# NVIDIA-ISAAC-ROS/isaac_ros_nvblox

Hardware: AMD Instinct MI355X
Metric: frames/s, TSDF+Color+ESDF integrate per frame, synthetic Replica-like 640x480 @0.05m (higher is better)
Workload: dtype f32; 1 GPU; configs[1]: synthetic Replica-like room (SURVEY 8d); scene=room, cameras_per_gpu=1, unique_frames=200, color_deferral=True, parallelism=single GPU

## Files before the change

### isaac_ros_nvblox_amd/csrc/esdf.hip

```cpp
#include <algorithm>
#include <cmath>
#include <cstring>
#include <vector>
#include "nvbx_mapper.h"
#include "nvbx_esdf_mark.h"
#include "nvbx_esdf_edt.h"

using namespace nvbx;

__global__ __launch_bounds__(64) void k_esdf_mark(DMap m, EsdfArgs a) { esdf_mark_worker(m, a, (int)blockIdx.x, (int)gridDim.x); esdf_mark_pass_done(m, a, (int)gridDim.x); }

__global__ __launch_bounds__(256) void k_esdf_edt(DMap m, EsdfArgs a) {
  __shared__ EdtShared sh;
  esdf_edt_worker(m, a, (int)blockIdx.x, (int)gridDim.x, &sh);
}

constexpr int PROP_BATCH = 16;
constexpr int32_t PROP_NONE = INT32_MAX;
__device__ inline bool prop_block(const DMap& m, const EsdfArgs& a, int32_t s, uint32_t* flags_out) {
  const uint32_t flags = m.slot_flags[s];
  *flags_out = flags;
  return (flags & (F_ESDF | F_ESDF_PENDING)) && m.slot_index[3 * s + 2] == a.bz_out;
}
__global__ __launch_bounds__(64) void k_esdf_prop_init(DMap m, EsdfArgs a, int32_t plane_a) {
// ... 203 lines not shown
  NVBX_LAUNCH(m, k_esdf_slice, dim3(std::min(nbx * nby, 4096)), dim3(64), m->d, a.bz_out, a.vz_out, m->p.voxel_size,
                     unknown_value, image_dev, c[0], c[1], nbx, nby);
  NVBX_HIP(hipGetLastError());
  return NVBX_OK;
}

__global__ __launch_bounds__(64) void k_esdf_slice_rows(DMap m, int32_t bz_out, int32_t vz_out, float voxel_size, float unknown, float* img, int64_t cap, int32_t* header) {
  const int32_t bx0 = m.counters[C_ESDF_AABB], by0 = m.counters[C_ESDF_AABB + 1], bx1 = m.counters[C_ESDF_AABB + 2], by1 = m.counters[C_ESDF_AABB + 3];
  const int lane = (int)threadIdx.x;
  const bool empty = bx0 > bx1;
  const int32_t nbx = empty ? 0 : bx1 - bx0 + 1, nby = empty ? 0 : by1 - by0 + 1;
  const bool fits = (int64_t)nbx * nby * 64 <= cap;
  if (blockIdx.x == 0 && lane < 5) header[lane] = lane == 0 ? bx0 : lane == 1 ? by0 : lane == 2 ? bx1 : lane == 3 ? by1 : (empty ? 0 : (fits ? 1 : -1));
  if (empty || !fits) return;
  const int32_t strips_x = (nbx + 7) / 8, cols = nbx * 8;
  for (int32_t s = (int32_t)blockIdx.x; s < strips_x * nby; s += (int32_t)gridDim.x) {
    const int32_t cy = s / strips_x, cx0 = (s - cy * strips_x) * 8;
    uint32_t es = SLOT_NONE;
    if (lane < 8 && cx0 + lane < nbx) es = find_slot(m, bx0 + cx0 + lane, by0 + cy, bz_out, F_ESDF);
    const uint32_t mine = __shfl(es, lane >> 3);
    const bool in_img = cx0 + (lane >> 3) < nbx;
#pragma unroll
    for (int r = 0; r < 8; r++) {
      float v = unknown;
      if (slot_ok(mine)) {
        const uint2 e = m.esdf[(size_t)mine * 512 + vz_out * 64 + r * 8 + (lane & 7)];
        if (e.y & ESDF_OBSERVED) { v = sqrtf(__uint_as_float(e.x)) * voxel_size; if (e.y & ESDF_INSIDE) v = -v; }
      }
      if (in_img) img[(int64_t)(cy * 8 + r) * cols + cx0 * 8 + lane] = v;
    }
  }
}
static int ensure_slice_pinned(nvbx_mapper* m, int64_t elems) {
  if (elems <= m->slice_pinned_elems) return NVBX_OK;
  NVBX_HIP(hipStreamSynchronize(m->stream));
  if (m->slice_pinned) NVBX_HIP(hipHostFree(m->slice_pinned));
  m->slice_pinned = nullptr; m->slice_pinned_elems = 0; m->slice_pinned_dev = nullptr;
  NVBX_HIP(hipHostMalloc((void**)&m->slice_pinned, (size_t)(elems + 16) * 4, hipHostMallocMapped));
  { void* dp = nullptr; NVBX_HIP(hipHostGetDevicePointer(&dp, m->slice_pinned, 0)); m->slice_pinned_dev = (float*)dp; }
  m->slice_pinned_elems = elems;
  return NVBX_OK;
}

extern "C" int nvbx_esdf_slice_to_host(nvbx_mapper* m, float unknown_value, float* image_host, int64_t capacity_elems, int32_t* rows,
                                       int32_t* cols, float aabb[6]) {
  if (!m || !rows || !cols) return NVBX_E_INVALID;
  *rows = 0; *cols = 0;
  if (m->join_side()) return NVBX_E_DEVICE;
  int rc = ensure_slice_pinned(m, std::max<int64_t>(image_host ? capacity_elems : 0, 65536)); if (rc) return rc;
  const EsdfArgs a = m->make_esdf_args();
  int32_t* header = reinterpret_cast<int32_t*>(m->slice_pinned_dev);
  volatile int32_t* h = reinterpret_cast<volatile int32_t*>(m->slice_pinned);
  NVBX_LAUNCH(m, k_esdf_slice_rows, dim3(1024), dim3(64), m->d, a.bz_out, a.vz_out, m->p.voxel_size, unknown_value, m->slice_pinned_dev + 16, m->slice_pinned_elems, header);
  NVBX_HIP(hipGetLastError());
  if (m->wait_stream()) return NVBX_E_DEVICE;
  if (h[4] == 0) return NVBX_OK;
  const float bs = m->p.voxel_size * 8.0f;
  *cols = (h[2] - h[0] + 1) * 8; *rows = (h[3] - h[1] + 1) * 8;
  if (aabb) {
    aabb[0] = (float)h[0] * bs; aabb[1] = (float)h[1] * bs; aabb[2] = (float)a.bz_out * bs;
    aabb[3] = (float)(h[2] + 1) * bs; aabb[4] = (float)(h[3] + 1) * bs; aabb[5] = (float)(a.bz_out + 1) * bs;
  }
  const int64_t n = (int64_t)*rows * *cols;
  if (!image_host || n > capacity_elems) { set_error("slice image capacity too small"); return NVBX_E_CAPACITY; }
  if (h[4] < 0) {
    rc = ensure_slice_pinned(m, n + n / 2); if (rc) return rc;
    return nvbx_esdf_slice_to_host(m, unknown_value, image_host, capacity_elems, rows, cols, aabb);
  }
  memcpy(image_host, m->slice_pinned + 16, (size_t)n * 4);
  return NVBX_OK;
}

__global__ void k_occupancy(const float* img, int64_t n, float unknown, int8_t* grid) {
  for (int64_t i = (int64_t)blockIdx.x * blockDim.x + threadIdx.x; i < n; i += (int64_t)gridDim.x * blockDim.x) {
    const float v = img[i];
    int8_t o = 0;
    if (fabsf(v - unknown) < 1e-2f) o = -1; else if (v <= 0.0f) o = 100;
    grid[i] = o;
  }
}
extern "C" int nvbx_occupancy_grid_from_slice(nvbx_mapper* m, const float* image_dev, int32_t rows, int32_t cols, float unknown_value,
                                              int8_t* grid_dev) {
  if (!m || !image_dev || !grid_dev || rows <= 0 || cols <= 0) return NVBX_E_INVALID;
  if (m->join_side()) return NVBX_E_DEVICE;
  const int64_t n = (int64_t)rows * cols;
  NVBX_LAUNCH(m, k_occupancy, dim3((unsigned)std::min<int64_t>((n + 255) / 256, 2048)), dim3(256), image_dev, n, unknown_value, grid_dev);
  NVBX_HIP(hipGetLastError());
  return NVBX_OK;
}

__global__ __launch_bounds__(64) void k_slice_pointcloud(DMap m, const float* img, int32_t rows, int32_t cols, float ax, float ay,
                                                         float slice_height, float voxel_size, float unknown, float4* out) {
  const int lane = threadIdx.x;
  const int tiles_x = (cols + 7) >> 3, tiles_y = (rows + 7) >> 3;
  for (int32_t t = blockIdx.x; t < tiles_x * tiles_y; t += gridDim.x) {
    const int ty = t / tiles_x, tx = t - ty * tiles_x;
    const int r = ty * 8 + (lane >> 3), c = tx * 8 + (lane & 7);
    bool keep = false; float v = 0.0f;
    if (r < rows && c < cols) { v = img[(int64_t)r * cols + c]; keep = !(fabsf(v - unknown) < 1e-2f); }
    const u64 mask = __ballot(keep);
    int base = 0;
    if (lane == 0 && mask) base = atomicAdd(&m.counters[C_TMP], (int)__popcll(mask));
    base = __shfl(base, 0);
    if (keep) {
      const int off = (int)__popcll(mask & ((1ull << lane) - 1ull));
      out[base + off] = make_float4(ax + voxel_size * (float)c, ay + voxel_size * (float)r, slice_height, v);
    }
  }
}
__global__ void k_zero_tmp2(DMap m) { m.counters[C_TMP] = 0; }

extern "C" int nvbx_pointcloud_from_slice(nvbx_mapper* m, const float* image_dev, int32_t rows, int32_t cols, const float aabb[6],
                                          float slice_height, float unknown_value, float* points_xyzi_dev, int32_t* n_points) {
  if (!m || !image_dev || !aabb || !points_xyzi_dev || !n_points || rows <= 0 || cols <= 0) return NVBX_E_INVALID;
  if (m->join_side()) return NVBX_E_DEVICE;
  NVBX_LAUNCH(m, k_zero_tmp2, dim3(1), dim3(1), m->d);
  const int tiles = ((rows + 7) / 8) * ((cols + 7) / 8);
  NVBX_LAUNCH(m, k_slice_pointcloud, dim3(std::min(tiles, 4096)), dim3(64), m->d, image_dev, rows, cols, aabb[0], aabb[1],
                     slice_height, m->p.voxel_size, unknown_value, (float4*)points_xyzi_dev);
  if (m->fetch_counters()) return NVBX_E_DEVICE;
  *n_points = m->h_counters[C_TMP];
  return NVBX_OK;
}

__global__ void k_esdf_dense(DMap m, int32_t mx, int32_t my, int32_t mz, int32_t sx, int32_t sy, int32_t sz, float voxel_size, float def, float* out) {
  const int64_t n = (int64_t)sx * sy * sz;
  for (int64_t i = (int64_t)blockIdx.x * blockDim.x + threadIdx.x; i < n; i += (int64_t)gridDim.x * blockDim.x) {
    const int32_t z = (int32_t)(i % sz), y = (int32_t)((i / sz) % sy), x = (int32_t)(i / ((int64_t)sz * sy));
    const int32_t gx = mx + x, gy = my + y, gz = mz + z;
    const uint32_t es = find_slot(m, gx >> 3, gy >> 3, gz >> 3, F_ESDF);
    float v = def;
    if (slot_ok(es)) {
      const uint2 e = m.esdf[(size_t)es * 512 + (gx & 7) + 8 * (gy & 7) + 64 * (gz & 7)];
      if (e.y & ESDF_OBSERVED) { v = sqrtf(__uint_as_float(e.x)) * voxel_size; if (e.y & ESDF_INSIDE) v = v * -1.0f; }
    }
    out[i] = v;
  }
}
extern "C" int nvbx_esdf_dense_grid(nvbx_mapper* m, const int32_t min_vox[3], const int32_t size_vox[3], float default_value, float* grid_dev) {
  if (!m || !min_vox || !size_vox || !grid_dev || size_vox[0] <= 0 || size_vox[1] <= 0 || size_vox[2] <= 0) return NVBX_E_INVALID;
  if (m->join_side()) return NVBX_E_DEVICE;
  const int64_t n = (int64_t)size_vox[0] * size_vox[1] * size_vox[2];
  NVBX_LAUNCH(m, k_esdf_dense, dim3((unsigned)std::min<int64_t>((n + 255) / 256, 4096)), dim3(256), m->d, min_vox[0], min_vox[1],
                     min_vox[2], size_vox[0], size_vox[1], size_vox[2], m->p.voxel_size, default_value, grid_dev);
  NVBX_HIP(hipGetLastError());
  return NVBX_OK;
}

__global__ void k_export_dirty(DMap m, int32_t* out_idx, int32_t* out_count, int32_t cap) {
  ListView lv;
  int32_t n = list_open(m, S_LIST_ESDF_DIRTY, &lv); if (n > cap) n = cap;
  if (blockIdx.x == 0 && threadIdx.x == 0) *out_count = n;
  for (int32_t i = blockIdx.x * blockDim.x + threadIdx.x; i < n; i += gridDim.x * blockDim.x) {
    const int32_t s = list_at(m, S_LIST_ESDF_DIRTY, lv, i);
    out_idx[3 * i] = m.slot_index[3 * s]; out_idx[3 * i + 1] = m.slot_index[3 * s + 1]; out_idx[3 * i + 2] = m.slot_index[3 * s + 2];
  }
}
extern "C" int nvbx_esdf_dirty_list(nvbx_mapper* m, int32_t* indices_dev_out, int32_t* count_dev_out, int64_t capacity) {
  if (!m || !indices_dev_out || !count_dev_out || capacity <= 0) return NVBX_E_INVALID;
  if (m->join_side()) return NVBX_E_DEVICE;
  NVBX_LAUNCH(m, k_export_dirty, dim3(64), dim3(256), m->d, indices_dev_out, count_dev_out, (int32_t)std::min<int64_t>(capacity, m->capacity));
  NVBX_HIP(hipGetLastError());
  return NVBX_OK;
}
extern "C" int nvbx_set_view_export(nvbx_mapper* m, int32_t* packed_dev, int64_t capacity) {
  if (!m || capacity < 0) return NVBX_E_INVALID;
  m->view_export = packed_dev; m->view_export_cap = packed_dev ? std::min<int64_t>(capacity, m->capacity) : 0;
  return NVBX_OK;
}
__global__ void k_import_dirty(DMap m, const int32_t* idx, const int32_t* count, int64_t max_count) {
  int64_t n = *count; if (n > max_count) n = max_count;
  for (int64_t i = (int64_t)blockIdx.x * blockDim.x + threadIdx.x; i < n; i += (int64_t)gridDim.x * blockDim.x) {
    const uint32_t s = find_slot(m, idx[3 * i], idx[3 * i + 1], idx[3 * i + 2], F_TSDF);
    if (!slot_ok(s)) continue;
    const uint32_t old = atomicOr(&m.slot_flags[s], F_DIRTY_ESDF);
    if (!(old & F_DIRTY_ESDF)) list_append(m, S_LIST_ESDF_DIRTY, (int32_t)s);
  }
}
extern "C" int nvbx_mark_esdf_dirty(nvbx_mapper* m, const int32_t* indices_dev, const int32_t* count_dev, int64_t max_count) {
  if (!m || !indices_dev || !count_dev || max_count < 0) return NVBX_E_INVALID;
  if (m->join_side()) return NVBX_E_DEVICE;
  if (m->begin_dirtying()) return NVBX_E_DEVICE;
  NVBX_LAUNCH(m, k_import_dirty, dim3(64), dim3(256), m->d, indices_dev, count_dev, max_count);
  NVBX_HIP(hipGetLastError());
  return m->mark_main();
}

__global__ void k_import_dirty_gathered(DMap m, const int32_t* g, int32_t self_rank, int64_t max_count) {
  const int32_t r = (int32_t)blockIdx.y;
  if (r == self_rank) return;
  const int32_t* base = g + (size_t)r * (size_t)(max_count + 1) * 3;
  int64_t n = base[0]; if (n > max_count) n = max_count;
  const int32_t* idx = base + 3;
  for (int64_t i = (int64_t)blockIdx.x * blockDim.x + threadIdx.x; i < n; i += (int64_t)gridDim.x * blockDim.x) {
    const uint32_t s = find_slot(m, idx[3 * i], idx[3 * i + 1], idx[3 * i + 2], F_TSDF);
    if (!slot_ok(s)) continue;
    const uint32_t old = atomicOr(&m.slot_flags[s], F_DIRTY_ESDF);
    if (!(old & F_DIRTY_ESDF)) list_append(m, S_LIST_ESDF_DIRTY, (int32_t)s);
  }
}
__global__ __launch_bounds__(64) void k_import_mark_gathered(DMap m, EsdfArgs a, const int32_t* g, int32_t self_rank, int64_t max_count) {
  const int32_t r = (int32_t)blockIdx.y;
  if (r == self_rank) return;
  const int32_t* base = g + (size_t)r * (size_t)(max_count + 1) * 3;
  int64_t n = base[0]; if (n > max_count) n = max_count;
  const int32_t* idx = base + 3;
  const int srec = S_ESDF_REC + (int)(a.epoch & 1), sh = my_shard();
  for (int64_t i = blockIdx.x; i < n; i += gridDim.x) {
    const uint32_t s = find_slot(m, idx[3 * i], idx[3 * i + 1], idx[3 * i + 2], F_TSDF);
    if (!slot_ok(s)) continue;
    esdf_mark_entry(m, a, s, srec, sh);
  }
}
extern "C" int nvbx_mark_esdf_dirty_gathered(nvbx_mapper* m, const int32_t* gathered_dev, int32_t world, int32_t self_rank, int64_t max_count) {
  if (!m || !gathered_dev || world < 1 || max_count < 0) return NVBX_E_INVALID;
  if (m->join_side()) return NVBX_E_DEVICE;
  if (!(world > 1 || self_rank < 0)) return NVBX_OK;
  const EsdfArgs probe = m->make_esdf_args();
  if (m->p.esdf_mode == 0 && probe.bz_hi >= probe.bz_lo && probe.bz_hi - probe.bz_lo + 1 <= 63) {
    m->mark_pass++;
    const EsdfArgs a = m->make_esdf_args();
    m->unresolved_marks = true;
    NVBX_LAUNCH(m, k_import_mark_gathered, dim3(256, (unsigned)world), dim3(64), m->d, a, gathered_dev, self_rank, max_count);
  } else {
    if (m->begin_dirtying()) return NVBX_E_DEVICE;
    NVBX_LAUNCH(m, k_import_dirty_gathered, dim3(16, (unsigned)world), dim3(256), m->d, gathered_dev, self_rank, max_count);
  }
  NVBX_HIP(hipGetLastError());
  return m->mark_main();
}

__global__ __launch_bounds__(64) void k_undo_marks(DMap m, uint32_t pass_floor, int32_t srec, int32_t vz_out) {
  const int lane = threadIdx.x;
  if (blockIdx.x == 0 && lane < NSH) *shc_at(m, srec, lane, 4) = 0;
  const int32_t hw = m.counters[C_HIGH_WATER];
  for (int32_t s = blockIdx.x; s < hw; s += gridDim.x) {
    const uint32_t flags = m.slot_flags[s], cons = m.slot_consumed[s], stamp = m.slot_stamp[s];
    const bool cons_unres = cons != STAMP_NEVER && (int32_t)(cons - pass_floor) > 0;
    const bool stamp_unres = stamp != STAMP_NEVER && (int32_t)(stamp - pass_floor) > 0;
    if (cons_unres && lane == 0) {
      m.slot_consumed[s] = STAMP_NEVER;
      if (flags & (F_TSDF | F_COLOR | F_ESDF | F_MESH | F_ESDF_PENDING)) {
        const uint32_t old = atomicOr(&m.slot_flags[s], F_DIRTY_ESDF);
        if (!(old & F_DIRTY_ESDF)) list_append(m, S_LIST_ESDF_DIRTY, s);
      }
    }
    if (stamp_unres) {
      if (flags & F_ESDF) {
        const uint32_t meta = m.esdf[(size_t)s * 512 + vz_out * 64 + lane].y;
        const u64 sb = __ballot((meta & ESDF_SITE) != 0), ob = __ballot((meta & ESDF_OBSERVED) != 0), ib = __ballot((meta & ESDF_INSIDE) != 0);
        if (lane == 0) { m.site_bits[s] = sb; m.obs_bits[s] = ob; m.inside_bits[s] = ib; m.slot_stamp[s] = STAMP_NEVER; }
      } else if ((flags & F_ESDF_PENDING) && lane == 0) {
        atomicAnd(&m.slot_flags[s], ~F_ESDF_PENDING);
        m.site_bits[s] = 0ull; m.obs_bits[s] = 0ull; m.inside_bits[s] = 0ull; m.slot_stamp[s] = STAMP_NEVER;
        if (!(flags & (F_TSDF | F_COLOR | F_ESDF | F_MESH))) {
          atomicAnd(&m.slot_flags[s], ~(F_DIRTY_ESDF | F_DIRTY_MESH));
          const int32_t pos = atomicAdd(&m.counters[C_FREE_TOP], 1);
          m.free_stack[pos] = (uint32_t)s;

        }
      }
    }
  }
}
int nvbx_mapper::undo_marks() {
  if (!unresolved_marks) return NVBX_OK;
  if (reset_consumed_list()) return NVBX_E_DEVICE;
  const EsdfArgs a = make_esdf_args();
  NVBX_LAUNCH(this, k_undo_marks, dim3((unsigned)std::min<int64_t>(capacity, 2048)), dim3(64), d, pass_at_last_edt,
              (int32_t)(S_ESDF_REC + (int)(a.epoch & 1)), a.vz_out);
  NVBX_HIP(hipGetLastError());
  unresolved_marks = false; dirty_since_mark = true;
  return NVBX_OK;
}

extern "C" int nvbx_mark_esdf_dirty_gathered_deferred(nvbx_mapper* m, const int32_t* gathered_dev, int32_t world, int32_t self_rank, int64_t max_count) {
  if (!m || !gathered_dev || world < 1 || max_count < 0) return NVBX_E_INVALID;
  if (m->flush_import()) return NVBX_E_DEVICE;
  if (!(world > 1 || self_rank < 0)) return NVBX_OK;
  const EsdfArgs probe = m->make_esdf_args();
  if (!(m->p.esdf_mode == 0 && probe.bz_hi >= probe.bz_lo && probe.bz_hi - probe.bz_lo + 1 <= 63))
    return nvbx_mark_esdf_dirty_gathered(m, gathered_dev, world, self_rank, max_count);
  m->held.import_pending = true; m->held.import_ptr = gathered_dev; m->held.import_world = world; m->held.import_rank = self_rank; m->held.import_max = max_count;
  return NVBX_OK;
}
int nvbx_mapper::flush_import() {
  if (!held.import_pending) return NVBX_OK;
  held.import_pending = false;
  if (flush_edt()) return NVBX_E_DEVICE;
  mark_pass++;
  const EsdfArgs a = make_esdf_args();
  unresolved_marks = true;
  NVBX_LAUNCH(this, k_import_mark_gathered, dim3(256, (unsigned)held.import_world), dim3(64), d, a, held.import_ptr, held.import_rank, held.import_max);
  NVBX_HIP(hipGetLastError());
  return NVBX_OK;
}

int nvbx_mapper::flush_edt() {
  if (held.edt_pending) {
    held.edt_pending = false;
    NVBX_LAUNCH(this, k_esdf_edt, dim3(1024), dim3(256), d, held.edt_args);
    NVBX_HIP(hipGetLastError());
  }
  return NVBX_OK;
}
```

### isaac_ros_nvblox_amd/csrc/esdf3d.hip

```cpp
#include <algorithm>
#include <cmath>
#include "nvbx_mapper.h"

using namespace nvbx;

struct Win3 { int32_t bx0, by0, bz0, nbx, nby, nbz; };
constexpr uint32_t B_NONE = 0xFFFFFFFFu;

__global__ __launch_bounds__(512) void k_esdf3_mark(DMap m, EsdfArgs a) {
  const int tid = threadIdx.x;
  const int vx = tid >> 6, vy = (tid >> 3) & 7, vz = tid & 7;
  ListView lv;
  const int32_t n = list_open(m, S_LIST_ESDF_DIRTY, &lv);
  for (int32_t i = blockIdx.x; i < n; i += gridDim.x) {
    const uint32_t s = (uint32_t)list_at(m, S_LIST_ESDF_DIRTY, lv, i);
    const uint32_t flags = m.slot_flags[s];
    if (!(flags & (F_TSDF | F_ESDF))) continue;
    const float2 tv = m.tsdf[(size_t)s * 512 + tid];
    int observed = 0, inside = 0, site = 0;
    if (a.site_rule == 2) { if (tv.x != 0.0f) observed = 1; if (tv.x > 0.0f) { inside = 1; site = 1; } }
    else if ((flags & F_TSDF) && tv.y >= a.min_weight) {
      observed = 1;
      const int in = tv.x <= 0.0f;
      if (in) inside = 1;
      if ((a.site_rule == 1 || in) && fabsf(tv.x) <= a.site_dist_m) site = 1;
    }
    uint2* ev = &m.esdf[(size_t)s * 512 + vx + 8 * vy + 64 * vz];
    const uint2 old = *ev;
    *ev = make_uint2(old.x, (old.y & ~ESDF_FLAG_MASK) | (observed ? ESDF_OBSERVED : 0u) | (inside ? ESDF_INSIDE : 0u) | (site ? ESDF_SITE : 0u));
    if (tid == 0) {
      atomicOr(&m.slot_flags[s], F_ESDF);
      atomicAnd(&m.slot_flags[s], ~(F_DIRTY_ESDF | F_ESDF_REMARK));
      const int32_t bx = m.slot_index[3 * s], by = m.slot_index[3 * s + 1], bz = m.slot_index[3 * s + 2];
      if (bz == a.bz_out) {
        atomicMin(&m.counters[C_ESDF_AABB + 0], bx); atomicMin(&m.counters[C_ESDF_AABB + 1], by);
        atomicMax(&m.counters[C_ESDF_AABB + 2], bx); atomicMax(&m.counters[C_ESDF_AABB + 3], by);
      }
      atomicMin(&m.counters[C_ESDF3_WIN + 0], bx); atomicMin(&m.counters[C_ESDF3_WIN + 1], by); atomicMin(&m.counters[C_ESDF3_WIN + 2], bz);
      atomicMax(&m.counters[C_ESDF3_WIN + 3], bx); atomicMax(&m.counters[C_ESDF3_WIN + 4], by); atomicMax(&m.counters[C_ESDF3_WIN + 5], bz);
      atomicAdd(&m.counters[C_ESDF3_WIN + 6], 1);
    }
  }
}
__global__ void k_esdf3_reset(DMap m) {
  const int t = threadIdx.x;
  if (t < 3) m.counters[C_ESDF3_WIN + t] = INT32_MAX; else if (t < 6) m.counters[C_ESDF3_WIN + t] = INT32_MIN; else if (t == 6) m.counters[C_ESDF3_WIN + 6] = 0;
  if (t < NSH) *shc_at(m, S_LIST_ESDF_DIRTY, t, 0) = 0;
}

__global__ __launch_bounds__(64) void k_esdf3_bits(DMap m, Win3 w, uint8_t* bits) {
  const int lane = threadIdx.x, y = lane & 7, z = lane >> 3;
  const int64_t nblk = (int64_t)w.nbx * w.nby * w.nbz;
  const int64_t H = (int64_t)w.nby * 8;
  for (int64_t c = blockIdx.x; c < nblk; c += gridDim.x) {
    const int32_t cx = (int32_t)(c % w.nbx), cy = (int32_t)((c / w.nbx) % w.nby), cz = (int32_t)(c / ((int64_t)w.nbx * w.nby));
    const uint32_t s = find_slot(m, w.bx0 + cx, w.by0 + cy, w.bz0 + cz, F_ESDF);
    uint32_t byte = 0;
    if (slot_ok(s)) {
      const uint2* row = &m.esdf[(size_t)s * 512 + 8 * y + 64 * z];
#pragma unroll
      for (int x = 0; x < 8; x++) if (row[x].y & ESDF_SITE) byte |= 1u << x;
    }
    bits[(((int64_t)cz * 8 + z) * H + (int64_t)cy * 8 + y) * w.nbx + cx] = (uint8_t)byte;
  }
}
__device__ inline bool bit_at(const uint8_t* row_bits, int32_t nbx, int64_t x) {
  if (x < 0 || x >= (int64_t)nbx * 8) return false;
  return (row_bits[x >> 3] >> (x & 7)) & 1u;
}
__global__ __launch_bounds__(256) void k_esdf3_x(Win3 w, const uint8_t* bits, int8_t* A, int32_t ri) {
  const int64_t rows = (int64_t)w.nbz * 8 * w.nby * 8;
  const int64_t n = rows * w.nbx;
  for (int64_t i = (int64_t)blockIdx.x * blockDim.x + threadIdx.x; i < n; i += (int64_t)gridDim.x * blockDim.x) {
    const int64_t r = i / w.nbx; const int32_t cx = (int32_t)(i - r * w.nbx);
    const uint8_t* rb = bits + r * w.nbx;
    int8_t out[8];
#pragma unroll
    for (int x = 0; x < 8; x++) {
      const int64_t p = (int64_t)cx * 8 + x;
      int best = 127;
      for (int32_t d = 0; d <= ri; d++) {
        if (bit_at(rb, w.nbx, p - d)) { best = -d; break; }
        if (bit_at(rb, w.nbx, p + d)) { best = d; break; }
      }
      out[x] = (int8_t)best;
    }
    *reinterpret_cast<uint2*>(A + r * ((int64_t)w.nbx * 8) + (int64_t)cx * 8) = *reinterpret_cast<const uint2*>(out);
  }
}
__global__ __launch_bounds__(256) void k_esdf3_y(Win3 w, const int8_t* A, uint32_t* B, int32_t ri) {
  const int64_t W = (int64_t)w.nbx * 8, H = (int64_t)w.nby * 8, D = (int64_t)w.nbz * 8;
  const int64_t n = W * H * D;
  for (int64_t i = (int64_t)blockIdx.x * blockDim.x + threadIdx.x; i < n; i += (int64_t)gridDim.x * blockDim.x) {
    const int64_t x = i % W, y = (i / W) % H, z = i / (W * H);
    const int8_t* col = A + z * H * W + x;
    uint32_t best = B_NONE;
    for (int32_t k = 0; k <= ri; k++) {
      if (best != B_NONE && (uint32_t)(k * k) > (best >> 16)) break;
      for (int sgn = (k == 0 ? 1 : -1); sgn <= 1; sgn += 2) {
        const int64_t yy = y + (int64_t)sgn * k;
        if (yy < 0 || yy >= H) continue;
        const int dx = col[yy * W];
        if (dx == 127) continue;
        const uint32_t key = ((uint32_t)(k * k + dx * dx) << 16) | ((uint32_t)(sgn * k + 128) << 8) | (uint32_t)(dx + 128);
        if (key < best) best = key;
      }
    }
    B[i] = best;
  }
}
__global__ __launch_bounds__(512) void k_esdf3_z(DMap m, Win3 w, int32_t margin, const uint32_t* B, int32_t ri, float max_sq) {
  const int tid = threadIdx.x;
  const int x = tid & 7, y = (tid >> 3) & 7, z = tid >> 6;
  const int32_t ox = w.nbx - 2 * margin, oy = w.nby - 2 * margin, oz = w.nbz - 2 * margin;
  const int64_t W = (int64_t)w.nbx * 8, H = (int64_t)w.nby * 8, D = (int64_t)w.nbz * 8;
  const int64_t nblk = (int64_t)ox * oy * oz;
  for (int64_t c = blockIdx.x; c < nblk; c += gridDim.x) {
    const int32_t cx = (int32_t)(c % ox) + margin, cy = (int32_t)((c / ox) % oy) + margin, cz = (int32_t)(c / ((int64_t)ox * oy)) + margin;
    const uint32_t s = find_slot(m, w.bx0 + cx, w.by0 + cy, w.bz0 + cz, F_ESDF);
    if (!slot_ok(s)) continue;
    const int64_t gx = (int64_t)cx * 8 + x, gy = (int64_t)cy * 8 + y, gz = (int64_t)cz * 8 + z;
    const uint32_t* colz = B + gy * W + gx;
    uint64_t best = ~0ull;
    for (int32_t k = 0; k <= ri; k++) {
      if (best != ~0ull && (uint64_t)(k * k) > (best >> 32)) break;
      for (int sgn = (k == 0 ? 1 : -1); sgn <= 1; sgn += 2) {
        const int64_t zz = gz + (int64_t)sgn * k;
        if (zz < 0 || zz >= D) continue;
        const uint32_t b = colz[zz * H * W];
        if (b == B_NONE) continue;
        const uint64_t key = ((uint64_t)((uint32_t)(k * k) + (b >> 16)) << 32) | ((uint64_t)(uint32_t)(sgn * k + 128) << 24) | (uint64_t)(b & 0xFFFFu);
        if (key < best) best = key;
      }
    }
    uint2* ev = &m.esdf[(size_t)s * 512 + tid];
    const uint32_t fl = ev->y & ESDF_FLAG_MASK;
    float sq = max_sq; int dx = 0, dy = 0, dz = 0;
    if (best != ~0ull && (float)(uint32_t)(best >> 32) <= max_sq) {
      sq = (float)(uint32_t)(best >> 32);
      dz = (int)((best >> 24) & 0xFF) - 128; dy = (int)((best >> 8) & 0xFF) - 128; dx = (int)(best & 0xFF) - 128;
    }
    *ev = make_uint2(__float_as_uint(sq), (esdf_meta(dx, dy, dz, 0, 0, 0) & ~ESDF_FLAG_MASK) | fl);
  }
}

int nvbx_mapper::update_esdf_3d() {
  const EsdfArgs a = make_esdf_args();
  if (dirty_since_mark) NVBX_LAUNCH(this, k_esdf3_mark, dim3((unsigned)std::min<int64_t>(capacity, 1024)), dim3(512), d, a);
  dirty_since_mark = false; premark_consumed = false;
  if (fetch_counters()) return NVBX_E_DEVICE;
  const int32_t* c = h_counters + C_ESDF3_WIN;
  esdf3_blocks_marked = c[6];
  if (c[0] > c[3]) { NVBX_LAUNCH(this, k_esdf3_reset, dim3(1), dim3(64), d); esdf_epoch++; return NVBX_OK; }
  const int32_t rb = a.rb;
  Win3 w;
  w.bx0 = c[0] - 2 * rb; w.by0 = c[1] - 2 * rb; w.bz0 = c[2] - 2 * rb;
  w.nbx = c[3] - c[0] + 1 + 4 * rb; w.nby = c[4] - c[1] + 1 + 4 * rb; w.nbz = c[5] - c[2] + 1 + 4 * rb;
  const int64_t nblk = (int64_t)w.nbx * w.nby * w.nbz, nvox = nblk * 512;
  if (nvox > (1ll << 31)) { set_error("3-D ESDF update: the changed region (+ 2 R) exceeds 2^31 voxels; update more often or lower esdf_max_distance_m"); return NVBX_E_CAPACITY; }
  const int64_t need = nvox / 8 + nvox + nvox * 4 + 1024;
  if (esdf3_scratch.ensure(stream, (size_t)need)) return NVBX_E_DEVICE;
  uint32_t* B = esdf3_scratch.as<uint32_t>();
  int8_t* A = esdf3_scratch.as<int8_t>() + nvox * 4;
  uint8_t* bits = esdf3_scratch.as<uint8_t>() + nvox * 5;
  const unsigned gblk = (unsigned)std::min<int64_t>(nblk, 1 << 16);
  NVBX_LAUNCH(this, k_esdf3_bits, dim3(gblk), dim3(64), d, w, bits);
  NVBX_LAUNCH(this, k_esdf3_x, dim3((unsigned)std::min<int64_t>((nvox / 8 + 255) / 256, 1 << 16)), dim3(256), w, (const uint8_t*)bits, A, a.ri);
  NVBX_LAUNCH(this, k_esdf3_y, dim3((unsigned)std::min<int64_t>((nvox + 255) / 256, 1 << 18)), dim3(256), w, (const int8_t*)A, B, a.ri);
// ... 8 lines not shown
```

### isaac_ros_nvblox_amd/csrc/layers.hip

```cpp
#include <cstring>
#include "nvbx_mapper.h"
using namespace nvbx;

__global__ void k_collect_indices(DMap m, uint32_t layer, int32_t* out, int32_t cap) {
  const int32_t hw = m.counters[C_HIGH_WATER];
  for (int32_t s = blockIdx.x * blockDim.x + threadIdx.x; s < hw; s += gridDim.x * blockDim.x) {
    if (m.slot_flags[s] & layer) {
      const int32_t p = atomicAdd(&m.counters[C_TMP], 1);
      if (p < cap) { out[3 * p] = m.slot_index[3 * s]; out[3 * p + 1] = m.slot_index[3 * s + 1]; out[3 * p + 2] = m.slot_index[3 * s + 2]; }
    }
  }
}
__global__ void k_zero_tmp(DMap m) { m.counters[C_TMP] = 0; }

__global__ void k_viewlist_to_indices(DMap m, const int4* list, int32_t count_idx, uint32_t cam_mask, int32_t* out, int32_t cap) {
  int32_t n = m.counters[count_idx]; if (n > cap) n = cap;
  for (int32_t i = blockIdx.x * blockDim.x + threadIdx.x; i < n; i += gridDim.x * blockDim.x) {
    const int4 r = list[i];
    bool ok = slot_ok((uint32_t)r.x) && m.slot_flags[(uint32_t)r.x];
    if (ok && cam_mask && !(m.table[m.slot_entry[(uint32_t)r.x]].stamp & cam_mask)) ok = false;
    out[3 * i] = ok ? r.y : INT32_MIN; out[3 * i + 1] = ok ? r.z : INT32_MIN; out[3 * i + 2] = ok ? r.w : INT32_MIN;
  }
}

__global__ void k_shardlist_to_indices(DMap m, int list, int32_t* out, int32_t cap, int32_t* n_out) {
  ListView v; int32_t n = list_open(m, list, &v); if (n > cap) n = cap;
  if (blockIdx.x == 0 && threadIdx.x == 0) *n_out = n;
  for (int32_t i = blockIdx.x * blockDim.x + threadIdx.x; i < n; i += gridDim.x * blockDim.x) {
    const uint32_t s = (uint32_t)list_at(m, list, v, i);
    if (slot_ok(s) && m.slot_flags[s]) { out[3 * i] = m.slot_index[3 * s]; out[3 * i + 1] = m.slot_index[3 * s + 1]; out[3 * i + 2] = m.slot_index[3 * s + 2]; }
    else { out[3 * i] = INT32_MIN; out[3 * i + 1] = INT32_MIN; out[3 * i + 2] = INT32_MIN; }
  }
}

__global__ __launch_bounds__(512) void k_gather_blocks(DMap m, uint32_t layer, int32_t occupancy, const int32_t* idx, int32_t n, uint8_t* out, int32_t* found) {
  const int i = blockIdx.x; if (i >= n) return;
  const uint32_t s = find_slot(m, idx[3 * i], idx[3 * i + 1], idx[3 * i + 2], layer);
  const int t = threadIdx.x;
  if (t == 0) found[i] = slot_ok(s) ? 1 : 0;
  if (!slot_ok(s)) {
    const size_t vb = layer == F_ESDF ? sizeof(nvbx_esdf_voxel) : (layer == F_FREESPACE ? sizeof(nvbx_freespace_voxel) : ((layer == F_TSDF && occupancy) ? 4 : 8));
    for (size_t q = t; q < 512 * vb / 4; q += 512) reinterpret_cast<uint32_t*>(out + (size_t)i * 512 * vb)[q] = 0u;
    return;
  }
  if (layer == F_TSDF && occupancy) { reinterpret_cast<float*>(out)[(size_t)i * 512 + t] = m.tsdf[(size_t)s * 512 + t].x; }
  else if (layer == F_TSDF) { reinterpret_cast<float2*>(out)[(size_t)i * 512 + t] = m.tsdf[(size_t)s * 512 + t]; }
  else if (layer == F_COLOR) { reinterpret_cast<uint2*>(out)[(size_t)i * 512 + t] = m.color[(size_t)s * 512 + t]; }
  else if (layer == F_FREESPACE) {
    const int4 v = m.freespace[(size_t)s * 512 + t];
    nvbx_freespace_voxel o;
    o.last_occupied_timestamp_ms = (int64_t)(((u64)(uint32_t)v.y << 32) | (u64)(uint32_t)v.x);
    o.consecutive_occupancy_duration_ms = (int64_t)v.z;
    o.is_high_confidence_freespace = (uint8_t)(v.w & 1); o.initialized = (uint8_t)((v.w >> 1) & 1);
    for (int q = 0; q < 6; q++) o.pad[q] = 0;
    reinterpret_cast<nvbx_freespace_voxel*>(out)[(size_t)i * 512 + t] = o;
  }
  else if (layer == F_ESDF) {
    const int x = t >> 6, y = (t >> 3) & 7, z = t & 7;
    const uint2 v = m.esdf[(size_t)s * 512 + x + 8 * y + 64 * z];
    nvbx_esdf_voxel o;
    o.squared_distance_vox = __uint_as_float(v.x);
    o.parent_direction[0] = (int8_t)(v.y & 0xFF); o.parent_direction[1] = (int8_t)((v.y >> 8) & 0xFF); o.parent_direction[2] = (int8_t)((v.y >> 16) & 0xFF);
    o.observed = (v.y & ESDF_OBSERVED) ? 1 : 0; o.is_inside = (v.y & ESDF_INSIDE) ? 1 : 0; o.is_site = (v.y & ESDF_SITE) ? 1 : 0; o.pad = 0;
    reinterpret_cast<nvbx_esdf_voxel*>(out)[(size_t)i * 512 + t] = o;
  }
}

__global__ __launch_bounds__(512) void k_scatter_blocks(DMap m, uint32_t layer, int32_t occupancy, const int32_t* idx, const uint8_t* in_all, size_t block_bytes,
                                                        int32_t mesh_list, int32_t bz_out, int32_t vz_out, float trunc) {
  __shared__ uint32_t s_slot;
  __shared__ u64 s_sites, s_obs, s_ins;
  const int t = threadIdx.x;
  const int32_t x = idx[3 * blockIdx.x], y = idx[3 * blockIdx.x + 1], z = idx[3 * blockIdx.x + 2];
  const uint8_t* in = in_all + (size_t)blockIdx.x * block_bytes;
  if (t == 0) {
    bool is_new; const int32_t h = hash_insert(m, x, y, z, layer, &is_new);
    uint32_t s = SLOT_NONE;
    if (h >= 0) { do { s = ld_slot_acquire(&m.table[h]); } while (s == SLOT_INVALID); }
    if (slot_ok(s)) {
      uint32_t add = layer;
      if (layer == F_TSDF) add |= F_DIRTY_ESDF | F_DIRTY_MESH;
      const uint32_t old = atomicOr(&m.slot_flags[s], add);
      if (layer == F_TSDF) {
        if (!(old & F_DIRTY_ESDF)) list_append(m, S_LIST_ESDF_DIRTY, (int32_t)s);
        if (!(old & F_DIRTY_MESH)) list_append(m, mesh_list, (int32_t)s);
      }
      if (layer == F_ESDF && z == bz_out) {
        atomicMin(&m.counters[C_ESDF_AABB + 0], x); atomicMin(&m.counters[C_ESDF_AABB + 1], y);
        atomicMax(&m.counters[C_ESDF_AABB + 2], x); atomicMax(&m.counters[C_ESDF_AABB + 3], y);
      }
    }
    s_slot = s; s_sites = 0ull; s_obs = 0ull; s_ins = 0ull;
  }
  __syncthreads();
  const uint32_t s = s_slot;
  if (!slot_ok(s)) return;
  if (layer == F_TSDF && occupancy) m.tsdf[(size_t)s * 512 + t] = make_float2(reinterpret_cast<const float*>(in)[t], 0.0f);
  else if (layer == F_TSDF) {
    const float2 v = reinterpret_cast<const float2*>(in)[t];
    m.tsdf[(size_t)s * 512 + t] = v;
    publish_band(m.slot_flags, s, t, in_band(v.x, v.y, trunc));
  }
  else if (layer == F_COLOR) m.color[(size_t)s * 512 + t] = reinterpret_cast<const uint2*>(in)[t];
  else if (layer == F_ESDF) {
    const int vx = t >> 6, vy = (t >> 3) & 7, vz = t & 7;
    const nvbx_esdf_voxel v = reinterpret_cast<const nvbx_esdf_voxel*>(in)[t];
    m.esdf[(size_t)s * 512 + vx + 8 * vy + 64 * vz] =
        make_uint2(__float_as_uint(v.squared_distance_vox),
                   esdf_meta(v.parent_direction[0], v.parent_direction[1], v.parent_direction[2], v.observed, v.is_inside, v.is_site));
    if (z == bz_out && vz == vz_out) {
      if (v.is_site) atomicOr(&s_sites, 1ull << (vx + 8 * vy));
      if (v.observed) atomicOr(&s_obs, 1ull << (vx + 8 * vy));
      if (v.is_inside) atomicOr(&s_ins, 1ull << (vx + 8 * vy));
    }
    __syncthreads();
    if (t == 0) { m.site_bits[s] = (z == bz_out) ? s_sites : 0ull; m.obs_bits[s] = (z == bz_out) ? s_obs : 0ull; m.inside_bits[s] = (z == bz_out) ? s_ins : 0ull; }
  }
}
uint32_t nvbx::internal_layer(const nvbx_mapper* m, uint32_t layer) {
  const bool occ = m->p.projective_layer_type == 1;
  if (layer == NVBX_LAYER_OCCUPANCY) return occ ? F_TSDF : 0u;
  if (layer == F_TSDF) return occ ? 0u : F_TSDF;
  if (layer == F_FREESPACE) return m->d.freespace ? F_FREESPACE : 0u;
  return layer;
}

static void sort_indices(nvbx_index3d* v, int64_t n) {
  std::sort(v, v + n, [](const nvbx_index3d& a, const nvbx_index3d& b) {
    if (a.x != b.x) return a.x < b.x; if (a.y != b.y) return a.y < b.y; return a.z < b.z; });
}
static int64_t download_indices(nvbx_mapper* m, int64_t n, bool filter, nvbx_index3d* out, int64_t capacity) {
  if (!filter && !(out && std::min(n, capacity) > 0)) return n;
  std::vector<nvbx_index3d> tmp((size_t)n);
  if (n > 0) NVBX_HIP(hipMemcpy(tmp.data(), m->export_idx, (size_t)n * 12, hipMemcpyDeviceToHost));
  if (filter) { tmp.erase(std::remove_if(tmp.begin(), tmp.end(), [](const nvbx_index3d& i) { return i.x == INT32_MIN; }), tmp.end()); n = (int64_t)tmp.size(); }
  const int64_t k = std::min(n, capacity);
  if (out && k > 0) { sort_indices(tmp.data(), n); memcpy(out, tmp.data(), (size_t)k * 12); }
  return n;
}

extern "C" int64_t nvbx_block_indices(nvbx_mapper* m, uint32_t layer, nvbx_index3d* out, int64_t capacity) {
  if (!m || !layer_listable(layer)) return NVBX_E_INVALID;
  layer = internal_layer(m, layer);
  if (!layer) return 0;
  if (m->join_side()) return NVBX_E_DEVICE;
  NVBX_LAUNCH(m, k_zero_tmp, dim3(1), dim3(1), m->d);
  NVBX_LAUNCH(m, k_collect_indices, dim3(256), dim3(256), m->d, layer, m->export_idx, (int32_t)m->capacity);
  if (m->fetch_counters()) return NVBX_E_DEVICE;
  int64_t n = m->h_counters[C_TMP];
  if (n > m->capacity) n = m->capacity;
  return download_indices(m, n, false, out, capacity);
}
extern "C" int64_t nvbx_num_blocks(nvbx_mapper* m, uint32_t layer) { return nvbx_block_indices(m, layer, nullptr, 0); }

extern "C" int64_t nvbx_last_depth_view(nvbx_mapper* m, nvbx_index3d* out, int64_t capacity) {
  if (!m) return NVBX_E_INVALID;
  if (m->last_view_frame == 0) return 0;
  if (m->join_side()) return NVBX_E_DEVICE;
  const uint32_t cam_mask = m->last_view_batch > 1 ? (1u << (m->last_view_batch - 1)) : 0u;
  NVBX_LAUNCH(m, k_viewlist_to_indices, dim3(64), dim3(256), m->d, (const int4*)m->view_list, C_VIEW_COUNT + (int)(m->last_view_frame & 3), cam_mask, m->export_idx, (int32_t)m->capacity);
  if (m->fetch_counters()) return NVBX_E_DEVICE;
  int64_t n = m->h_counters[C_VIEW_COUNT + (m->last_view_frame & 3)]; if (n > m->capacity) n = m->capacity;
  return download_indices(m, n, true, out, capacity);
}
extern "C" int64_t nvbx_last_color_view(nvbx_mapper* m, nvbx_index3d* out, int64_t capacity) {
  if (!m) return NVBX_E_INVALID;
  if (m->join_side()) return NVBX_E_DEVICE;
  NVBX_LAUNCH(m, k_shardlist_to_indices, dim3(64), dim3(256), m->d, (int)S_LIST_COLOR, m->export_idx, (int32_t)m->capacity, m->export_count);
  int32_t n32 = 0;
  NVBX_HIP(hipMemcpyAsync(&n32, m->export_count, 4, hipMemcpyDeviceToHost, m->stream));
  NVBX_HIP(hipStreamSynchronize(m->stream));
  return download_indices(m, n32, false, out, capacity);
}

size_t nvbx::ref_voxel_bytes(uint32_t layer) { return layer == F_ESDF ? sizeof(nvbx_esdf_voxel) : (layer == NVBX_LAYER_OCCUPANCY ? sizeof(nvbx_occupancy_voxel) : (layer == F_FREESPACE ? sizeof(nvbx_freespace_voxel) : 8)); }

extern "C" int nvbx_get_blocks(nvbx_mapper* m, uint32_t layer, const nvbx_index3d* idx, int64_t n, void* voxels_out, int32_t* found_out) {
  if (!m || !idx || !voxels_out || n < 0 || !layer_readable(layer)) return NVBX_E_INVALID;
  if (m->join_side()) return NVBX_E_DEVICE;
  const size_t bb = 512 * ref_voxel_bytes(layer);
  const uint32_t ilayer = internal_layer(m, layer);
  if (!ilayer) { if (found_out) memset(found_out, 0, (size_t)n * 4); return NVBX_OK; }
  const int64_t chunk = std::max<int64_t>(1, (int64_t)((m->staging.bytes - 65536) / (bb + 16)));
  for (int64_t o = 0; o < n; o += chunk) {
    const int64_t c = std::min(chunk, n - o);
    int32_t* d_idx = m->staging.as<int32_t>(); int32_t* d_found = d_idx + 3 * c;
    uint8_t* d_out = m->staging.as<uint8_t>() + (((size_t)c * 16 + 255) & ~(size_t)255);
    NVBX_HIP(hipMemcpyAsync(d_idx, idx + o, (size_t)c * 12, hipMemcpyHostToDevice, m->stream));
    NVBX_LAUNCH(m, k_gather_blocks, dim3((unsigned)c), dim3(512), m->d, ilayer, (int32_t)(layer == NVBX_LAYER_OCCUPANCY), d_idx, (int32_t)c, d_out, d_found);
    NVBX_HIP(hipMemcpyAsync((uint8_t*)voxels_out + (size_t)o * bb, d_out, (size_t)c * bb, hipMemcpyDeviceToHost, m->stream));
    if (found_out) NVBX_HIP(hipMemcpyAsync(found_out + o, d_found, (size_t)c * 4, hipMemcpyDeviceToHost, m->stream));
    NVBX_HIP(hipStreamSynchronize(m->stream));
  }
  return NVBX_OK;
}
extern "C" int nvbx_get_block(nvbx_mapper* m, uint32_t layer, nvbx_index3d idx, void* voxels_out) {
  int32_t found = 0;
  const int rc = nvbx_get_blocks(m, layer, &idx, 1, voxels_out, &found);
  if (rc) return rc;
  return found ? NVBX_OK : NVBX_E_NOTFOUND;
}
extern "C" int nvbx_set_blocks(nvbx_mapper* m, uint32_t layer, const nvbx_index3d* idx, int64_t n, const void* voxels_in) {
  if (!m || (n > 0 && (!voxels_in || !idx)) || n < 0 || !layer_writable(layer)) return NVBX_E_INVALID;
  const uint32_t ilayer = internal_layer(m, layer);
  if (!ilayer) { set_error("nvbx_set_blocks: this mapper's projective layer type does not hold that layer"); return NVBX_E_INVALID; }
  for (int64_t i = 0; i < n; i++) if (!nvbx_index_in_range(idx[i].x, idx[i].y, idx[i].z)) { set_error("nvbx_set_blocks: block index outside +-2^20"); return NVBX_E_INVALID; }
  if (m->join_side()) return NVBX_E_DEVICE;
  if (m->capacity < m->max_capacity) {
    if (m->fetch_counters()) return NVBX_E_DEVICE;
    m->h_mirror[0] = m->h_counters[C_FREE_TOP];
    const int rcg = m->maybe_grow(n); if (rcg) return rcg;
  }
  if (m->begin_dirtying()) return NVBX_E_DEVICE;
  const size_t bb = 512 * ref_voxel_bytes(layer);
  const EsdfArgs ea = m->make_esdf_args();
  const int64_t chunk = std::max<int64_t>(1, (int64_t)((m->staging.bytes - 65536) / (bb + 16)));
  for (int64_t o = 0; o < n; o += chunk) {
    const int64_t c = std::min(chunk, n - o);
    int32_t* d_idx = m->staging.as<int32_t>();
    uint8_t* d_in = m->staging.as<uint8_t>() + (((size_t)c * 16 + 255) & ~(size_t)255);
    NVBX_HIP(hipMemcpyAsync(d_idx, idx + o, (size_t)c * 12, hipMemcpyHostToDevice, m->stream));
    NVBX_HIP(hipMemcpyAsync(d_in, (const uint8_t*)voxels_in + (size_t)o * bb, (size_t)c * bb, hipMemcpyHostToDevice, m->stream));
    NVBX_LAUNCH(m, k_scatter_blocks, dim3((unsigned)c), dim3(512), m->d, ilayer, (int32_t)(layer == NVBX_LAYER_OCCUPANCY), (const int32_t*)d_idx, (const uint8_t*)d_in, bb,
                (int32_t)m->mesh_list_live(), ea.bz_out, ea.vz_out, m->p.truncation_distance_vox * m->p.voxel_size);
    NVBX_HIP(hipStreamSynchronize(m->stream));
  }
  return NVBX_OK;
}
extern "C" int nvbx_set_block(nvbx_mapper* m, uint32_t layer, nvbx_index3d idx, const void* voxels_in) {
  return nvbx_set_blocks(m, layer, &idx, 1, voxels_in);
}
```

### isaac_ros_nvblox_amd/csrc/lidar.hip

```cpp
#define NVBX_WGT_HERE
#include "nvbx_view.h"

#ifdef NVBX_WG_TIMES
int wgt_bind_lidar(unsigned long long* buf) { return hipMemcpyToSymbol(HIP_SYMBOL(g_wgt), &buf, sizeof(buf)) == hipSuccess ? 0 : -1; }
#endif

struct ViewGrid {
  uint8_t* fine;
  uint8_t* coarse;
  int32_t ox, oy, oz;
  int32_t ncx, ncy, ncz;
  int32_t cx, cy, cz;
  uint32_t tag;
};
#ifndef NVBX_VG_NEAR
#define NVBX_VG_NEAR 0
#define NVBX_VG_CHUNK 16
#endif
constexpr int VG_NEAR = NVBX_VG_NEAR, VG_CHUNK = NVBX_VG_CHUNK;
constexpr uint32_t VG_NONE = 0xFFFFFFFFu;

#ifndef NVBX_VIEW_GRID_ATTR
#define NVBX_VIEW_GRID_ATTR
#endif
// ... 264 lines not shown
  int32_t n_mine = 0;
  const int32_t G = (n + 7) >> 3;
  auto ridx = [&](int32_t p, int g) -> int32_t { return NVBX_LIDAR_SPARSE_STRIDED ? g * G + p : p * 8 + g; };
  int32_t pass = (int32_t)blockIdx.x * 4 + wv;
  int4 rec_next = (pass < G && ridx(pass, grp) < n) ? view_list[ridx(pass, grp)] : make_int4((int32_t)SLOT_NONE, 0, 0, 0);
  for (; pass < G; pass += n_waves) {
    const int4 rec_g = rec_next;
    if (pass + n_waves < G && ridx(pass + n_waves, grp) < n) rec_next = view_list[ridx(pass + n_waves, grp)]; else rec_next = make_int4((int32_t)SLOT_NONE, 0, 0, 0);
    bool sparse_g = ridx(pass, grp) < n && slot_ok((uint32_t)rec_g.x);
    float org_g[3];
    sensor_block_origin(f, rec_g.y, rec_g.z, rec_g.w, org_g);
    int c0_g = 0, r0_g = 0, w_g = 0, h_g = 0;
    {
      float off[3], pc[3], u = 0.0f, v = 0.0f;
      rotate(f.R_CL, (float)(lane & 1) * bs, (float)((lane >> 1) & 1) * bs, (float)((lane >> 2) & 1) * bs, off);
      pc[0] = org_g[0] + off[0]; pc[1] = org_g[1] + off[1]; pc[2] = org_g[2] + off[2];
      const bool okc = nvbx_lidar_project(&sensor.l, pc, nvbx_lidar_range(pc), &u, &v) != 0;
      const u64 bad = __ballot(!okc);
      if ((bad >> (8 * grp)) & 0xFFull) sparse_g = false;
      float umin = u, umax = u, vmin = v, vmax = v;
#pragma unroll
      for (int o = 1; o < 8; o <<= 1) {
        umin = fminf(umin, __shfl_xor(umin, o)); umax = fmaxf(umax, __shfl_xor(umax, o));
        vmin = fminf(vmin, __shfl_xor(vmin, o)); vmax = fmaxf(vmax, __shfl_xor(vmax, o));
      }
      if (sparse_g) {
        if (umax - umin > (float)cols * 0.5f) sparse_g = false;
        c0_g = (int)floorf(umin - 0.75f); r0_g = (int)floorf(vmin - 0.75f);
        w_g = (int)floorf(umax + 0.75f) - c0_g + 1; h_g = (int)floorf(vmax + 0.75f) - r0_g + 1;
        if (w_g < 1 || h_g < 1 || w_g * h_g > 64) sparse_g = false;
      }
    }
    const u64 sparse_groups = __ballot(sparse_g);
    uint32_t dmask = 0;
#pragma unroll 1
    for (int j = 0; j < 8; j++) {
    const int32_t i = ridx(pass, j);
    if (i >= n) continue;
    bool sparse = ((sparse_groups >> (8 * j)) & 1ull) != 0;
    const uint32_t slot = (uint32_t)__builtin_amdgcn_readlane(rec_g.x, 8 * j);
    if (!sparse) { if (lane == 0) view_class[i] = 0; if (slot_ok(slot)) dmask |= 1u << j; continue; }
    const float org[3] = {__int_as_float(__builtin_amdgcn_readlane(__float_as_int(org_g[0]), 8 * j)), __int_as_float(__builtin_amdgcn_readlane(__float_as_int(org_g[1]), 8 * j)),
                          __int_as_float(__builtin_amdgcn_readlane(__float_as_int(org_g[2]), 8 * j))};
    const int c0 = __builtin_amdgcn_readlane(c0_g, 8 * j), r0 = __builtin_amdgcn_readlane(r0_g, 8 * j), w = __builtin_amdgcn_readlane(w_g, 8 * j), h = __builtin_amdgcn_readlane(h_g, 8 * j);
    const int ly = (int)(((float)lane + 0.5f) * (1.0f / (float)w)), lx = lane - ly * w;
    const int bc = c0 + lx, brr = r0 + ly;
    const bool in_img = ly < h && bc >= 0 && brr >= 0 && bc < cols && brr < rows;
    const float bd = in_img ? img(pix(brr, bc, cols)) : 0.0f;
    const float2 te = sensor.el_tab[in_img ? brr : 0], ta = sensor.az_tab[in_img ? bc : 0];
    bool anyq = false;
    const int nq = (w + 1) * (h + 1);
    const float iw1 = 1.0f / (float)(w + 1);
    for (int qi = lane; qi < nq; qi += 64) {
      const int qy = (int)(((float)qi + 0.5f) * iw1), qx = qi - qy * (w + 1);
      const int x0 = c0 - 1 + qx, y0 = r0 - 1 + qy;
      if (!(x0 < 0 || y0 < 0 || x0 + 1 > cols - 1 || y0 + 1 > rows - 1)) {
        const int32_t i00 = pix(y0, x0, cols);
        const float f00 = img(i00), f10 = img(i00 + 1), f01 = img(i00 + cols), f11 = img(i00 + cols + 1);
        if (f00 > 0.0f && f10 > 0.0f && f01 > 0.0f && f11 > 0.0f) {
          const float mx = fmaxf(fmaxf(f00, f10), fmaxf(f01, f11)), mn = fminf(fminf(f00, f10), fminf(f01, f11));
          if (mx - mn <= sensor.max_diff_m) anyq = true;
        }
      }
    }
    if (__ballot(anyq)) sparse = false;
    if (!sparse) { if (lane == 0) view_class[i] = 0; dmask |= 1u << j; continue; }
    float ob[3] = {0.0f, 0.0f, 0.0f}, db[3] = {1.0f, 0.0f, 0.0f};
    const float dir[3] = {te.y * ta.y, te.y * ta.x, te.x};
    bool crossing = false; int axis = 0;
    if (in_img && bd > 0.0f) {
      float t3[3];
      rotate(f.R_LC, org[0], org[1], org[2], t3);
      const float ivs = 1.0f / vs;
      ob[0] = -t3[0] * ivs; ob[1] = -t3[1] * ivs; ob[2] = -t3[2] * ivs;
      rotate(f.R_LC, dir[0], dir[1], dir[2], db);
      int a = 0; if (fabsf(db[1]) > fabsf(db[a])) a = 1; if (fabsf(db[2]) > fabsf(a == 0 ? db[0] : db[1])) a = 2;
      axis = a;
      const float oa = a == 0 ? ob[0] : (a == 1 ? ob[1] : ob[2]), da = a == 0 ? db[0] : (a == 1 ? db[1] : db[2]);
      const float obb = a == 0 ? ob[1] : (a == 1 ? ob[2] : ob[0]), dbb = a == 0 ? db[1] : (a == 1 ? db[2] : db[0]);
      const float occ = a == 0 ? ob[2] : (a == 1 ? ob[0] : ob[1]), dcc = a == 0 ? db[2] : (a == 1 ? db[0] : db[1]);
      const float ida = 1.0f / da;
      const float t0 = (0.5f - oa) * ida, t7 = (7.5f - oa) * ida;
      const float b0 = obb + t0 * dbb - 0.5f, b7 = obb + t7 * dbb - 0.5f, cc0 = occ + t0 * dcc - 0.5f, cc7 = occ + t7 * dcc - 0.5f;
      crossing = fmaxf(b0, b7) >= -1.0f && fminf(b0, b7) <= 8.0f && fmaxf(cc0, cc7) >= -1.0f && fminf(cc0, cc7) <= 8.0f;
    }
    const u64 cross = __ballot(crossing);
    const int nb = (int)__popcll(cross);
    if (crossing) {
      const int k = (int)__popcll(cross & ((1ull << lane) - 1ull));
      float* q = s_beam[wv][k];
      q[0] = ob[0]; q[1] = ob[1]; q[2] = ob[2]; q[3] = db[0]; q[4] = db[1]; q[5] = db[2];
      q[6] = __int_as_float(pix(brr, bc, cols)); q[7] = bd; q[8] = dir[0]; q[9] = dir[1]; q[10] = dir[2]; q[11] = __int_as_float(axis);
    }
    __threadfence_block();
    __builtin_amdgcn_wave_barrier();
    int32_t ns = 0;
    const float pre = sensor.max_ray_dist_m / vs + 0.02f, pre2 = pre * pre;
    for (int it0 = 0; it0 < nb * 32; it0 += 64) {
      const int item = it0 + lane;
      const int kb = item >> 5, sl = (item >> 2) & 7, cell = item & 3;
      bool keep = false; int vox = 0;
      if (kb < nb) {
        const float* q = s_beam[wv][kb];
        const float o0 = q[0], o1 = q[1], o2 = q[2], d0 = q[3], d1 = q[4], d2 = q[5];
        const int a = __float_as_int(q[11]);
        const float oa = a == 0 ? o0 : (a == 1 ? o1 : o2), da = a == 0 ? d0 : (a == 1 ? d1 : d2);
        const float obb = a == 0 ? o1 : (a == 1 ? o2 : o0), dbb = a == 0 ? d1 : (a == 1 ? d2 : d0);
        const float occ = a == 0 ? o2 : (a == 1 ? o0 : o1), dcc = a == 0 ? d2 : (a == 1 ? d0 : d1);
        const float t = ((float)sl + 0.5f - oa) / da;
        const int jb = (int)floorf(obb + t * dbb - 0.5f) + (cell & 1), jc = (int)floorf(occ + t * dcc - 0.5f) + (cell >> 1);
        if (jb >= 0 && jb <= 7 && jc >= 0 && jc <= 7) {
          const int vx = a == 0 ? sl : (a == 1 ? jc : jb), vy = a == 0 ? jb : (a == 1 ? sl : jc), vz = a == 0 ? jc : (a == 1 ? jb : sl);
          const float px = (float)vx + 0.5f - o0, py = (float)vy + 0.5f - o1, pz = (float)vz + 0.5f - o2;
          const float cx = py * d2 - pz * d1, cy = pz * d0 - px * d2, cz = px * d1 - py * d0;
          keep = (cx * cx + cy * cy) + cz * cz <= pre2;
          vox = vz + 8 * vy + 64 * vx;
        }
      }
      const u64 km = __ballot(keep);
      if (keep) { const int pos = ns + (int)__popcll(km & ((1ull << lane) - 1ull)); if (pos < 512) s_item[wv][pos] = (uint16_t)((kb << 9) | vox); }
      ns += (int32_t)__popcll(km);
    }
    if (ns > 512) sparse = false;
    if (lane == 0) view_class[i] = sparse ? 1 : 0;
    if (!sparse) { dmask |= 1u << j; __builtin_amdgcn_wave_barrier(); continue; }
    uint32_t old = 0;
    if (lane == 0) old = atomicOr(&m.slot_flags[slot], F_TSDF | F_DIRTY_ESDF | F_DIRTY_MESH | F_BAND_STALE);
    __threadfence_block();
    __builtin_amdgcn_wave_barrier();
    for (int it0 = 0; it0 < ns; it0 += 64) {
      if (it0 + lane >= ns) continue;
      const int code = s_item[wv][it0 + lane];
      const float* q = s_beam[wv][code >> 9];
      const int vox = code & 511, vx = vox >> 6, vy = (vox >> 3) & 7, vz = vox & 7;
      float off[3], pc[3];
      sensor_voxel_offset(f, vx, vy, vz, off);
      pc[0] = org[0] + off[0]; pc[1] = org[1] + off[1]; pc[2] = org[2] + off[2];
      const float r = nvbx_lidar_range(pc);
      if (f.max_dist > 0.0f && r > f.max_dist) continue;
      float u, v;
      if (!nvbx_lidar_project(&sensor.l, pc, r, &u, &v)) continue;
      const int c = (int)floorf(u), rr = (int)floorf(v);
      if (c < 0 || rr < 0 || c >= cols || rr >= rows) continue;
      if (pix(rr, c, cols) != __float_as_int(q[6])) continue;
      const float d = q[7];
      const float bdx = q[8], bdy = q[9], bdz = q[10];
      const float dot = __builtin_fmaf(pc[2], bdz, __builtin_fmaf(pc[1], bdy, pc[0] * bdx));
      const float ex = __builtin_fmaf(-dot, bdx, pc[0]), ey = __builtin_fmaf(-dot, bdy, pc[1]), ez = __builtin_fmaf(-dot, bdz, pc[2]);
      if (__builtin_fmaf(ez, ez, __builtin_fmaf(ey, ey, ex * ex)) > sensor.max_ray_dist_m * sensor.max_ray_dist_m) continue;
      float2* vp = &m.tsdf[(size_t)slot * 512 + vox];
      float2 fin = *vp;
      if (tsdf_fuse_plain(f, &fin, d, r)) *vp = fin;
    }
    if (lane == 0) {
      if (!(old & F_DIRTY_ESDF)) list_append(m, S_LIST_ESDF_DIRTY, (int32_t)slot);
      if (!(old & F_DIRTY_MESH)) list_append(m, mesh_list, (int32_t)slot);
    }
    n_mine++;
    __threadfence_block();
    __builtin_amdgcn_wave_barrier();
    }
    if (dense_list && dmask) {
      const int sh = my_shard();
      int32_t base0 = 0;
      if (lane == 0) base0 = atomicAdd(shc_at(m, S_LIDAR_SPARSE, sh, 1), (int32_t)__popc(dmask));
      base0 = __shfl(base0, 0);
      if (lane < 8 && ((dmask >> lane) & 1u)) {
        const int32_t pos = base0 + (int32_t)__popc(dmask & ((1u << lane) - 1u));
        if (pos < list_cap) dense_list[(size_t)sh * list_cap + pos] = ridx(pass, lane);
      }
    }
  }
  if (lane == 0 && n_mine) atomicAdd(shc_at(m, S_LIDAR_SPARSE, my_shard(), 0), n_mine);
}

int launch_lidar_sparse(nvbx_mapper* m, const FrameSet<DepthF32, 1>& fs, const LidarSensor& sensor, bool plain, uint8_t** view_class, int32_t** dense_list) {
  *view_class = nullptr; *dense_list = nullptr;
  static const int enabled = nvbx_knob_switch(getenv("NVBX_LIDAR_SPARSE"));
  if (!enabled || !plain || !(m->p.lidar_nearest_interpolation_max_allowable_dist_to_ray_vox <= 0.55f)) return NVBX_OK;
  const size_t class_bytes = ((size_t)m->capacity + 15) & ~(size_t)15;
  if (m->view_class.ensure(m->stream, class_bytes + (size_t)NSH * (size_t)m->capacity * 4)) return NVBX_E_DEVICE;
  uint8_t* vc = m->view_class.as<uint8_t>();
  static const int sparse_grid = nvbx_knob_lidar_sparse_grid(getenv("NVBX_LIDAR_SPARSE_GRID"));
  static const int use_list = nvbx_knob_switch(getenv("NVBX_LIDAR_DENSE_LIST"));
  int32_t* dense = (use_list && !m->view_export) ? reinterpret_cast<int32_t*>(vc + class_bytes) : nullptr;
  NVBX_LAUNCH(m, (k_lidar_sparse<DepthF32>), dim3(sparse_grid), dim3(256), m->d, fs, sensor, (const int4*)m->view_list, (int32_t)m->capacity, m->mesh_list_live(), vc, dense);
  *dense_list = dense;
  *view_class = vc;
  return NVBX_OK;
}

int launch_view_grid(nvbx_mapper* m, const FrameSet<DepthF32, 1>& fs, const LidarSensor& sensor, int tiles, int32_t fence_report, bool* used) {
  *used = false;
  static const int enabled = getenv("NVBX_LIDAR_VIEW_GRID") ? atoi(getenv("NVBX_LIDAR_VIEW_GRID")) : 1;
  const Frame& f = fs.f[0];
  if (!enabled || !(f.max_dist > 0.0f) || m->capacity > (1ll << 24)) return NVBX_OK;
  const double reach = (double)f.max_dist / (double)f.block_size;
  double wz = 0.0;
  const double hxy = std::hypot((double)f.R_LC[6], (double)f.R_LC[7]);
  for (int k = 0; k < sensor.l.rows; k++) wz = std::max(wz, hxy * std::fabs((double)m->lidar_host[2 * (size_t)k + 1]) + std::fabs((double)f.R_LC[8] * (double)m->lidar_host[2 * (size_t)k]));
  int64_t H = (int64_t)std::ceil(reach) + 2, Hz = std::min<int64_t>(H, (int64_t)std::ceil(reach * std::min(1.0, wz)) + 2);
  static const int64_t reach_cap = getenv("NVBX_VIEW_GRID_REACH") ? atoll(getenv("NVBX_VIEW_GRID_REACH")) : 0;
  if (reach_cap > 0) { H = std::min(H, reach_cap); Hz = std::min(Hz, reach_cap); }
  const int64_t ncx = (2 * H + 1 + 3) / 4, ncz = (2 * Hz + 1 + 3) / 4;
  const int64_t cells = ncx * ncx * ncz;
  static const int64_t cap_mb = getenv("NVBX_VIEW_GRID_MAX_MB") ? atoll(getenv("NVBX_VIEW_GRID_MAX_MB")) : 128;
  if (ncx > 256 || ncz > 256 || cells * 64 > (cap_mb << 20)) return NVBX_OK;
  const size_t coarse_bytes = ((size_t)cells + 3) & ~(size_t)3;
  bool grew = false;
  if (m->view_grid_fine.ensure(m->stream, (size_t)cells * 64 + coarse_bytes, &grew)) return NVBX_E_DEVICE;
  if (grew) { m->view_grid_cells = cells; m->view_grid_dirty = true; }
  if (m->view_grid_dirty) NVBX_HIP(hipMemsetAsync(m->view_grid_fine.p, 0, m->view_grid_fine.bytes, m->stream));
  m->view_grid_dirty = true;
  ViewGrid vg{};
  vg.fine = m->view_grid_fine.as<uint8_t>(); vg.coarse = vg.fine + (size_t)m->view_grid_cells * 64;
  vg.cx = (int32_t)std::floor(f.t_LC[0] / f.block_size); vg.cy = (int32_t)std::floor(f.t_LC[1] / f.block_size); vg.cz = (int32_t)std::floor(f.t_LC[2] / f.block_size);
  vg.ox = vg.cx - (int32_t)H; vg.oy = vg.cy - (int32_t)H; vg.oz = vg.cz - (int32_t)Hz;
  vg.ncx = (int32_t)ncx; vg.ncy = (int32_t)ncx; vg.ncz = (int32_t)ncz;
  vg.tag = 0x80000000u | f.frame_id;
  NVBX_LAUNCH(m, (k_mark_view_grid<DepthF32>), dim3(tiles), dim3(64), m->d, fs, sensor, (int4*)m->view_list, (int32_t)m->capacity, (int32_t)(m->premark_consumed ? 1 : 0), fence_report, vg);
  const int64_t coarse_lines = ((cells + 3) / 4 + 15) / 16;
  const int64_t scan_wg = (coarse_lines + 4 * VG_SCAN_WAVES - 1) / (4 * VG_SCAN_WAVES);
  NVBX_LAUNCH(m, k_scan_view_grid, dim3((unsigned)scan_wg), dim3(64 * VG_SCAN_WAVES), m->d, f.frame_id, (int4*)m->view_list, (int32_t)m->capacity, vg);
  const int64_t n_hint = std::max<int64_t>(0, __atomic_load_n(&m->h_mirror[2], __ATOMIC_RELAXED));
  const int64_t rec_wg = n_hint == 0 ? 512 : std::max<int64_t>(8, std::min<int64_t>(2048, (n_hint + n_hint / 4 + 255) / 256));
  NVBX_LAUNCH(m, k_resolve_view, dim3((unsigned)rec_wg), dim3(256), m->d, f.frame_id, (int4*)m->view_list, (int32_t)m->capacity, vg.tag);
  NVBX_HIP(hipGetLastError());
  m->view_grid_dirty = false;
  *used = true;
  return NVBX_OK;
}

static bool same_lidar(const nvbx_lidar& a, const nvbx_lidar& b) { return memcmp(&a, &b, sizeof(a)) == 0; }

static int ensure_lidar_tables(nvbx_mapper* m, const nvbx_lidar* ld, const nvbx_lidar_model& l) {
  if (m->lidar_tab.p && same_lidar(m->lidar_cached, *ld)) return NVBX_OK;
  const size_t n = (size_t)l.rows + (size_t)l.cols;
  if (m->lidar_tab.ensure(m->stream, n * sizeof(float2))) return NVBX_E_DEVICE;
  m->lidar_host.resize(n * 2);
  for (int k = 0; k < l.rows; k++) {
    const double el = (double)l.max_el - (double)k * (double)l.rpp_el;
    m->lidar_host[2 * (size_t)k] = (float)sin(el); m->lidar_host[2 * (size_t)k + 1] = (float)cos(el);
  }
  for (int j = 0; j < l.cols; j++) {
    const double az = -(double)NVBX_PI_F + (double)j * (double)l.rpp_az;
    m->lidar_host[2 * ((size_t)l.rows + j)] = (float)sin(az); m->lidar_host[2 * ((size_t)l.rows + j) + 1] = (float)cos(az);
  }
  NVBX_HIP(hipMemcpyAsync(m->lidar_tab.p, m->lidar_host.data(), n * sizeof(float2), hipMemcpyHostToDevice, m->stream));
  NVBX_HIP(hipStreamSynchronize(m->stream));
  m->lidar_cached = *ld;
  return NVBX_OK;
}

static bool lidar_ok(const nvbx_lidar* ld) {
  return ld && ld->num_azimuth_divisions >= 2 && ld->num_elevation_divisions >= 2 && ld->max_elevation_rad > ld->min_elevation_rad &&
         image_dims_ok(ld->num_elevation_divisions, ld->num_azimuth_divisions);
}

extern "C" int nvbx_integrate_lidar_depth(nvbx_mapper* m, const float* range_dev, int32_t rows, int32_t cols, const float T_L_C[16],
                                          const nvbx_lidar* lidar) {
  if (!m || !range_dev || !T_L_C || !lidar_ok(lidar) || rows != lidar->num_elevation_divisions || cols != lidar->num_azimuth_divisions) {
    set_error("nvbx_integrate_lidar_depth: invalid argument (range image must be elevation x azimuth divisions)"); return NVBX_E_INVALID;
  }
  if (!nvbx_pose_in_range(T_L_C, m->p.voxel_size * 8.0f, m->p.lidar_max_integration_distance_m + 2.0f * m->p.truncation_distance_vox * m->p.voxel_size)) {
    set_error("nvbx_integrate_lidar_depth: T_L_C is not finite or lies outside the addressable block range (+-2^20 blocks)"); return NVBX_E_INVALID; }
  NVBX_HIP(hipSetDevice(m->device));
  if (m->join_side()) return NVBX_E_DEVICE;
  const nvbx_lidar_model l = nvbx_lidar_make(cols, rows, lidar->min_valid_range_m, lidar->min_elevation_rad, lidar->max_elevation_rad);
  const int rc = ensure_lidar_tables(m, lidar, l); if (rc) return rc;
  { const int rcg = m->maybe_grow(); if (rcg) return rcg; }
  { const int rc2 = next_frame_id(m); if (rc2) return rc2; }
  nvbx_camera none{1.f, 1.f, 0.f, 0.f, cols, rows};
  FrameSet<DepthF32, 1> fs{}; fs.n = 1; fs.img[0] = DepthF32{range_dev};
  fs.f[0] = m->make_frame(T_L_C, &none, rows, cols, m->p.raycast_subsampling_factor);
  fs.f[0].max_dist = m->p.lidar_max_integration_distance_m;
  LidarSensor s{l, m->lidar_tab.as<const float2>(), m->lidar_tab.as<const float2>() + rows,
                m->p.lidar_linear_interpolation_max_allowable_difference_vox * m->p.voxel_size,
                m->p.lidar_nearest_interpolation_max_allowable_dist_to_ray_vox * m->p.voxel_size};
  return integrate_lidar_frame(m, fs, s);
}

__global__ void k_depth_from_points(const float* pts, int64_t n, nvbx_lidar_model l, float* img) {
  for (int64_t i = (int64_t)blockIdx.x * blockDim.x + threadIdx.x; i < n; i += (int64_t)gridDim.x * blockDim.x) {
    const float p[3] = {pts[3 * i], pts[3 * i + 1], pts[3 * i + 2]};
    if (isnan(p[0]) || isnan(p[1]) || isnan(p[2])) continue;
    const float r = nvbx_lidar_range(p);
    float u, v;
    if (!nvbx_lidar_project(&l, p, r, &u, &v)) continue;
    const int c = (int)floorf(u), rr = (int)floorf(v);
    if (c < 0 || rr < 0 || c >= l.cols || rr >= l.rows) continue;
    img[(int64_t)rr * l.cols + c] = r;
  }
}
extern "C" int nvbx_depth_image_from_pointcloud(nvbx_mapper* m, const float* points_xyz_dev, int64_t n_points, const nvbx_lidar* lidar,
                                                float* range_dev) {
  if (!m || !points_xyz_dev || n_points < 0 || !lidar_ok(lidar) || !range_dev) { set_error("nvbx_depth_image_from_pointcloud: invalid argument"); return NVBX_E_INVALID; }
  NVBX_HIP(hipSetDevice(m->device));
  if (m->join_side()) return NVBX_E_DEVICE;
  const nvbx_lidar_model l = nvbx_lidar_make(lidar->num_azimuth_divisions, lidar->num_elevation_divisions, lidar->min_valid_range_m,
                                             lidar->min_elevation_rad, lidar->max_elevation_rad);
  NVBX_HIP(hipMemsetAsync(range_dev, 0, (size_t)l.rows * l.cols * sizeof(float), m->stream));
  if (n_points > 0)
    NVBX_LAUNCH(m, k_depth_from_points, dim3((unsigned)std::min<int64_t>((n_points + 255) / 256, 4096)), dim3(256), points_xyz_dev, n_points, l, range_dev);
  NVBX_HIP(hipGetLastError());
  return NVBX_OK;
}
```

### isaac_ros_nvblox_amd/csrc/maintenance.hip

```cpp
#include <algorithm>
#include <cstring>
#include <vector>
#include "nvbx_mapper.h"

using namespace nvbx;

constexpr uint32_t LAYER_MASK = F_TSDF | F_COLOR | F_ESDF | F_MESH | F_ESDF_PENDING | F_FREESPACE;

__device__ inline void free_slot(DMap& m, uint32_t slot) {
  const int32_t pos = atomicAdd(&m.counters[C_FREE_TOP], 1);
  m.free_stack[pos] = slot;
  m.slot_consumed[slot] = STAMP_NEVER; m.slot_stamp[slot] = STAMP_NEVER; m.slot_cam[slot] = STAMP_NEVER;
}

__device__ inline void wave_list_append(const DMap& m, int32_t list, bool push, int32_t v, int lane) {
  const u64 mask = __ballot(push);
  if (!mask) return;
  const int sh = my_shard();
  int32_t base = 0;
  const int leader = __ffsll((long long)mask) - 1;
  if (lane == leader) base = atomicAdd(shc_at(m, list, sh, 0), (int32_t)__popcll(mask));
  base = __shfl(base, leader);
  if (push) {
    const int32_t p = base + (int32_t)__popcll(mask & ((1ull << lane) - 1ull));
    if (p < (int32_t)m.capacity) m.lists[((size_t)list * NSH + sh) * m.capacity + p] = v;
  }
}
template <bool OCC>
__global__ __launch_bounds__(512) __attribute__((amdgpu_waves_per_eu(8, 8))) void k_decay(DMap m, float factor, float thresh, uint32_t exclude_stamp, uint32_t exclude_mask, int32_t mesh_list,
                                               int32_t bz_lo, int32_t bz_hi, int32_t bz_out, float trunc, int32_t* cleared_idx, int32_t keep_blocks, int32_t to_free, float free_dist, Entry* next_table,
                                               Entry* clear_table, int32_t n_clear_wg) {
  const int tid = threadIdx.x, lane = tid & 63;
  const int32_t n_decay_wg = (int32_t)gridDim.x - n_clear_wg;
  if ((int32_t)blockIdx.x >= n_decay_wg) {
    uint4* t = reinterpret_cast<uint4*>(clear_table);
    const uint4 ff = make_uint4(0xFFFFFFFFu, 0xFFFFFFFFu, 0xFFFFFFFFu, 0xFFFFFFFFu);
    for (uint32_t i = ((uint32_t)blockIdx.x - (uint32_t)n_decay_wg) * 512u + (uint32_t)tid; i <= m.mask; i += (uint32_t)n_clear_wg * 512u) t[i] = ff;
    return;
  }
  const int32_t hw = m.counters[C_HIGH_WATER];
  const int32_t stride = n_decay_wg * 8;
  for (int32_t s0 = (int32_t)blockIdx.x * 8 + (tid >> 6); s0 < hw; s0 += 64 * stride) {
    const int32_t mine = s0 + lane * stride;
    const uint32_t fl = mine < hw ? m.slot_flags[mine] : 0u;
    bool act = (fl & F_TSDF) != 0;
    if (exclude_stamp && act) {
      const uint32_t st = m.slot_cam[mine];
      if (stamp_frame(st) == exclude_stamp && (st & exclude_mask)) act = false;
    }
    const u64 act_mask = __ballot(act);
    bool my_alive = false; uint32_t my_band = 0u;
#pragma unroll 1
    for (int j = 0; j < 64; j++) {
      if (!((act_mask >> j) & 1ull)) continue;
      const int32_t slot = s0 + j * stride;
      const uint32_t bflags = (uint32_t)__builtin_amdgcn_readlane((int)fl, j);
      float2* vp = &m.tsdf[(size_t)slot * 512 + lane];
      float2 tv[8];
#pragma unroll
      for (int r = 0; r < 8; r++) tv[r] = vp[r * 64];
      bool live = false;
#pragma unroll
      for (int r = 0; r < 8; r++) {
        if (OCC) {
          float v = tv[r].x;
          if (v > 0.0f) { v = v + thresh; if (v < 0.0f && !to_free) v = 0.0f; }
          else if (v < 0.0f && !to_free) { v = v + factor; if (v > 0.0f) v = 0.0f; }
          tv[r] = make_float2(v, 0.0f); live = live || v != 0.0f;
        } else {
          const float w0 = tv[r].y;
          float w = w0 * factor;
          if (!(w < thresh)) live = true;
          else if (to_free && w0 > 0.0f) { tv[r].x = free_dist; w = thresh; }
          tv[r].y = w;
        }
      }
      const bool alive = keep_blocks || __ballot(live) != 0ull;
      uint32_t band = 0u;
      if (alive) {
#pragma unroll
        for (int r = 0; r < 8; r++) {
          vp[r * 64] = tv[r];
          if (!OCC && __ballot(in_band(tv[r].x, tv[r].y, trunc)) != 0ull) band |= 1u << (F_BAND_SHIFT + r);
        }
      } else {
#pragma unroll
        for (int r = 0; r < 8; r++) vp[r * 64] = make_float2(0.0f, 0.0f);
        if (!OCC) {
          uint2* cp = &m.color[(size_t)slot * 512 + lane];
#pragma unroll
          for (int r = 0; r < 8; r++) cp[r * 64] = make_uint2(0u, 0u);
          if (bflags & F_FREESPACE) {
            int4* fp = &m.freespace[(size_t)slot * 512 + lane];
#pragma unroll
            for (int r = 0; r < 8; r++) fp[r * 64] = make_int4(0, 0, 0, 0);
          }
        }
      }
      if (lane == j) { my_alive = alive; my_band = band; }
    }
    const int32_t slot = mine;
    bool push_esdf = false, push_esdf2 = false, push_mesh = false, push_cleared = false; int32_t esdf2 = 0;
    if (act) {
      uint32_t old = F_DIRTY_MESH;
      if (my_alive) {
        if (!OCC) { atomicAnd(&m.slot_flags[slot], ~(F_BAND | F_BAND_STALE)); }
        const uint32_t o = atomicOr(&m.slot_flags[slot], OCC ? F_DIRTY_ESDF : (F_DIRTY_ESDF | F_DIRTY_MESH | my_band));
        if (!OCC) old = o;
        push_esdf = !(o & F_DIRTY_ESDF);
      } else {
        if (!OCC) old = atomicOr(&m.slot_flags[slot], F_DIRTY_MESH);
        push_cleared = true;
        atomicAnd(&m.slot_flags[slot], ~(F_TSDF | F_COLOR | F_FEATURE | F_MESH | F_FREESPACE | F_BAND | F_BAND_STALE));
        const int32_t bx = m.slot_index[3 * slot], by = m.slot_index[3 * slot + 1], bz = m.slot_index[3 * slot + 2];
        if (bz >= bz_lo && bz <= bz_hi) {
          const uint32_t es = bz_out == INT32_MIN ? (uint32_t)slot : any_slot(m, bx, by, bz_out);
          if (slot_ok(es) && (m.slot_flags[es] & F_ESDF)) {
            const uint32_t eold = atomicOr(&m.slot_flags[es], F_ESDF_REMARK | F_DIRTY_ESDF);
            if (!(eold & F_DIRTY_ESDF)) { push_esdf2 = true; esdf2 = (int32_t)es; }
          }
        }
        if (!(fl & (F_ESDF | F_ESDF_PENDING))) { atomicAnd(&m.slot_flags[slot], OCC ? ~(F_DIRTY_ESDF | F_DIRTY_MESH) : ~F_DIRTY_ESDF); free_slot(m, (uint32_t)slot); }
      }
      push_mesh = !(old & F_DIRTY_MESH);
    }
    wave_list_append(m, S_LIST_ESDF_DIRTY, push_esdf, slot, lane);
    wave_list_append(m, S_LIST_ESDF_DIRTY, push_esdf2, esdf2, lane);
    wave_list_append(m, mesh_list, push_mesh, slot, lane);
    {
      const u64 cm = __ballot(push_cleared);
      if (cm) {
        int32_t base = 0;
        const int leader = __ffsll((long long)cm) - 1;
        if (lane == leader) base = atomicAdd(&m.counters[C_CLEARED], (int32_t)__popcll(cm));
        base = __shfl(base, leader);
        if (push_cleared) {
          const int32_t p = base + (int32_t)__popcll(cm & ((1ull << lane) - 1ull));
          if (p < (int32_t)m.capacity) { cleared_idx[3 * p] = m.slot_index[3 * slot]; cleared_idx[3 * p + 1] = m.slot_index[3 * slot + 1]; cleared_idx[3 * p + 2] = m.slot_index[3 * slot + 2]; }
        }
      }
    }
    if (next_table && mine < hw) {
      const uint32_t layers_after = (act && !my_alive) ? (fl & (F_ESDF | F_ESDF_PENDING)) : (fl & LAYER_MASK);
      if (layers_after) {
        const int32_t x = m.slot_index[3 * slot], y = m.slot_index[3 * slot + 1], z = m.slot_index[3 * slot + 2];
        const uint32_t stamp = m.table[m.slot_entry[slot]].stamp;
        const u64 key = pack_key(x, y, z);
        uint32_t h = table_pos(m, x, y, z);
        for (;;) {
          const u64 k = atomicCAS(&next_table[h].key, KEY_EMPTY, key);
          if (k == KEY_EMPTY) break;
          h = (h + 1) & m.mask;
        }
        next_table[h].slot = (uint32_t)slot; next_table[h].stamp = stamp;
        m.slot_entry[slot] = h;
      }
    }
  }
}

__global__ __launch_bounds__(512) void k_clear_outside(DMap m, float cx, float cy, float cz, float r2, float bs, int32_t srec, int32_t esdf3d, int32_t* cleared_idx) {
  __shared__ int32_t s_out[512];
  __shared__ uint32_t s_oflags[512];
  __shared__ int32_t s_nout;
  const int32_t hw = m.counters[C_HIGH_WATER];
  const int tid = threadIdx.x;
  for (int32_t base = (int32_t)blockIdx.x * 512; base < hw; base += (int32_t)gridDim.x * 512) {
    __syncthreads();
    if (tid == 0) s_nout = 0;
    __syncthreads();
    {
      const int32_t slot = base + tid;
      const uint32_t flags = slot < hw ? m.slot_flags[slot] : 0u;
      if (flags & LAYER_MASK) {
        const float dx = ((float)m.slot_index[3 * slot] * bs + bs * 0.5f) - cx;
        const float dy = ((float)m.slot_index[3 * slot + 1] * bs + bs * 0.5f) - cy;
        const float dz = ((float)m.slot_index[3 * slot + 2] * bs + bs * 0.5f) - cz;
        const float d2 = (dx * dx + dy * dy) + dz * dz;
        if (d2 > r2) { const int32_t q = atomicAdd(&s_nout, 1); s_out[q] = slot; s_oflags[q] = flags; }
      }
    }
    __syncthreads();
    const int32_t nout = s_nout;
    for (int32_t k = 0; k < nout; k++) {
    const int32_t slot = s_out[k];
    const uint32_t flags = s_oflags[k];
    if (flags & F_TSDF) m.tsdf[(size_t)slot * 512 + tid] = make_float2(0.0f, 0.0f);
    if (flags & F_COLOR) m.color[(size_t)slot * 512 + tid] = make_uint2(0u, 0u);
    if (flags & F_ESDF) m.esdf[(size_t)slot * 512 + tid] = make_uint2(0u, 0u);
    if (flags & F_FREESPACE) m.freespace[(size_t)slot * 512 + tid] = make_int4(0, 0, 0, 0);
    if (tid == 0) {
      if (flags & F_TSDF) {
        const int32_t p = atomicAdd(&m.counters[C_CLEARED], 1);
        if (p < (int32_t)m.capacity) { cleared_idx[3 * p] = m.slot_index[3 * slot]; cleared_idx[3 * p + 1] = m.slot_index[3 * slot + 1]; cleared_idx[3 * p + 2] = m.slot_index[3 * slot + 2]; }
      }
      if ((flags & F_ESDF) && esdf3d) {
        const int32_t bx = m.slot_index[3 * slot], by = m.slot_index[3 * slot + 1], bz = m.slot_index[3 * slot + 2];
        atomicMin(&m.counters[C_ESDF3_WIN + 0], bx); atomicMin(&m.counters[C_ESDF3_WIN + 1], by); atomicMin(&m.counters[C_ESDF3_WIN + 2], bz);
        atomicMax(&m.counters[C_ESDF3_WIN + 3], bx); atomicMax(&m.counters[C_ESDF3_WIN + 4], by); atomicMax(&m.counters[C_ESDF3_WIN + 5], bz);
      } else if ((flags & F_ESDF) && m.site_bits[slot] != 0ull) {
        const int sh = my_shard(); const int32_t bx = m.slot_index[3 * slot], by = m.slot_index[3 * slot + 1];
        atomicMin(shc_at(m, srec, sh, 0), bx); atomicMin(shc_at(m, srec, sh, 1), by);
        atomicMax(shc_at(m, srec, sh, 2), bx); atomicMax(shc_at(m, srec, sh, 3), by);
      }
      atomicAnd(&m.slot_flags[slot], ~(LAYER_MASK | F_FEATURE | F_DIRTY_ESDF | F_DIRTY_MESH | F_ESDF_REMARK | F_BAND | F_BAND_STALE));
      m.site_bits[slot] = 0ull; m.obs_bits[slot] = 0ull; m.inside_bits[slot] = 0ull; free_slot(m, (uint32_t)slot);
    }
    }
  }
}

struct ShapeArgs { int32_t n; nvbx_bounding_shape s[16]; };
__global__ __launch_bounds__(512) void k_clear_shapes(DMap m, ShapeArgs sh, float vs, float bs, int32_t mesh_list, float trunc, int32_t occupancy) {
  __shared__ int s_touched;
  const int32_t hw = m.counters[C_HIGH_WATER];
  const int tid = threadIdx.x;
  const int vx = tid >> 6, vy = (tid >> 3) & 7, vz = tid & 7;
  for (int32_t slot = blockIdx.x; slot < hw; slot += gridDim.x) {
    if (!(m.slot_flags[slot] & F_TSDF)) continue;
    __syncthreads();
    if (tid == 0) s_touched = 0;
    __syncthreads();
    const float px = voxel_center(m.slot_index[3 * slot], vx, bs, vs), py = voxel_center(m.slot_index[3 * slot + 1], vy, bs, vs),
                pz = voxel_center(m.slot_index[3 * slot + 2], vz, bs, vs);
    bool inside = false;
    for (int k = 0; k < sh.n && !inside; k++) {
      const nvbx_bounding_shape& q = sh.s[k];
      if (q.kind == 0) { const float dx = px - q.a[0], dy = py - q.a[1], dz = pz - q.a[2]; inside = ((dx * dx + dy * dy) + dz * dz) <= q.b[0] * q.b[0]; }
      else inside = px >= q.a[0] && py >= q.a[1] && pz >= q.a[2] && px <= q.b[0] && py <= q.b[1] && pz <= q.b[2];
    }
    float2 fin = m.tsdf[(size_t)slot * 512 + tid];
    if (inside) { fin = make_float2(0.0f, 0.0f); m.tsdf[(size_t)slot * 512 + tid] = fin; s_touched = 1; }
    __syncthreads();
    if (s_touched && !occupancy) publish_band(m.slot_flags, (uint32_t)slot, tid, in_band(fin.x, fin.y, trunc));
    if (tid == 0 && s_touched) {
      const uint32_t old = atomicOr(&m.slot_flags[slot], F_DIRTY_ESDF | F_DIRTY_MESH);
      if (!(old & F_DIRTY_ESDF)) list_append(m, S_LIST_ESDF_DIRTY, slot);
      if (!(old & F_DIRTY_MESH)) list_append(m, mesh_list, slot);
    }
  }
}
extern "C" int nvbx_clear_tsdf_inside_shapes(nvbx_mapper* m, const nvbx_bounding_shape* shapes_host, int32_t n_shapes) {
  if (!m || n_shapes < 0 || (n_shapes > 0 && !shapes_host)) return NVBX_E_INVALID;
  NVBX_HIP(hipSetDevice(m->device));
  if (m->join_side()) return NVBX_E_DEVICE;
  if (m->begin_dirtying()) return NVBX_E_DEVICE;
  const int grid = (int)std::min<int64_t>(m->capacity, 1024);
  for (int32_t o = 0; o < n_shapes; o += 16) {
    ShapeArgs a{}; a.n = std::min(16, n_shapes - o);
    for (int i = 0; i < a.n; i++) a.s[i] = shapes_host[o + i];
    NVBX_LAUNCH(m, k_clear_shapes, dim3(grid), dim3(512), m->d, a, m->p.voxel_size, m->p.voxel_size * 8.0f, m->mesh_list_live(),
                m->p.truncation_distance_vox * m->p.voxel_size, (int32_t)(m->p.projective_layer_type == 1));
  }
  NVBX_HIP(hipGetLastError());
  return m->mark_main();
}

__global__ void k_save_stamps(DMap m, uint32_t* tmp) {
  const int32_t hw = m.counters[C_HIGH_WATER];
  for (int32_t s = blockIdx.x * blockDim.x + threadIdx.x; s < hw; s += gridDim.x * blockDim.x)
    tmp[s] = (m.slot_flags[s] & LAYER_MASK) ? m.table[m.slot_entry[s]].stamp : 0xFFFFFFFFu;
  if (blockIdx.x == 0 && threadIdx.x < 4) m.counters[C_ESDF_AABB + threadIdx.x] = threadIdx.x < 2 ? INT32_MAX : INT32_MIN;
}
__global__ void k_reinsert(DMap m, const uint32_t* tmp, int32_t bz_out) {
  const int32_t hw = m.counters[C_HIGH_WATER];
  for (int32_t s = blockIdx.x * blockDim.x + threadIdx.x; s < hw; s += gridDim.x * blockDim.x) {
    const uint32_t flags = m.slot_flags[s];
    if (!(flags & LAYER_MASK)) continue;
    const int32_t x = m.slot_index[3 * s], y = m.slot_index[3 * s + 1], z = m.slot_index[3 * s + 2];
    const u64 key = pack_key(x, y, z);
    uint32_t h = table_pos(m, x, y, z);
    for (;;) {
      const u64 k = atomicCAS(&m.table[h].key, KEY_EMPTY, key);
      if (k == KEY_EMPTY) break;
      h = (h + 1) & m.mask;
    }
    m.table[h].slot = (uint32_t)s; m.table[h].stamp = tmp[s];
    m.slot_entry[s] = h;
    if ((flags & F_ESDF) && z == bz_out) {
      int32_t* bb = &m.counters[C_ESDF_AABB];
      if (x < __hip_atomic_load(&bb[0], __ATOMIC_RELAXED, __HIP_MEMORY_SCOPE_AGENT)) atomicMin(&bb[0], x);
      if (y < __hip_atomic_load(&bb[1], __ATOMIC_RELAXED, __HIP_MEMORY_SCOPE_AGENT)) atomicMin(&bb[1], y);
      if (x > __hip_atomic_load(&bb[2], __ATOMIC_RELAXED, __HIP_MEMORY_SCOPE_AGENT)) atomicMax(&bb[2], x);
      if (y > __hip_atomic_load(&bb[3], __ATOMIC_RELAXED, __HIP_MEMORY_SCOPE_AGENT)) atomicMax(&bb[3], y);
    }
  }
}

#ifndef NVBX_DECAY_INLINE_REBUILD
#define NVBX_DECAY_INLINE_REBUILD 1
#endif
static int prepare_tables(nvbx_mapper* m, Entry** next_out, Entry** clear_out) {
  const size_t bytes = ((size_t)m->d.mask + 1) * sizeof(Entry);
  if (m->table_mask_extra != m->d.mask) {
    NVBX_HIP(hipStreamSynchronize(m->stream));
    if (m->table_spare) NVBX_HIP(hipFree(m->table_spare));
    if (m->table_dirty) NVBX_HIP(hipFree(m->table_dirty));
    m->table_spare = nullptr; m->table_dirty = nullptr; m->table_mask_extra = m->d.mask;
  }
  if (!m->table_spare) {
    NVBX_HIP(hipMalloc(&m->table_spare, bytes));
    NVBX_HIP(hipMemsetAsync(m->table_spare, 0xFF, bytes, m->stream));
  }
  *next_out = static_cast<Entry*>(m->table_spare); *clear_out = static_cast<Entry*>(m->table_dirty);
  return NVBX_OK;
}
static int rotate_tables(nvbx_mapper* m) {
  Entry* old_live = m->d.table;
  m->d.table = static_cast<Entry*>(m->table_spare);
  m->table_spare = m->table_dirty;
  m->table_dirty = old_live;
  NVBX_HIP(hipGetLastError());
  return NVBX_OK;
}
static int rebuild_table(nvbx_mapper* m) {
  uint32_t* tmp = (uint32_t*)m->export_idx;
  const unsigned rg = (unsigned)std::min<int64_t>((m->capacity + 255) / 256, 2048);
  NVBX_LAUNCH(m, k_save_stamps, dim3(rg), dim3(256), m->d, tmp);
  NVBX_HIP(hipMemsetAsync(m->d.table, 0xFF, ((size_t)m->d.mask + 1) * sizeof(Entry), m->stream));
  NVBX_LAUNCH(m, k_reinsert, dim3(rg), dim3(256), m->d, tmp, m->make_esdf_args().bz_out);
  NVBX_HIP(hipGetLastError());
  return NVBX_OK;
}

extern "C" int nvbx_decay_occupancy(nvbx_mapper* m) {
  if (!m) return NVBX_E_INVALID;
  if (m->p.projective_layer_type != 1) { set_error("nvbx_decay_occupancy: not an occupancy mapper"); return NVBX_E_INVALID; }
  NVBX_HIP(hipSetDevice(m->device));
  if (m->join_side()) return NVBX_E_DEVICE;
  if (m->undo_marks()) return NVBX_E_DEVICE;
  if (m->begin_dirtying()) return NVBX_E_DEVICE;
  EsdfArgs ea = m->make_esdf_args();
  if (m->p.esdf_mode == 1) { ea.bz_lo = INT32_MIN + 1; ea.bz_hi = INT32_MAX; ea.bz_out = INT32_MIN; }
  else if (ea.plane_on) { ea.bz_lo = INT32_MIN + 1; ea.bz_hi = INT32_MAX; }
  const int64_t hw_seen = std::max<int64_t>(1, __atomic_load_n(&m->h_mirror[1], __ATOMIC_RELAXED));
  const bool inline_rebuild = NVBX_DECAY_INLINE_REBUILD != 0;
  Entry* next_table = nullptr; Entry* clear_table = nullptr;
  if (inline_rebuild && prepare_tables(m, &next_table, &clear_table)) return NVBX_E_DEVICE;
  const int32_t n_clear_wg = clear_table ? 64 : 0;
  NVBX_LAUNCH(m, k_decay<true>, dim3((unsigned)std::min<int64_t>(std::min<int64_t>(m->capacity, 4096), std::max<int64_t>(512, (hw_seen + 7) / 8)) + (unsigned)n_clear_wg), dim3(512), m->d,
              log_odds(m->p.free_region_decay_probability), log_odds(m->p.occupied_region_decay_probability), 0u, 0u, (int32_t)m->mesh_list_live(),
              ea.bz_lo, ea.bz_hi, ea.bz_out, 0.0f, m->cleared_idx, (int32_t)(m->p.decay_deallocate_decayed_blocks ? 0 : 1), (int32_t)(m->p.occupancy_decay_to_free ? 1 : 0), 0.0f,
              next_table, clear_table, n_clear_wg);
  return inline_rebuild ? rotate_tables(m) : rebuild_table(m);
}

extern "C" int nvbx_decay_tsdf(nvbx_mapper* m, int32_t exclude_last_view) {
  if (!m) return NVBX_E_INVALID;
  if (m->p.projective_layer_type == 1) { set_error("nvbx_decay_tsdf: occupancy mapper (use nvbx_decay_occupancy)"); return NVBX_E_INVALID; }
  NVBX_HIP(hipSetDevice(m->device));
  if (m->join_side()) return NVBX_E_DEVICE;
  if (m->undo_marks()) return NVBX_E_DEVICE;
  if (m->begin_dirtying()) return NVBX_E_DEVICE;
  static const int decay_grid = nvbx_knob_decay_grid(getenv("NVBX_DECAY_GRID"));
  const int64_t hw_seen = std::max<int64_t>(1, __atomic_load_n(&m->h_mirror[1], __ATOMIC_RELAXED));
  const int grid = (int)std::min<int64_t>(std::min<int64_t>(m->capacity, decay_grid), std::max<int64_t>(512, (hw_seen + 7) / 8));
  EsdfArgs ea = m->make_esdf_args();
  if (m->p.esdf_mode == 1) { ea.bz_lo = INT32_MIN + 1; ea.bz_hi = INT32_MAX; ea.bz_out = INT32_MIN; }
  else if (ea.plane_on) { ea.bz_lo = INT32_MIN + 1; ea.bz_hi = INT32_MAX; }
  const bool inline_rebuild = NVBX_DECAY_INLINE_REBUILD != 0;
  Entry* next_table = nullptr; Entry* clear_table = nullptr;
  if (inline_rebuild && prepare_tables(m, &next_table, &clear_table)) return NVBX_E_DEVICE;
  const int32_t n_clear_wg = clear_table ? 64 : 0;
  NVBX_LAUNCH(m, k_decay<false>, dim3((unsigned)(grid + n_clear_wg)), dim3(512), m->d, m->p.tsdf_decay_factor, m->p.tsdf_decayed_weight_threshold,
                     exclude_last_view ? m->last_camera_view_frame : 0u, m->last_camera_view_mask, m->mesh_list_live(), ea.bz_lo, ea.bz_hi, ea.bz_out,
                     m->p.truncation_distance_vox * m->p.voxel_size, m->cleared_idx, (int32_t)(m->p.decay_deallocate_decayed_blocks ? 0 : 1),
                     (int32_t)(m->p.tsdf_set_free_distance_on_decayed ? 1 : 0), m->p.tsdf_decayed_free_distance_vox * m->p.voxel_size,
                     next_table, clear_table, n_clear_wg);
  return inline_rebuild ? rotate_tables(m) : rebuild_table(m);
}

extern "C" int nvbx_clear_outside_radius(nvbx_mapper* m, const float center[3], float radius) {
  if (!m || !center) return NVBX_E_INVALID;
  NVBX_HIP(hipSetDevice(m->device));
  if (m->join_side()) return NVBX_E_DEVICE;
  if (m->undo_marks()) return NVBX_E_DEVICE;
  const int grid = (int)std::min<int64_t>((m->capacity + 511) / 512, 2048);
  NVBX_LAUNCH(m, k_clear_outside, dim3(grid), dim3(512), m->d, center[0], center[1], center[2], radius * radius, m->p.voxel_size * 8.0f,
              (int32_t)(S_ESDF_REC + (int)(m->esdf_epoch & 1)), (int32_t)(m->p.esdf_mode == 1), m->cleared_idx);
  return rebuild_table(m);
}

__global__ void k_zero_cleared(DMap m) { m.counters[C_CLEARED] = 0; }
extern "C" int64_t nvbx_take_cleared_blocks(nvbx_mapper* m, nvbx_index3d* out, int64_t capacity) {
  if (!m || capacity < 0 || (capacity > 0 && !out)) return NVBX_E_INVALID;
  if (m->fetch_counters()) return NVBX_E_DEVICE;
  int64_t n = m->h_counters[C_CLEARED];
  if (n > m->capacity) n = m->capacity;
  if (n == 0) return 0;
  std::vector<nvbx_index3d> tmp((size_t)n);
  NVBX_HIP(hipMemcpy(tmp.data(), m->cleared_idx, (size_t)n * 12, hipMemcpyDeviceToHost));
  auto less = [](const nvbx_index3d& a, const nvbx_index3d& b) { if (a.x != b.x) return a.x < b.x; if (a.y != b.y) return a.y < b.y; return a.z < b.z; };
  std::sort(tmp.begin(), tmp.end(), less);
  tmp.erase(std::unique(tmp.begin(), tmp.end(), [](const nvbx_index3d& a, const nvbx_index3d& b) { return a.x == b.x && a.y == b.y && a.z == b.z; }), tmp.end());
  const int64_t u = (int64_t)tmp.size();
  if (u > capacity) return u;
  memcpy(out, tmp.data(), (size_t)u * 12);
  NVBX_LAUNCH(m, k_zero_cleared, dim3(1), dim3(1), m->d);
  NVBX_HIP(hipGetLastError());
  return u;
}

__global__ void k_grow_free_stack(DMap m, uint32_t old_cap, uint32_t new_cap) {
  const int32_t top = m.counters[C_FREE_TOP];
  const uint32_t added = new_cap - old_cap;
  for (uint32_t i = blockIdx.x * blockDim.x + threadIdx.x; i < added; i += gridDim.x * blockDim.x) m.free_stack[top + i] = new_cap - 1u - i;
}
__global__ void k_grow_commit(DMap m, int32_t added) { m.counters[C_FREE_TOP] += added; m.host_mirror[0] = m.counters[C_FREE_TOP]; }
__global__ void k_remap_mesh_records(MeshRecord* rec, int32_t n, int64_t old_vreg, int64_t new_vreg, int64_t old_treg, int64_t new_treg) {
  for (int32_t i = blockIdx.x * blockDim.x + threadIdx.x; i < n; i += gridDim.x * blockDim.x) {
    MeshRecord r = rec[i];
    if (r.x == INT32_MIN || r.vbase < 0) continue;
    const int64_t sv = r.vbase / old_vreg, st = r.tbase / old_treg;
    r.vbase = (int32_t)(sv * new_vreg + (r.vbase - sv * old_vreg)); r.tbase = (int32_t)(st * new_treg + (r.tbase - st * old_treg));
    rec[i] = r;
  }
}

int nvbx_mapper::grow_map(int64_t new_cap) {
  if (new_cap <= capacity) return NVBX_OK;
  if (new_cap > (1ll << 24)) new_cap = 1ll << 24;
  const int64_t old_cap = capacity;
  if (join_side()) return NVBX_E_DEVICE;
  if (fetch_counters()) return NVBX_E_DEVICE;
  { size_t free_b = 0, total_b = 0; NVBX_HIP(hipMemGetInfo(&free_b, &total_b));
    const size_t need = (size_t)new_cap * 4096 + ((size_t)new_cap - (size_t)old_cap) * (3 * 4096 + (d.freespace ? 8192 : 0) + 512) + (64u << 20) +
                        (feat_val ? (size_t)new_cap * (1024 * (size_t)feat_channels + 2048) : 0);
    if (free_b < need) { set_error("pool growth: not enough free HBM, the block pools stay at their size"); max_capacity = capacity; return NVBX_OK; } }
  std::vector<PoolArr> arrs;
  for (const PoolArr& a : pool_arrays(new_cap)) if (a.bytes_per_block && *a.p) arrs.push_back(a);
  const int64_t new_vcap = mesh_verts(new_cap), new_tcap = new_vcap * 2;
  const bool grow_mesh = new_vcap > mesh_vert_cap;
  const uint64_t tsz = hash_slots(new_cap);
  std::vector<void*> fresh;
  auto take = [&](size_t bytes) -> void* {
    void* q = nullptr;
    if (hipMalloc(&q, bytes) != hipSuccess) { (void)hipGetLastError(); return nullptr; }
    fresh.push_back(q); return q;
  };
  bool ok = true;
  uint32_t* saved = (uint32_t*)take((size_t)old_cap * sizeof(uint32_t)); ok = ok && saved;
  std::vector<void*> np(arrs.size(), nullptr);
  for (size_t i = 0; ok && i < arrs.size(); i++) { np[i] = take(arrs[i].bytes_per_block * (size_t)new_cap); ok = ok && np[i]; }
  int32_t* nl = ok ? (int32_t*)take((size_t)N_LISTS * NSH * (size_t)new_cap * 4) : nullptr; ok = ok && nl;
  float* nv = nullptr; float* nn = nullptr; uint8_t* nc = nullptr; int32_t* nt = nullptr;
  if (ok && grow_mesh) {
    nv = (float*)take(new_vcap * 12); nn = (float*)take(new_vcap * 12); nc = (uint8_t*)take(new_vcap * 4); nt = (int32_t*)take(new_tcap * 12);
    ok = nv && nn && nc && nt;
  }
  Entry* ntab = ok ? (Entry*)take(tsz * sizeof(Entry)) : nullptr; ok = ok && ntab;
  if (!ok) {
    for (void* q : fresh) (void)hipFree(q);
    set_error("pool growth: device allocation failed, the block pools stay at their size"); max_capacity = capacity;
    return NVBX_OK;
  }
  const unsigned rg = (unsigned)std::min<int64_t>((old_cap + 255) / 256, 2048);
  NVBX_LAUNCH(this, k_save_stamps, dim3(rg), dim3(256), d, saved);
  for (size_t i = 0; i < arrs.size(); i++) {
    const PoolArr& a = arrs[i];
    NVBX_HIP(hipMemcpyAsync(np[i], *a.p, a.bytes_per_block * (size_t)old_cap, hipMemcpyDeviceToDevice, stream));
    if (a.fill >= 0) NVBX_HIP(hipMemsetAsync((char*)np[i] + a.bytes_per_block * (size_t)old_cap, a.fill, a.bytes_per_block * (size_t)(new_cap - old_cap), stream));
  }
  for (int q = 0; q < N_LISTS * NSH; q++)
    NVBX_HIP(hipMemcpyAsync(nl + (size_t)q * new_cap, d.lists + (size_t)q * old_cap, (size_t)old_cap * 4, hipMemcpyDeviceToDevice, stream));
  if (grow_mesh) {
    const int64_t ovr = mesh_vert_cap / NSH, otr = mesh_tri_cap / NSH, nvr = new_vcap / NSH, ntr = new_tcap / NSH;
    if (mesh_epoch) {
      const int par = (int)((mesh_epoch + 1) & 1);
      for (int sh = 0; sh < NSH; sh++) {
        const int64_t uv = std::min<int64_t>((uint32_t)h_shc[((S_MESH_REC + par) * NSH + sh) * SH_STRIDE + 2], ovr);
        const int64_t ut = std::min<int64_t>((uint32_t)h_shc[((S_MESH_REC + par) * NSH + sh) * SH_STRIDE + 3], otr);
        if (uv) {
          NVBX_HIP(hipMemcpyAsync(nv + sh * nvr * 3, mesh_vert + sh * ovr * 3, (size_t)uv * 12, hipMemcpyDeviceToDevice, stream));
          NVBX_HIP(hipMemcpyAsync(nn + sh * nvr * 3, mesh_nrm + sh * ovr * 3, (size_t)uv * 12, hipMemcpyDeviceToDevice, stream));
          NVBX_HIP(hipMemcpyAsync(nc + sh * nvr * 4, mesh_col + sh * ovr * 4, (size_t)uv * 4, hipMemcpyDeviceToDevice, stream));
        }
        if (ut) NVBX_HIP(hipMemcpyAsync(nt + sh * ntr * 3, mesh_tri + sh * otr * 3, (size_t)ut * 12, hipMemcpyDeviceToDevice, stream));
      }
      const int32_t nraw = h_counters[C_MESH_OUT + 4 * par + 0];
      MeshRecord* new_rec = nullptr;
      for (size_t i = 0; i < arrs.size(); i++) if (arrs[i].p == reinterpret_cast<void**>(&mesh_rec)) new_rec = (MeshRecord*)np[i];
      if (nraw > 0) NVBX_LAUNCH(this, k_remap_mesh_records, dim3(64), dim3(256), new_rec, std::min<int32_t>(nraw, (int32_t)old_cap), ovr, nvr, otr, ntr);
    }
  }
  NVBX_HIP(hipMemsetAsync(ntab, 0xFF, tsz * sizeof(Entry), stream));
  NVBX_HIP(hipStreamSynchronize(stream));
  for (size_t i = 0; i < arrs.size(); i++) { (void)hipFree(*arrs[i].p); *arrs[i].p = np[i]; }
  (void)hipFree(d.lists); d.lists = nl;
  if (grow_mesh) {
    (void)hipFree(mesh_vert); (void)hipFree(mesh_nrm); (void)hipFree(mesh_col); (void)hipFree(mesh_tri);
    mesh_vert = nv; mesh_nrm = nn; mesh_col = nc; mesh_tri = nt; mesh_vert_cap = new_vcap; mesh_tri_cap = new_tcap;
  }
  (void)hipFree(d.table); d.table = ntab;
  d.mask = (uint32_t)(tsz - 1);
  { uint32_t lg = 0; while ((1ull << lg) < tsz) lg++; d.shift = 32u - lg; }
  d.capacity = (uint32_t)new_cap; capacity = new_cap;
  NVBX_LAUNCH(this, k_grow_free_stack, dim3(256), dim3(256), d, (uint32_t)old_cap, (uint32_t)new_cap);
  NVBX_LAUNCH(this, k_grow_commit, dim3(1), dim3(1), d, (int32_t)(new_cap - old_cap));
  NVBX_LAUNCH(this, k_reinsert, dim3(rg), dim3(256), d, saved, make_esdf_args().bz_out);
  NVBX_HIP(hipStreamSynchronize(stream));
  (void)hipFree(saved);
  if (view_export_cap > 0) view_export_cap = std::min<int64_t>(view_export_cap, capacity);
  growths++;
  return NVBX_OK;
}

int nvbx_mapper::maybe_grow(int64_t extra_blocks_wanted) {
  if (capacity >= max_capacity) return NVBX_OK;
  const int64_t free_seen = __atomic_load_n(&h_mirror[0], __ATOMIC_RELAXED);
  int64_t target = capacity;
  while (target < max_capacity && (free_seen + (target - capacity) - extra_blocks_wanted) * 2 < target) target *= 2;
  if (target > max_capacity) target = max_capacity;
  if (target == capacity) return NVBX_OK;
  return grow_map(target);
}
extern "C" int nvbx_mapper_set_max_capacity(nvbx_mapper* m, int64_t max_block_capacity) {
  if (!m) return NVBX_E_INVALID;
  m->max_capacity = std::max<int64_t>(m->capacity, std::min<int64_t>(max_block_capacity, 1ll << 24));
  return NVBX_OK;
}
extern "C" int64_t nvbx_mapper_capacity(nvbx_mapper* m) { return m ? m->capacity : NVBX_E_INVALID; }
```

### isaac_ros_nvblox_amd/csrc/mapper.hip

```cpp
#include <cstdlib>
#include <cstring>
#include "nvbx_mapper.h"
using namespace nvbx;

namespace nvbx {
static thread_local std::string g_err;
void set_error(const char* what, hipError_t e) {
  g_err = std::string(what) + ": " + hipGetErrorString(e);
}
void set_error(const char* what) { g_err = what; }
}

extern "C" const char* nvbx_last_error(void) { return nvbx::g_err.c_str(); }
__global__ void k_init_map(DMap m) {
  const uint32_t i = blockIdx.x * blockDim.x + threadIdx.x;
  if (i < m.capacity) { m.free_stack[i] = m.capacity - 1 - i; m.slot_flags[i] = 0; m.slot_stamp[i] = STAMP_NEVER; m.slot_consumed[i] = STAMP_NEVER; m.slot_cam[i] = STAMP_NEVER; }
  if (i < (uint32_t)(S_NUM * NSH * SH_STRIDE)) {
    const int id = (int)i / (NSH * SH_STRIDE), field = (int)i % SH_STRIDE;
    int32_t v = 0;
    if (id == S_ESDF_REC || id == S_ESDF_REC + 1) { if (field < 2) v = INT32_MAX; else if (field < 4) v = INT32_MIN; }
    m.shc[i] = v;
  }
  if (i < C_NUM) {
    int32_t v = 0;
    if (i == C_FREE_TOP) v = (int32_t)m.capacity;
    const int a = (int)i - C_ESDF_AABB;
    if (a >= 0 && a < 4) v = a < 2 ? INT32_MAX : INT32_MIN;
    const int w3 = (int)i - C_ESDF3_WIN;
    if (w3 >= 0 && w3 < 6) v = w3 < 3 ? INT32_MAX : INT32_MIN;
#ifdef NVBX_CHECK_INVARIANTS
    if (i >= C_INV_I1 && i <= C_INV_I3) v = m.counters[i];
#endif
    m.counters[i] = v;
  }
}

__global__ __launch_bounds__(512) void k_recompute_band(DMap m, float trunc) {
  const int32_t hw = m.counters[C_HIGH_WATER];
  for (int32_t slot = blockIdx.x; slot < hw; slot += gridDim.x) {
    if (!(m.slot_flags[slot] & F_TSDF)) continue;
    const float2 v = m.tsdf[(size_t)slot * 512 + threadIdx.x];
    publish_band(m.slot_flags, (uint32_t)slot, (int)threadIdx.x, in_band(v.x, v.y, trunc));
  }
}

std::vector<PoolArr> nvbx_mapper::pool_arrays(int64_t cap) {
  const size_t n = (size_t)cap, mv = (size_t)mesh_verts(cap);
  auto per_block = [n](auto** p, size_t bpb, int fill) { return PoolArr{reinterpret_cast<void**>(p), bpb, fill, bpb * n}; };
  auto other = [](auto** p, size_t bytes) { return PoolArr{reinterpret_cast<void**>(p), 0, -1, bytes}; };
  return {
      per_block(&d.free_stack, 4, -1), per_block(&d.slot_flags, 4, 0), per_block(&d.slot_index, 12, 0), per_block(&d.slot_entry, 4, 0), per_block(&d.slot_stamp, 4, 0xFF),
      per_block(&d.slot_consumed, 4, 0xFF), per_block(&d.slot_cam, 4, 0xFF), per_block(&d.tsdf, 4096, 0), per_block(&d.color, 4096, 0), per_block(&d.esdf, 4096, 0),
      per_block(&view_list, 16, -1),
      per_block(&export_idx, 12, -1), per_block(&cleared_idx, 12, -1), per_block(&d.site_bits, 8, 0), per_block(&d.obs_bits, 8, 0), per_block(&d.inside_bits, 8, 0),
      per_block(&mesh_rec, sizeof(MeshRecord), -1),
      PoolArr{reinterpret_cast<void**>(&d.freespace), 512 * 16, 0, 0},
      PoolArr{&feat_val, 1024 * (size_t)feat_channels, -1, 0}, PoolArr{reinterpret_cast<void**>(&feat_w), feat_channels ? (size_t)2048 : 0, -1, 0},
      other(&d.table, hash_slots(cap) * sizeof(Entry)), other(&d.lists, (size_t)N_LISTS * NSH * n * 4),
      other(&mesh_vert, mv * 12), other(&mesh_nrm, mv * 12), other(&mesh_col, mv * 4), other(&mesh_tri, mv * 2 * 12),
      other(&d.counters, C_NUM * 4), other(&d.shc, S_NUM * NSH * SH_STRIDE * 4), other(&export_count, 64),
      other(&table_spare, 0), other(&table_dirty, 0)};
}

static int alloc_all(nvbx_mapper* m) {
  const int64_t cap = m->capacity;
  const uint64_t tsz = nvbx_mapper::hash_slots(cap);
  DMap& d = m->d;
  d.capacity = (uint32_t)cap; d.mask = (uint32_t)(tsz - 1);
  { uint32_t lg = 0; while ((1ull << lg) < tsz) lg++; d.shift = 32u - lg; }
  for (const PoolArr& a : m->pool_arrays(cap)) if (a.bytes) NVBX_HIP(hipMalloc(a.p, a.bytes));
  m->mesh_vert_cap = nvbx_mapper::mesh_verts(cap); m->mesh_tri_cap = m->mesh_vert_cap * 2;
  NVBX_HIP(hipMemsetAsync(d.counters, 0, C_NUM * 4, m->stream));
  if (m->staging.ensure(m->stream, 8 << 20)) return NVBX_E_DEVICE;
  NVBX_HIP(hipHostMalloc(&m->h_counters, C_NUM * 4));
  NVBX_HIP(hipHostMalloc(&m->h_shc, S_NUM * NSH * SH_STRIDE * 4));
  NVBX_HIP(hipHostMalloc(&m->h_mirror, 64, hipHostMallocMapped));
  { void* dp = nullptr; NVBX_HIP(hipHostGetDevicePointer(&dp, m->h_mirror, 0)); d.host_mirror = (int32_t*)dp; }
  m->h_mirror[0] = (int32_t)cap; m->h_mirror[1] = 0; m->h_mirror[2] = 0; m->h_mirror[3] = 0; m->h_mirror[4] = 0; m->h_mirror[8] = 0;
  return NVBX_OK;
}

static int reset_map(nvbx_mapper* m) {
  DMap& d = m->d;
  const int64_t cap = m->capacity;
  NVBX_HIP(hipMemsetAsync(d.table, 0xFF, ((size_t)d.mask + 1) * sizeof(Entry), m->stream));
  NVBX_HIP(hipMemsetAsync(d.tsdf, 0, cap * 4096, m->stream));
  NVBX_HIP(hipMemsetAsync(d.color, 0, cap * 4096, m->stream));
  NVBX_HIP(hipMemsetAsync(d.esdf, 0, cap * 4096, m->stream));
  NVBX_HIP(hipMemsetAsync(d.site_bits, 0, cap * 8, m->stream));
  NVBX_HIP(hipMemsetAsync(d.obs_bits, 0, cap * 8, m->stream));
  NVBX_HIP(hipMemsetAsync(d.inside_bits, 0, cap * 8, m->stream));
  NVBX_HIP(hipMemsetAsync(m->export_count, 0, 64, m->stream));
  if (d.freespace) NVBX_HIP(hipMemsetAsync(d.freespace, 0, cap * 512 * 16, m->stream));
  const int64_t n = std::max<int64_t>(cap, std::max<int64_t>(C_NUM, S_NUM * NSH * SH_STRIDE));
  NVBX_LAUNCH(m, k_init_map, dim3((unsigned)((n + 255) / 256)), dim3(256), d);
  NVBX_HIP(hipGetLastError());
  m->reset_marking(); m->held.drop(*m); m->lidar_integrated = false;
  if (m->h_mirror) { m->h_mirror[0] = (int32_t)m->capacity; m->h_mirror[1] = 0; m->h_mirror[2] = 0; m->h_mirror[3] = 0; }
  m->frame_id = 0; m->esdf_epoch = 0; m->mesh_epoch = 0; m->last_view_frame = 0; m->last_camera_view_frame = 0; m->synth_rows = m->synth_cols = 0;
  return NVBX_OK;
}

int nvbx_mapper::wait_stream() {
  NVBX_HIP(hipStreamSynchronize(stream));
  return NVBX_OK;
}
int nvbx_mapper::fetch_counters() {
  if (join_side()) return NVBX_E_DEVICE;
  NVBX_HIP(hipMemcpyAsync(h_counters, d.counters, C_NUM * 4, hipMemcpyDeviceToHost, stream));
  NVBX_HIP(hipMemcpyAsync(h_shc, d.shc, S_NUM * NSH * SH_STRIDE * 4, hipMemcpyDeviceToHost, stream));
  return wait_stream();
}

float nvbx::log_odds(float p) { return logf(p / (1.0f - p)); }

Frame nvbx_mapper::make_frame(const float T[16], const nvbx_camera* cam, int32_t rows, int32_t cols, int32_t subsample) const {
  Frame f{};
  for (int i = 0; i < 3; i++) { for (int j = 0; j < 3; j++) f.R_LC[3 * i + j] = T[4 * i + j]; f.t_LC[i] = T[4 * i + 3]; }
  for (int i = 0; i < 3; i++) for (int j = 0; j < 3; j++) f.R_CL[3 * i + j] = f.R_LC[3 * j + i];
  for (int i = 0; i < 3; i++) {
    float s = f.R_CL[3 * i + 0] * f.t_LC[0];
    s = s + f.R_CL[3 * i + 1] * f.t_LC[1];
    s = s + f.R_CL[3 * i + 2] * f.t_LC[2];
    f.t_CL[i] = -s;
  }
  f.fu = cam->fu; f.fv = cam->fv; f.cu = cam->cu; f.cv = cam->cv; f.w = cam->width; f.h = cam->height;
  f.rows = rows; f.cols = cols;
  f.voxel_size = p.voxel_size; f.block_size = p.voxel_size * 8.0f;
  f.trunc = p.truncation_distance_vox * p.voxel_size;
  f.max_dist = p.max_integration_distance_m; f.max_weight = p.max_weight;
  f.weighting_mode = p.weighting_mode; f.interp_nearest = p.depth_interp_nearest;
  f.invalid_decay = p.invalid_depth_decay_factor;
  f.weighting_variant = p.tsdf_weighting_variant; f.skip_at_neg_trunc = p.tsdf_skip_at_negative_truncation; f.clamp_before_blend = p.tsdf_weight_clamp_before_blend;
  f.occlusion_thresh = p.color_occlusion_threshold_vox < 0.0f ? f.trunc : p.color_occlusion_threshold_vox * p.voxel_size;
  f.occupancy = p.projective_layer_type == 1 ? 1 : 0;
  f.lo_free = log_odds(p.free_region_occupancy_probability); f.lo_occupied = log_odds(p.occupied_region_occupancy_probability);
  f.lo_unobserved = log_odds(p.unobserved_region_occupancy_probability); f.occ_half_width = p.occupied_region_half_width_m;
  f.ws_type = p.workspace_bounds_type;
  for (int i = 0; i < 3; i++) { f.ws_min[i] = p.workspace_bounds_min_corner_m[i]; f.ws_max[i] = p.workspace_bounds_max_corner_m[i]; }
  f.subsample = subsample < 1 ? 1 : subsample;
  f.n_ray_rows = 0; f.n_ray_cols = 0;
  f.frame_id = frame_id;
  return f;
}

EsdfArgs nvbx_mapper::make_esdf_args() const {
  EsdfArgs c{};
  const float vs = p.voxel_size;
  c.kz_min = (int32_t)floorf(p.esdf_slice_min_height / vs);
  c.kz_max = (int32_t)floorf(p.esdf_slice_max_height / vs);
  c.kz_out = (int32_t)floorf(p.esdf_slice_height / vs);
  c.bz_lo = c.kz_min >> 3; c.bz_hi = c.kz_max >> 3; c.bz_out = c.kz_out >> 3; c.vz_out = c.kz_out & 7;
  const float r = p.esdf_max_distance_m / vs;
  c.max_sq = r * r;
  c.ri = (int32_t)floorf(r); if (c.ri > 63) c.ri = 63; if (c.ri < 1) c.ri = 1;
  c.rb = (c.ri + 7) / 8;
  c.site_dist_m = p.esdf_max_site_distance_vox * vs;
  c.min_weight = p.esdf_min_weight; c.voxel_size = vs; c.site_rule = p.projective_layer_type == 1 ? 2 : p.esdf_site_rule;
  c.epoch = esdf_epoch; c.mark_pass = mark_pass;
  c.rec = C_ESDF_UPD + 8 * (int)(esdf_epoch & 1); c.rec_next = C_ESDF_UPD + 8 * (int)((esdf_epoch + 1) & 1);
  c.self_reset = c.keep_list = pipelined_order ? 1 : 0;
  c.plane_on = (p.esdf_use_ground_plane && p.esdf_ground_plane[2] > 1e-3f && p.slice_height_thickness_m > 0.0f) ? 1 : 0;
  for (int i = 0; i < 4; i++) c.pl[i] = p.esdf_ground_plane[i];
  c.above = p.slice_height_above_plane_m; c.thick = p.slice_height_thickness_m;
  return c;
}

static const char* params_problem(const nvbx_mapper_params* p) {
  auto pos = [](float v) { return std::isfinite(v) && v > 0.0f; };
  if (!pos(p->voxel_size)) return "voxel_size must be > 0";
  if (!pos(p->max_integration_distance_m)) return "max_integration_distance_m must be > 0 (it bounds the view rays)";
  if (!pos(p->lidar_max_integration_distance_m)) return "lidar_max_integration_distance_m must be > 0 (it bounds the view rays)";
  if (p->max_integration_distance_m / (p->voxel_size * 8.0f) > 65536.0f || p->lidar_max_integration_distance_m / (p->voxel_size * 8.0f) > 65536.0f)
    return "integration distance exceeds 65536 blocks";
  if (!pos(p->truncation_distance_vox)) return "truncation_distance_vox must be > 0";
  if (!pos(p->max_weight)) return "max_weight must be > 0";
  if (p->projective_layer_type < 0 || p->projective_layer_type > 2) return "projective_layer_type must be 0 (TSDF), 1 (occupancy) or 2 (TSDF + freespace)";
  if (p->esdf_mode < 0 || p->esdf_mode > 1) return "esdf_mode must be 0 (2-D) or 1 (3-D)";
  if (p->tsdf_weighting_variant < 0 || p->tsdf_weighting_variant > 1 || p->esdf_propagation < 0 || p->esdf_propagation > 1 ||
      p->mesh_ambiguity_rule < 0 || p->mesh_ambiguity_rule > 2 || p->mesh_normal_rule < 0 || p->mesh_normal_rule > 1) return "open-choice switch out of range";
  if (p->esdf_propagation == 1 && p->esdf_mode == 1) return "esdf_propagation 1 (iterative) is defined for the 2-D slice only";
  if (p->sphere_tracing_max_steps < 0 || p->sphere_tracing_max_steps > (1 << 20)) return "sphere_tracing_max_steps out of range";
  if (p->projective_layer_type == 1) {
    auto prob = [](float v) { return v > 0.0f && v < 1.0f; };
    if (!prob(p->free_region_occupancy_probability) || !prob(p->occupied_region_occupancy_probability) || !prob(p->unobserved_region_occupancy_probability) ||
        !prob(p->free_region_decay_probability) || !prob(p->occupied_region_decay_probability)) return "occupancy probabilities must lie strictly between 0 and 1";
  }
  return nullptr;
}

extern "C" int nvbx_mapper_create(int device, void* hip_stream, const nvbx_mapper_params* params, int64_t block_capacity, nvbx_mapper** out) {
  if (!params || !out || (block_capacity != 0 && (block_capacity < 64 || block_capacity > (1ll << 24)))) {
    set_error("nvbx_mapper_create: invalid argument (null pointer, or block_capacity outside 64 .. 2^24 and not 0 = automatic)"); return NVBX_E_INVALID;
  }
  if (const char* why = params_problem(params)) { set_error(why); return NVBX_E_INVALID; }
  NVBX_HIP(hipSetDevice(device));
  if (block_capacity == 0) {
    size_t free_b = 0, total_b = 0; NVBX_HIP(hipMemGetInfo(&free_b, &total_b));
    int64_t want = (int64_t)((double)free_b * 0.04 / 12700.0), cap = 1ll << 16;
    while (cap * 2 <= want && cap < (1ll << 20)) cap *= 2;
    block_capacity = cap;
  }
  nvbx_mapper* m = new nvbx_mapper();
  m->device = device; m->p = *params; m->capacity = block_capacity;
  m->max_capacity = std::max<int64_t>(block_capacity, 1ll << 22);
  { const char* e = getenv("NVBX_MAX_BLOCKS"); if (e && atoll(e) > 0) m->max_capacity = std::max<int64_t>(block_capacity, std::min<int64_t>(atoll(e), 1ll << 24)); }
  if (hip_stream) { m->stream = (hipStream_t)hip_stream; m->own_stream = false; }
  else { hipError_t e = hipStreamCreateWithFlags(&m->stream, hipStreamNonBlocking); if (e != hipSuccess) { set_error("hipStreamCreate", e); delete m; return NVBX_E_DEVICE; } m->own_stream = true; }
  nvbx::frames_register_stream(device, m->stream); m->stream_registered = true;
  { const char* e = getenv("NVBX_SIDE_STREAM"); m->use_side = (e && e[0] == '1'); }
  m->defer_edt = nvbx_knob_switch(getenv("NVBX_DEFER_EDT")) != 0;
// ... 165 lines not shown
```

### isaac_ros_nvblox_amd/csrc/measure.hip

```cpp
#include "nvbx_view.h"

struct MeasRec { int32_t x, y, z, rank; float2 v[512]; };
static_assert(sizeof(MeasRec) == sizeof(nvbx_measurement_block), "measurement record layout");

template <typename Img>
__global__ __launch_bounds__(512) void k_measure_tsdf(DMap m, Frame f, Img depth, CameraSensor sensor, const int4* view_list, int32_t list_cap,
                                                      MeasRec* out, int32_t* out_count, int32_t out_cap) {
  int32_t n = m.counters[C_VIEW_COUNT + (f.frame_id & 3)];
  if (n > list_cap) n = list_cap;
  if (n > out_cap) n = out_cap;
  const int tid = threadIdx.x;
  if (blockIdx.x == 0 && tid == 0) *out_count = n;
  if (blockIdx.x == 0 && tid == 64) __hip_atomic_store(&m.host_mirror[0], m.counters[C_FREE_TOP], __ATOMIC_RELAXED, __HIP_MEMORY_SCOPE_SYSTEM);
  const int vx = tid >> 6, vy = (tid >> 3) & 7, vz = tid & 7;
  for (int32_t i = blockIdx.x; i < n; i += gridDim.x) {
    const int4 rec = view_list[i];
    float pc[3], org[3], off[3];
    sensor_block_origin(f, rec.y, rec.z, rec.w, org); sensor_voxel_offset(f, vx, vy, vz, off);
    pc[0] = org[0] + off[0]; pc[1] = org[1] + off[1]; pc[2] = org[2] + off[2];
    float ds = 0.0f, vd = 0.0f;
    const int got = sensor.sample(f, depth, pc, &ds, &vd);
    float2 o = make_float2(0.0f, -1.0f);
    if (got > 0) o = make_float2(ds, vd); else if (got < 0) o = make_float2(-1.0f, vd);
    MeasRec* r = out + i;
    if (tid == 0) { r->x = rec.y; r->y = rec.z; r->z = rec.w; r->rank = 0; }
    if (tid == 64 && slot_ok((uint32_t)rec.x)) m.slot_cam[rec.x] = (f.frame_id << 8) | 1u;
    r->v[tid] = o;
  }
}
__global__ void k_apply_index(DMap m, const MeasRec* all, const int32_t* counts, int32_t world, int64_t stride, int32_t owner_mod, int32_t owner_rank,
                              uint32_t frame_id, int32_t* postab, int4* view_list, int32_t list_cap) {
  int32_t* cnt = &m.counters[C_VIEW_COUNT + (frame_id & 3)];
  if (blockIdx.x == 0 && blockIdx.y == 0 && threadIdx.x == 0) m.counters[C_VIEW_COUNT + ((frame_id + 1) & 3)] = 0;
  const int32_t r = (int32_t)blockIdx.y;
  int64_t n = counts[r]; if (n > stride) n = stride;
  for (int64_t i = (int64_t)blockIdx.x * blockDim.x + threadIdx.x; i < n; i += (int64_t)gridDim.x * blockDim.x) {
    const MeasRec* rec = all + (size_t)r * stride + i;
    const int32_t x = rec->x, y = rec->y, z = rec->z;
    if (owner_mod > 1 && (int32_t)(index_hash(x, y, z) % (uint32_t)owner_mod) != owner_rank) continue;
    int4 out;
    int32_t h = -1;
    const bool first = mark_block(m, pack_key(x, y, z), frame_id, 1u << r, &out, &h);
    uint32_t slot;
    if (first) slot = (uint32_t)out.x;
    else { slot = SLOT_INVALID; if (h >= 0) { do { slot = ld_slot_acquire(&m.table[h]); } while (slot == SLOT_INVALID); } }
    if (!slot_ok(slot)) continue;
    postab[(size_t)slot * MAX_BATCH + r] = (int32_t)i + 1;
    if (first) { const int32_t p = atomicAdd(cnt, 1); if (p < list_cap) view_list[p] = out; }
  }
}
__global__ __launch_bounds__(512) void k_apply_fuse(DMap m, Frame f, const MeasRec* all, int64_t stride, int32_t world, int32_t* postab,
                                                    const int4* view_list, int32_t list_cap, int32_t mesh_list) {
  int32_t n = m.counters[C_VIEW_COUNT + (f.frame_id & 3)];
  if (n > list_cap) n = list_cap;
  const int tid = threadIdx.x;
  if (blockIdx.x == 0 && tid == 64) __hip_atomic_store(&m.host_mirror[0], m.counters[C_FREE_TOP], __ATOMIC_RELAXED, __HIP_MEMORY_SCOPE_SYSTEM);
  for (int32_t i = blockIdx.x; i < n; i += gridDim.x) {
    const uint32_t slot = (uint32_t)view_list[i].x;
    if (!slot_ok(slot)) continue;
    float2* vp = &m.tsdf[(size_t)slot * 512 + tid];
    float2 fin = *vp;
    uint32_t old = 0;
    if (tid == 0) old = atomicOr(&m.slot_flags[slot], F_TSDF | F_DIRTY_ESDF | F_DIRTY_MESH);
    bool touched = false;
    uint32_t cams = 0u;
    for (int r = 0; r < world; r++) {
      const int32_t p = postab[(size_t)slot * MAX_BATCH + r];
      if (!p) continue;
      cams |= 1u << r;
      const float2 mv = all[(size_t)r * stride + (p - 1)].v[tid];
      if (mv.y < 0.0f) continue;
      if (f.occupancy) { if (!(mv.x < 0.0f)) { fin = make_float2(occupancy_update(f, fin.x, mv.x, mv.y), 0.0f); touched = true; } }
      else if (mv.x < 0.0f) { if (f.invalid_decay >= 0.0f) { fin = make_float2(fin.x, fin.y * f.invalid_decay); touched = true; } }
      else if (tsdf_fuse(f, &fin, mv.x, mv.y)) touched = true;
    }
    if (touched) *vp = fin;
    if (tid == 64) m.slot_cam[slot] = (f.frame_id << 8) | cams;
    __syncthreads();
    if (tid < MAX_BATCH) postab[(size_t)slot * MAX_BATCH + tid] = 0;
    if (!f.occupancy) {
      const int any_band = __syncthreads_or(in_band(fin.x, fin.y, f.trunc) ? 1 : 0);
      if (tid == 0) { if (any_band) atomicOr(&m.slot_flags[slot], F_BAND); else atomicAnd(&m.slot_flags[slot], ~F_BAND); if (old & F_BAND_STALE) atomicAnd(&m.slot_flags[slot], ~F_BAND_STALE); }
    }
    if (tid == 0) {
      if (!(old & F_DIRTY_ESDF)) list_append(m, S_LIST_ESDF_DIRTY, (int32_t)slot);
      if (!(old & F_DIRTY_MESH)) list_append(m, mesh_list, (int32_t)slot);
    }
  }
}

extern "C" int nvbx_measure_depth(nvbx_mapper* m, const float* depth_dev, int32_t rows, int32_t cols, const float T_L_C[16], const nvbx_camera* camera,
                                  nvbx_measurement_block* out_dev, int32_t* count_dev, int64_t capacity_blocks) {
  if (!m || !depth_dev || !T_L_C || !camera || !out_dev || !count_dev || capacity_blocks <= 0 || !image_dims_ok(rows, cols)) { set_error("nvbx_measure_depth: invalid argument"); return NVBX_E_INVALID; }
  if (!nvbx_camera_matches(camera, rows, cols)) { set_error("nvbx_measure_depth: camera width/height must equal the image's cols/rows, focal lengths > 0"); return NVBX_E_INVALID; }
  if (!nvbx_pose_in_range(T_L_C, m->p.voxel_size * 8.0f, m->p.max_integration_distance_m + 2.0f * m->p.truncation_distance_vox * m->p.voxel_size)) {
    set_error("nvbx_measure_depth: T_L_C is not finite or lies outside the addressable block range"); return NVBX_E_INVALID; }
  if (m->p.projective_layer_type == 2 || (m->p.do_depth_preprocessing && m->p.depth_preprocessing_num_dilations > 0)) {
    set_error("nvbx_measure_depth: mappers with depth preprocessing (dilation) or a freespace layer integrate per frame -- use nvbx_integrate_depth"); return NVBX_E_INVALID; }
  NVBX_HIP(hipSetDevice(m->device));
  if (m->join_side()) return NVBX_E_DEVICE;
  { const int rc = m->maybe_grow(); if (rc) return rc; }
  { const int rc = next_frame_id(m); if (rc) return rc; }
  FrameSet<DepthF32, 1> fs{}; fs.n = 1; fs.img[0] = DepthF32{depth_dev};
  fs.f[0] = m->make_frame(T_L_C, camera, rows, cols, m->p.raycast_subsampling_factor);
  size_ray_grid(fs);
  const Frame& f = fs.f[0];
  launch_mark_view_camera(m, fs);
  NVBX_LAUNCH(m, (k_measure_tsdf<DepthF32>), dim3((unsigned)std::min<int64_t>(m->capacity, 1024)), dim3(512), m->d, f, DepthF32{depth_dev}, CameraSensor{},
              (const int4*)m->view_list, (int32_t)m->capacity, reinterpret_cast<MeasRec*>(out_dev), count_dev, (int32_t)std::min<int64_t>(capacity_blocks, INT32_MAX));
  NVBX_HIP(hipGetLastError());
  m->last_view_frame = m->frame_id; m->last_camera_view_frame = m->frame_id; m->last_camera_view_mask = 1u; m->last_view_batch = 1;
  return m->mark_main();
}

extern "C" int nvbx_apply_measurements(nvbx_mapper* m, const nvbx_measurement_block* gathered_dev, const int32_t* counts_dev, int32_t world, int64_t stride_blocks,
                                       int32_t owner_mod, int32_t owner_rank) {
  if (!m || !gathered_dev || !counts_dev || world < 1 || world > MAX_BATCH || stride_blocks <= 0 || owner_mod < 0 || (owner_mod > 1 && (owner_rank < 0 || owner_rank >= owner_mod))) {
    set_error("nvbx_apply_measurements: invalid argument (1 <= world <= 8)"); return NVBX_E_INVALID; }
  if (m->p.projective_layer_type == 2) { set_error("nvbx_apply_measurements: mappers with a freespace layer integrate per frame (time stamps)"); return NVBX_E_INVALID; }
  NVBX_HIP(hipSetDevice(m->device));
  if (m->join_side()) return NVBX_E_DEVICE;
  { const int rc = m->maybe_grow(); if (rc) return rc; }
  bool grew = false;
  if (m->apply_postab.ensure(m->stream, (size_t)m->capacity * MAX_BATCH * 4, &grew)) return NVBX_E_DEVICE;
  if (grew) NVBX_HIP(hipMemsetAsync(m->apply_postab.p, 0, m->apply_postab.bytes, m->stream));
  if (m->begin_dirtying()) return NVBX_E_DEVICE;
  { const int rc = next_frame_id(m); if (rc) return rc; }
  nvbx_camera none{1.f, 1.f, 0.f, 0.f, 1, 1};
  float I[16] = {1, 0, 0, 0, 0, 1, 0, 0, 0, 0, 1, 0, 0, 0, 0, 1};
  const Frame f = m->make_frame(I, &none, 1, 1, 1);
  const MeasRec* all = reinterpret_cast<const MeasRec*>(gathered_dev);
  NVBX_LAUNCH(m, k_apply_index, dim3(64, (unsigned)world), dim3(256), m->d, all, counts_dev, world, stride_blocks, owner_mod, owner_rank, m->frame_id, m->apply_postab.as<int32_t>(),
              (int4*)m->view_list, (int32_t)m->capacity);
  NVBX_LAUNCH(m, k_apply_fuse, dim3((unsigned)std::min<int64_t>(m->capacity, 1024)), dim3(512), m->d, f, all, stride_blocks, world, m->apply_postab.as<int32_t>(),
              (const int4*)m->view_list, (int32_t)m->capacity, m->mesh_list_live());
  NVBX_HIP(hipGetLastError());
  m->last_view_frame = m->frame_id; m->last_camera_view_frame = m->frame_id; m->last_camera_view_mask = 1u << (world - 1); m->last_view_batch = world;
  return m->mark_main();
}
```

### isaac_ros_nvblox_amd/csrc/nvbx_esdf_mark.h

```cpp
#pragma once
#include "nvbx_mapper.h"

namespace nvbx {

__device__ inline void esdf_mark_entry(const DMap& m, const EsdfArgs& a, uint32_t tslot, int srec, int sh, bool from_dirty_list = false) {
  const int lane = threadIdx.x & 63;
  const int vx = lane & 7, vy = lane >> 3;
  const uint32_t tflags = m.slot_flags[tslot];
  const int32_t bx = m.slot_index[3 * tslot], by = m.slot_index[3 * tslot + 1], bz = m.slot_index[3 * tslot + 2];
  int32_t kz_lo = a.kz_min, kz_hi = a.kz_max, bz_lo = a.bz_lo, bz_hi = a.bz_hi;
  if (a.plane_on) {
    const float bs = a.voxel_size * 8.0f;
    const float hl = esdf_plane_height(a.pl, voxel_center(bx, vx, bs, a.voxel_size), voxel_center(by, vy, bs, a.voxel_size));
    kz_lo = (int32_t)floorf((hl + a.above) / a.voxel_size); kz_hi = (int32_t)floorf(((hl + a.above) + a.thick) / a.voxel_size);
    const float x0 = (float)bx * bs, x1 = (float)(bx + 1) * bs, y0 = (float)by * bs, y1 = (float)(by + 1) * bs;
    const float h00 = esdf_plane_height(a.pl, x0, y0), h10 = esdf_plane_height(a.pl, x1, y0), h01 = esdf_plane_height(a.pl, x0, y1), h11 = esdf_plane_height(a.pl, x1, y1);
    const float hmin = fminf(fminf(h00, h10), fminf(h01, h11)), hmax = fmaxf(fmaxf(h00, h10), fmaxf(h01, h11));
    bz_lo = floor_div8((int32_t)floorf((hmin + a.above) / a.voxel_size)); bz_hi = floor_div8((int32_t)floorf(((hmax + a.above) + a.thick) / a.voxel_size));
    if (bz_hi - bz_lo > 61) bz_hi = bz_lo + 61;
  }
  const int nz = bz_hi - bz_lo + 1;
  if (from_dirty_list && !(tflags & F_DIRTY_ESDF)) return;
  NVBX_INV_TSDF_READER(m);
  NVBX_INV_COUNT(m, C_INV_I4, lane == 0 && from_dirty_list && !(tflags & (F_TSDF | F_ESDF)));
  NVBX_TV(0, 3, wall_clock64());
  if (lane == 0) { atomicAnd(&m.slot_flags[tslot], ~F_DIRTY_ESDF); m.slot_consumed[tslot] = a.mark_pass; }
  if (!(tflags & F_ESDF_REMARK) && (bz < bz_lo || bz > bz_hi)) return;
  const int32_t qz = lane == 0 ? a.bz_out : bz_lo + lane - 1;
  const bool probing = lane <= nz;
  const u64 qkey = pack_key(bx, by, qz);
  const uint32_t qh = probing ? table_pos(m, bx, by, qz) : 0u;
  const uint4 qe = ld_entry(m, qh);
  uint32_t qslot = probing ? resolve_any(m, qkey, qh, qe) : SLOT_NONE;
  uint32_t eslot = __shfl(qslot, 0);
  NVBX_TV(0, 4, wall_clock64());
  const bool early = (tflags & F_TSDF) && slot_ok(eslot);
  int first = 0;
  if (early && lane == 0) first = atomicExch(&m.slot_stamp[eslot], a.mark_pass) != a.mark_pass;
  const uint32_t ts0 = __shfl(qslot, 1), ts1 = __shfl(qslot, nz > 1 ? 2 : 1);
  const float4* c0 = reinterpret_cast<const float4*>(&m.tsdf[(size_t)(slot_ok(ts0) ? ts0 : 0) * 512 + 64 * vx + 8 * vy]);
  const float4* c1 = reinterpret_cast<const float4*>(&m.tsdf[(size_t)(slot_ok(ts1) ? ts1 : 0) * 512 + 64 * vx + 8 * vy]);
  const float4 p00 = c0[0], p01 = c0[1], p02 = c0[2], p03 = c0[3], p10 = c1[0], p11 = c1[1], p12 = c1[2], p13 = c1[3];
  const bool e_exists = slot_ok(eslot) && (m.slot_flags[slot_ok(eslot) ? eslot : 0] & (F_ESDF | F_ESDF_PENDING));
  if (!(tflags & F_TSDF) && !(e_exists && (tflags & F_ESDF_REMARK))) return;
  if (lane == 0) {
    if (!slot_ok(eslot)) {
      bool is_new;
      const int32_t h = hash_insert(m, bx, by, a.bz_out, F_ESDF_PENDING, &is_new);
      if (h >= 0) { do { eslot = ld_slot_acquire(&m.table[h]); } while (eslot == SLOT_INVALID); }
    }
    if (slot_ok(eslot)) {
      if (!e_exists) atomicOr(&m.slot_flags[eslot], F_ESDF_PENDING);
      if (!early) first = atomicExch(&m.slot_stamp[eslot], a.mark_pass) != a.mark_pass;
    }
  }
  int observed = 0, inside = 0, site = 0;
  auto column = [&](int32_t bzz, const float4& v0, const float4& v1, const float4& v2, const float4& v3) {
    const float dz[8] = {v0.x, v0.z, v1.x, v1.z, v2.x, v2.z, v3.x, v3.z}, wz[8] = {v0.y, v0.w, v1.y, v1.w, v2.y, v2.w, v3.y, v3.w};
#pragma unroll
    for (int z = 0; z < 8; z++) {
      const int32_t kz = bzz * 8 + z;
      if (kz < kz_lo || kz > kz_hi) continue;
      if (a.site_rule == 2) {
        if (dz[z] != 0.0f) observed = 1;
        if (dz[z] > 0.0f) { inside = 1; site = 1; }
      } else if (wz[z] >= a.min_weight) {
        observed = 1;
        const int in = dz[z] <= 0.0f;
        if (in) inside = 1;
        if ((a.site_rule == 1 || in) && fabsf(dz[z]) <= a.site_dist_m) site = 1;
      }
    }
  };
  if (slot_ok(ts0)) column(bz_lo, p00, p01, p02, p03);
  if (nz > 1 && slot_ok(ts1)) column(bz_lo + 1, p10, p11, p12, p13);
  for (int32_t q = 2; q < nz; ++q) {
    const uint32_t ts = __shfl(qslot, q + 1);
    if (!slot_ok(ts)) continue;
    const float4* col = reinterpret_cast<const float4*>(&m.tsdf[(size_t)ts * 512 + 64 * vx + 8 * vy]);
    column(bz_lo + q, col[0], col[1], col[2], col[3]);
  }
  eslot = __shfl(eslot, 0); first = __shfl(first, 0);
  NVBX_TV(0, 5, wall_clock64());
  if (!first || !slot_ok(eslot)) return;
  if (lane == 0) {
    atomicMin(shc_at(m, srec, sh, 0), bx); atomicMin(shc_at(m, srec, sh, 1), by);
    atomicMax(shc_at(m, srec, sh, 2), bx); atomicMax(shc_at(m, srec, sh, 3), by);
    atomicAdd(shc_at(m, srec, sh, 4), 1);
  }
  const u64 sbits = __ballot(site != 0), obits = __ballot(observed != 0), ibits = __ballot(inside != 0);
  if (lane == 0) { m.site_bits[eslot] = sbits; m.obs_bits[eslot] = obits; m.inside_bits[eslot] = ibits; }
}

__device__ inline void esdf_mark_worker(const DMap& m, const EsdfArgs& a, int wg, int nwg) {
  const int per = nwg >> 3;
  const int sh_l = wg & (NSH - 1), j0 = wg >> 3;
  if (per < 1 || j0 >= per) return;
  const int32_t* base = &m.lists[((size_t)S_LIST_ESDF_DIRTY * NSH + sh_l) * m.capacity];
  const int32_t first = base[j0];
  int32_t cnt = *shc_at(m, S_LIST_ESDF_DIRTY, sh_l, 0);
  if (cnt > (int32_t)m.capacity) cnt = (int32_t)m.capacity;
  const int srec = S_ESDF_REC + (int)(a.epoch & 1), sh = my_shard();
  int n_done = 0;
  for (int32_t j = j0; j < cnt; j += per) { esdf_mark_entry(m, a, (uint32_t)(j == j0 ? first : base[j]), srec, sh, true); n_done++;  if (n_done == 1) NVBX_TV(0, 1, wall_clock64()); }
  NVBX_TV(0, 6, n_done); NVBX_TV(0, 2, wall_clock64());
}

__device__ inline void esdf_mark_pass_done(const DMap& m, const EsdfArgs& a, int n_workers, int worker = -1) {
  if (!a.self_reset) return;
  if ((threadIdx.x & 63) == 0) {
    const int w = worker >= 0 ? worker : (int)blockIdx.x, sh = w & (NSH - 1);
    const int32_t in_shard = (n_workers - sh + NSH - 1) / NSH;
    const int32_t arrived = atomicAdd(shc_at(m, S_MARK_DONE, sh, 0), 1);
    if (arrived == in_shard - 1) {
      __hip_atomic_store(shc_at(m, S_MARK_DONE, sh, 0), 0, __ATOMIC_RELAXED, __HIP_MEMORY_SCOPE_AGENT);
      const int32_t shards_with_workers = n_workers < NSH ? n_workers : NSH;
      const int32_t done = atomicAdd(&m.counters[C_MARK_DONE], 1);
      if (done == shards_with_workers - 1) {
#pragma unroll
        for (int s = 0; s < NSH; s++) __hip_atomic_store(shc_at(m, S_LIST_ESDF_DIRTY, s, 0), 0, __ATOMIC_RELAXED, __HIP_MEMORY_SCOPE_AGENT);
        __hip_atomic_store(&m.counters[C_MARK_DONE], 0, __ATOMIC_RELAXED, __HIP_MEMORY_SCOPE_AGENT);
      }
    }
  }
}

struct ImportArgs { const int32_t* g; int32_t world, self_rank; int64_t max_count; int32_t n_wg; };
__device__ inline void esdf_import_mark_worker(const DMap& m, const EsdfArgs& a, const ImportArgs& imp, int w) {
  const int srec = S_ESDF_REC + (int)(a.epoch & 1), sh = my_shard();
  const int n_peers = imp.self_rank >= 0 && imp.self_rank < imp.world ? imp.world - 1 : imp.world;
  const int per_rank = max(1, imp.n_wg / max(1, n_peers));
  const int peer = w / per_rank, wi = w - peer * per_rank;
  if (peer >= n_peers) return;
  const int32_t r = (n_peers < imp.world && peer >= imp.self_rank) ? peer + 1 : peer;
  const int32_t* base = imp.g + (size_t)r * (size_t)(imp.max_count + 1) * 3;
  int64_t n = base[0]; if (n > imp.max_count) n = imp.max_count;
  const int32_t* idx = base + 3;
  for (int64_t i = wi; i < n; i += per_rank) {
    const uint32_t s = find_slot(m, idx[3 * i], idx[3 * i + 1], idx[3 * i + 2], F_TSDF);
    if (!slot_ok(s)) continue;
    esdf_mark_entry(m, a, s, srec, sh);
  }
}

__device__ inline void esdf_import_dirty_worker(const DMap& m, const ImportArgs& imp, int64_t t, int64_t nt) {
  for (int32_t r = 0; r < imp.world; r++) {
    if (r == imp.self_rank) continue;
    const int32_t* base = imp.g + (size_t)r * (size_t)(imp.max_count + 1) * 3;
    int64_t n = base[0]; if (n > imp.max_count) n = imp.max_count;
    const int32_t* idx = base + 3;
    for (int64_t i = t; i < n; i += nt) {
      const uint32_t s = find_slot(m, idx[3 * i], idx[3 * i + 1], idx[3 * i + 2], F_TSDF);
      if (!slot_ok(s)) continue;
      const uint32_t old = atomicOr(&m.slot_flags[s], F_DIRTY_ESDF);
      if (!(old & F_DIRTY_ESDF)) list_append(m, S_LIST_ESDF_DIRTY, (int32_t)s);
    }
  }
}

}
```

### isaac_ros_nvblox_amd/csrc/nvbx_internal.h

```cpp
#pragma once
#include <hip/hip_runtime.h>
#include <stdint.h>
#include "nvbx_arith.h"

namespace nvbx {

typedef unsigned long long u64;

constexpr u64 KEY_EMPTY = ~0ull;
constexpr uint32_t SLOT_INVALID = 0xFFFFFFFFu;
constexpr uint32_t STAMP_NEVER = 0xFFFFFFFFu;
constexpr uint32_t SLOT_NONE = 0xFFFFFFFEu;
__host__ __device__ inline bool slot_ok(uint32_t s) { return s < SLOT_NONE; }

constexpr uint32_t F_TSDF = 1u, F_COLOR = 2u, F_ESDF = 4u, F_MESH = 8u;
constexpr uint32_t F_FREESPACE = 32u;
constexpr uint32_t F_FEATURE = 64u;
constexpr uint32_t F_DIRTY_ESDF = 1u << 8, F_DIRTY_MESH = 1u << 9;
constexpr uint32_t F_ESDF_PENDING = 1u << 10;
constexpr uint32_t F_ESDF_REMARK = 1u << 11;
constexpr uint32_t F_BAND_SHIFT = 12, F_BAND = 0xFFu << F_BAND_SHIFT;
constexpr uint32_t F_BAND_STALE = 1u << 20;
__host__ __device__ inline bool in_band(float d, float w, float trunc) { return w > 1e-4f && fabsf(d) < trunc; }
#ifdef __HIPCC__
__device__ inline void publish_band(uint32_t* slot_flags, uint32_t slot, int tid, bool pred) {
  const unsigned long long b = __ballot(pred);
  if ((tid & 63) == 0) {
    const uint32_t bit = 1u << (F_BAND_SHIFT + (tid >> 6));
    if (b) atomicOr(&slot_flags[slot], bit); else atomicAnd(&slot_flags[slot], ~bit);
    if (tid == 0) atomicAnd(&slot_flags[slot], ~F_BAND_STALE);
  }
}
#endif

struct Entry { u64 key; uint32_t slot; uint32_t stamp; };
constexpr uint32_t STAMP_FRAME_MAX = 0xFFFFF0u;
constexpr int MAX_BATCH = 8;
constexpr int MAX_IMAGE_DIM = 32768;
inline bool image_dims_ok(int64_t rows, int64_t cols) { return rows > 0 && cols > 0 && rows <= MAX_IMAGE_DIM && cols <= MAX_IMAGE_DIM; }
__host__ __device__ inline uint32_t stamp_frame(uint32_t s) { return s >> 8; }

enum {
  C_FREE_TOP = 0,
  C_HIGH_WATER = 1,
  C_OVERFLOW = 2,
  C_VIEW_COUNT = 4,
  C_ESDF3_WIN = 8,
  C_ESDF_UPD = 16,
  C_ESDF_AABB = 32,
  C_MESH_OUT = 36,
  C_LIVE = 44,
  C_TMP = 45,
  C_CLEARED = 46,
  C_MARK_DONE = 47,
  C_CAND_COUNT = 48,
  C_INV_WRITERS = 50,
  C_INV_I1 = 51,
  C_INV_I4 = 52,
  C_INV_I3 = 53,
  C_NUM = 56
};

constexpr int NSH = 8;
constexpr int SH_STRIDE = 16;
enum {
  S_LIST_ESDF_DIRTY = 0,
  S_LIST_MESH_DIRTY = 1,
  S_LIST_COLOR = 3,
  S_ESDF_REC = 4,
  S_MESH_REC = 6,
  S_LIDAR_SPARSE = 9,
  S_MARK_DONE = 8,
  S_NUM = 10
};
constexpr int N_LISTS = 4;

struct DMap {
  Entry* table; uint32_t mask; uint32_t shift;
  uint32_t capacity;
  uint32_t* free_stack;
  int32_t* counters;
  uint32_t* slot_flags;
  int32_t* slot_index;
  uint32_t* slot_entry;
  uint32_t* slot_stamp;
  uint32_t* slot_cam;
  uint32_t* slot_consumed;
  float2* tsdf;
  uint2* color;
  uint2* esdf;
  int4* freespace;
  u64* site_bits;
  u64* obs_bits;
  u64* inside_bits;
  int32_t* shc;
  int32_t* lists;
  int32_t* host_mirror;
};

struct FrameCore {
  float R_CL[9], t_CL[3];
  float R_LC[9], t_LC[3];
  float fu, fv, cu, cv; int32_t w, h;
  int32_t rows, cols;
  float voxel_size, block_size, trunc, max_dist, max_weight;
  float occlusion_thresh;
  int32_t subsample;
};
struct Frame : FrameCore {
  int32_t weighting_mode, interp_nearest;
  int32_t weighting_variant, skip_at_neg_trunc, clamp_before_blend;
  float invalid_decay;
  int32_t occupancy; float lo_free, lo_occupied, lo_unobserved, occ_half_width;
  int32_t ws_type; float ws_min[3], ws_max[3];
  int32_t n_ray_rows, n_ray_cols;
  uint32_t frame_id;
  uint32_t cam_bit;
};

__host__ __device__ inline u64 pack_key(int32_t x, int32_t y, int32_t z) {
  const u64 B = 1ull << 20;
  return (((u64)(int64_t)x + B) & 0x1FFFFFull) | ((((u64)(int64_t)y + B) & 0x1FFFFFull) << 21) |
         ((((u64)(int64_t)z + B) & 0x1FFFFFull) << 42);
}
__host__ __device__ inline void unpack_key(u64 key, int32_t* x, int32_t* y, int32_t* z) {
  *x = (int32_t)(key & 0x1FFFFFull) - (1 << 20);
  *y = (int32_t)((key >> 21) & 0x1FFFFFull) - (1 << 20);
  *z = (int32_t)((key >> 42) & 0x1FFFFFull) - (1 << 20);
}
__host__ __device__ inline uint32_t index_hash(int32_t x, int32_t y, int32_t z) {
  return (uint32_t)x + (uint32_t)y * 17191u + (uint32_t)z * (17191u * 17191u);
}

__host__ __device__ inline uint32_t table_pos(const DMap& m, int32_t x, int32_t y, int32_t z) {
  return (index_hash(x, y, z) * 2654435761u) >> m.shift;
}

#ifdef __HIPCC__
#if defined(NVBX_WG_TIMES) && defined(NVBX_WGT_HERE)
__device__ unsigned long long* g_wgt = nullptr;
#define NVBX_TV(k, i, v) do { if ((threadIdx.x & 63) == 0 && (threadIdx.x >> 6) == 0 && g_wgt && blockIdx.x < 8192) g_wgt[((size_t)(k) * 8192 + blockIdx.x) * 8 + (i)] = (unsigned long long)(v); } while (0)
#else
#define NVBX_TV(k, i, v) do { (void)sizeof(v); } while (0)
#endif
#ifdef NVBX_CHECK_INVARIANTS
#define NVBX_INV_WRITER_BEGIN(m) do { __syncthreads(); if (threadIdx.x == 0) atomicAdd(&(m).counters[C_INV_WRITERS], 1); } while (0)
#define NVBX_INV_WRITER_END(m) do { __syncthreads(); if (threadIdx.x == 0) atomicSub(&(m).counters[C_INV_WRITERS], 1); } while (0)
#define NVBX_INV_TSDF_READER(m) do { if ((threadIdx.x & 63) == 0 && __hip_atomic_load(&(m).counters[C_INV_WRITERS], __ATOMIC_RELAXED, __HIP_MEMORY_SCOPE_AGENT) != 0) atomicAdd(&(m).counters[C_INV_I1], 1); } while (0)
#define NVBX_INV_COUNT(m, idx, cond) do { if (cond) atomicAdd(&(m).counters[idx], 1); } while (0)
#else
#define NVBX_INV_WRITER_BEGIN(m) do { } while (0)
#define NVBX_INV_WRITER_END(m) do { } while (0)
#define NVBX_INV_TSDF_READER(m) do { } while (0)
#define NVBX_INV_COUNT(m, idx, cond) do { } while (0)
#endif
__device__ inline int32_t* shc_at(const DMap& m, int id, int shard, int field) { return &m.shc[(id * NSH + shard) * SH_STRIDE + field]; }
__device__ inline int my_shard() { return (int)(blockIdx.x & (NSH - 1)); }

__device__ inline void list_append(const DMap& m, int list, int32_t v) {
  const int sh = my_shard();
  const int32_t p = atomicAdd(shc_at(m, list, sh, 0), 1);
  if (p < (int32_t)m.capacity) m.lists[((size_t)list * NSH + sh) * m.capacity + p] = v;
}
struct ListView { int32_t pre[NSH + 1]; };
__device__ inline int32_t list_open(const DMap& m, int list, ListView* v) {
  int32_t c[NSH];
#pragma unroll
  for (int s = 0; s < NSH; s++) c[s] = *shc_at(m, list, s, 0);
  v->pre[0] = 0;
#pragma unroll
  for (int s = 0; s < NSH; s++) v->pre[s + 1] = v->pre[s] + min(c[s], (int32_t)m.capacity);
  return v->pre[NSH];
}
__device__ inline int32_t list_at(const DMap& m, int list, const ListView& v, int32_t i) {
  int s = 0; int32_t base = 0;
#pragma unroll
  for (int q = 1; q < NSH; q++) if (i >= v.pre[q]) { s = q; base = v.pre[q]; }
  return m.lists[((size_t)list * NSH + s) * m.capacity + (i - base)];
}
__device__ inline void list_reset(const DMap& m, int list) {
#pragma unroll
  for (int s = 0; s < NSH; s++) *shc_at(m, list, s, 0) = 0;
}

#include "nvbx_numbering.h"
static_assert(NVBX_N_XCD == NSH, "one shard per XCD");

__device__ inline int32_t floor_div8(int32_t v) { return v >> 3; }
__device__ inline int32_t mod8(int32_t v) { return v & 7; }

__device__ inline uint32_t ld_slot_acquire(const Entry* e) {
  return __hip_atomic_load(&e->slot, __ATOMIC_RELAXED, __HIP_MEMORY_SCOPE_AGENT);
}

__device__ inline int32_t hash_find(const DMap& m, int32_t x, int32_t y, int32_t z) {
  const u64 key = pack_key(x, y, z);
  uint32_t h = table_pos(m, x, y, z);
  for (uint32_t probe = 0; probe <= m.mask; ++probe) {
    const u64 k = m.table[h].key;
    if (k == key) return (int32_t)h;
    if (k == KEY_EMPTY) return -1;
    h = (h + 1) & m.mask;
  }
  return -1;
}
__device__ inline uint32_t find_slot(const DMap& m, int32_t x, int32_t y, int32_t z, uint32_t layer) {
  const int32_t h = hash_find(m, x, y, z);
  if (h < 0) return SLOT_NONE;
  const uint32_t s = m.table[h].slot;
  if (!slot_ok(s)) return SLOT_NONE;
  return (m.slot_flags[s] & layer) ? s : SLOT_NONE;
}

__device__ inline uint4 ld_entry(const DMap& m, uint32_t h) { return *reinterpret_cast<const uint4*>(&m.table[h]); }
__device__ inline uint4 ld_pair(const uint2* p) {
  typedef unsigned int u4a8 __attribute__((ext_vector_type(4), aligned(8)));
  const u4a8 v = *reinterpret_cast<const u4a8*>(p);
  return make_uint4(v.x, v.y, v.z, v.w);
}
__device__ inline uint32_t resolve_any(const DMap& m, u64 key, uint32_t h, uint4 e) {
  for (uint32_t probe = 0; probe <= m.mask; ++probe) {
    const u64 k = ((u64)e.y << 32) | (u64)e.x;
    if (k == key) return slot_ok(e.z) ? e.z : SLOT_NONE;
    if (k == KEY_EMPTY) return SLOT_NONE;
    h = (h + 1) & m.mask;
    e = ld_entry(m, h);
  }
  return SLOT_NONE;
}
__device__ inline uint32_t any_slot(const DMap& m, int32_t x, int32_t y, int32_t z) {
  const uint32_t h = table_pos(m, x, y, z);
  return resolve_any(m, pack_key(x, y, z), h, ld_entry(m, h));
}

__device__ inline int32_t hash_insert(const DMap& m, int32_t x, int32_t y, int32_t z, uint32_t layer_flags, bool* is_new) {
  const u64 key = pack_key(x, y, z);
  uint32_t h = table_pos(m, x, y, z);
  *is_new = false;
  for (uint32_t probe = 0; probe <= m.mask; ++probe) {
    u64 k = m.table[h].key;
    if (k == KEY_EMPTY) {
      k = atomicCAS(&m.table[h].key, KEY_EMPTY, key);
      if (k == KEY_EMPTY) {
        *is_new = true;
        const int32_t top = atomicSub(&m.counters[C_FREE_TOP], 1);
        uint32_t slot = SLOT_NONE;
        if (top > 0) {
          slot = m.free_stack[top - 1];
          m.slot_index[3 * slot] = x; m.slot_index[3 * slot + 1] = y; m.slot_index[3 * slot + 2] = z;
          m.slot_entry[slot] = h;
          atomicOr(&m.slot_flags[slot], layer_flags);
          atomicMax(&m.counters[C_HIGH_WATER], (int32_t)slot + 1);
        } else {
          atomicAdd(&m.counters[C_FREE_TOP], 1);
          atomicExch(&m.counters[C_OVERFLOW], 1);
        }
        __hip_atomic_store(&m.table[h].slot, slot, __ATOMIC_RELAXED, __HIP_MEMORY_SCOPE_AGENT);
        return (int32_t)h;
      }
    }
    if (k == key) return (int32_t)h;
    h = (h + 1) & m.mask;
  }
  atomicExch(&m.counters[C_OVERFLOW], 1);
  return -1;
}

__device__ inline void apply_rt(const float* R, const float* t, float x, float y, float z, float* o) {
#pragma unroll
  for (int i = 0; i < 3; i++) {
    float s = R[3 * i + 0] * x;
    s = s + R[3 * i + 1] * y;
    s = s + R[3 * i + 2] * z;
    o[i] = s + t[i];
  }
}
__device__ inline void rotate(const float* R, float x, float y, float z, float* o) {
#pragma unroll
  for (int i = 0; i < 3; i++) {
    float s = R[3 * i + 0] * x;
    s = s + R[3 * i + 1] * y;
    s = s + R[3 * i + 2] * z;
    o[i] = s;
  }
}
__device__ inline void sensor_block_origin(const Frame& f, int32_t bx, int32_t by, int32_t bz, float* o) {
  apply_rt(f.R_CL, f.t_CL, (float)bx * f.block_size, (float)by * f.block_size, (float)bz * f.block_size, o);
}
__device__ inline void sensor_voxel_offset(const Frame& f, int vx, int vy, int vz, float* o) {
  const float h = f.voxel_size * 0.5f;
  rotate(f.R_CL, (float)vx * f.voxel_size + h, (float)vy * f.voxel_size + h, (float)vz * f.voxel_size + h, o);
}
__device__ inline float voxel_center(int32_t bi, int32_t vi, float bs, float vs) {
  return ((float)bi * bs + (float)vi * vs) + vs * 0.5f;
}
__device__ inline bool cam_project(const FrameCore& f, const float* p, float* u, float* v) {
  if (p[2] <= 0.0f) return false;
  *u = f.fu * NVBX_DIV(p[0], p[2]) + f.cu;
  *v = f.fv * NVBX_DIV(p[1], p[2]) + f.cv;
  return *u >= 0.0f && *v >= 0.0f && *u <= (float)f.w && *v <= (float)f.h;
}

__device__ inline int32_t pix(int r, int c, int cols) { return __mul24(r, cols) + c; }
struct DepthF32 { const float* p; __device__ float operator()(int32_t i) const { return p[i]; } };
struct DepthU16mm {
  const uint16_t* p; __device__ float operator()(int32_t i) const { return (float)p[i] * (1.0f / 1000.0f); } };

template <typename Img>
__device__ inline int interp_depth(const Img& img, int rows, int cols, float u, float v, int nearest, float* out) {
  if (nearest) {
    const int c = (int)floorf(u), r = (int)floorf(v);
    if (c < 0 || r < 0 || c >= cols || r >= rows) return 0;
    const float d = img(pix(r, c, cols));
    if (!(d > 0.0f)) return -1;
    *out = d; return 1;
  }
  const float uc = u - 0.5f, vc = v - 0.5f;
  const float fx = floorf(uc), fy = floorf(vc);
  const int x0 = (int)fx, y0 = (int)fy;
  if (x0 < 0 || y0 < 0 || x0 + 1 > cols - 1 || y0 + 1 > rows - 1) return 0;
  const float ax = uc - fx, ay = vc - fy;
  const int32_t i00 = pix(y0, x0, cols);
  const float f00 = img(i00), f10 = img(i00 + 1), f01 = img(i00 + cols), f11 = img(i00 + cols + 1);
  __builtin_amdgcn_sched_barrier(0);
  if (!(f00 > 0.0f) || !(f10 > 0.0f) || !(f01 > 0.0f) || !(f11 > 0.0f)) return -1;
  const float top = (1.0f - ax) * f00 + ax * f10;
  const float bot = (1.0f - ax) * f01 + ax * f11;
  *out = (1.0f - ay) * top + ay * bot;
  return 1;
}

// ... 79 lines not shown
```

### isaac_ros_nvblox_amd/csrc/tsdf.hip

```cpp
#define NVBX_WGT_HERE
#include "nvbx_view.h"

#ifdef NVBX_WG_TIMES
constexpr int WGT_MAX_WG = 8192, WGT_SLOTS = 8;
static unsigned long long* g_wgt_host = nullptr;
extern "C" int nvbx_debug_wg_times(unsigned long long* out_host, int64_t n_words) {
  const size_t total = (size_t)2 * WGT_MAX_WG * WGT_SLOTS;
  if (!g_wgt_host) {
    if (hipMalloc(&g_wgt_host, total * 8) != hipSuccess) return -1;
    (void)hipMemset(g_wgt_host, 0, total * 8);
    (void)hipMemcpyToSymbol(HIP_SYMBOL(g_wgt), &g_wgt_host, sizeof(g_wgt_host));
    (void)wgt_bind_lidar(g_wgt_host);
  }
  if (out_host) {
    (void)hipDeviceSynchronize();
    (void)hipMemcpy(out_host, g_wgt_host, std::min<size_t>(total, (size_t)n_words) * 8, hipMemcpyDeviceToHost);
    (void)hipMemset(g_wgt_host, 0, total * 8);
  }
  return (int)WGT_MAX_WG;
}
#endif

template <typename Img> struct MarkViewArgs { DMap m; FrameSet<Img, 1> fs; int4* view_list; int32_t list_cap, reset_esdf_dirty, n_edt_wg; EsdfArgs ea; TraceRiderT<1> tr; int32_t n_tiles, n_wg; };
template <typename Img>
__global__ __launch_bounds__(CameraSensor::kThreads) void k_mark_view_pair(MarkViewArgs<Img> a, MarkViewArgs<Img> b) {
  extern __shared__ __align__(16) unsigned char smem[];
  const int32_t g = (int32_t)blockIdx.x, at = a.n_tiles, bt = b.n_tiles, ar = a.n_wg - a.n_tiles;
  bool is_a; int32_t wg;
  if (g < at) { is_a = true; wg = g; }
  else if (g < at + bt) { is_a = false; wg = g - at; }
  else if (g < at + bt + ar) { is_a = true; wg = at + (g - at - bt); }
  else { is_a = false; wg = bt + (g - at - bt - ar); }
  if (is_a) mark_view_body<Img, CameraSensor, 1>(a.m, a.fs, CameraSensor{}, a.view_list, a.list_cap, a.reset_esdf_dirty, a.n_edt_wg, a.ea, a.tr, wg, smem);
  else mark_view_body<Img, CameraSensor, 1>(b.m, b.fs, CameraSensor{}, b.view_list, b.list_cap, b.reset_esdf_dirty, b.n_edt_wg, b.ea, b.tr, wg, smem);
}
static_assert(2 * sizeof(MarkViewArgs<DepthF32>) <= 4096, "k_mark_view_pair: kernel arguments");

template <typename T> __device__ inline T in_vgpr(T x) { asm volatile("" : "+v"(x)); return x; }

template <typename Img, typename Sensor, int NB, bool Plain>
__device__ inline void integrate_tsdf_worker(const DMap& m, const FrameSet<Img, NB>& fs, const Sensor& sensor, const int4* view_list, int32_t list_cap,
                                             int32_t mesh_list, int32_t* view_export, int32_t view_export_cap, int32_t spec_lanes, const uint8_t* view_class,
                                             const int32_t wgi, const int32_t n_wg, const int32_t* dense_list = nullptr) {
  const Frame& f0 = fs.f[0];
  const int tid = threadIdx.x, lane = tid & 63;
  const int32_t wgr = dense_list ? wgi : xcd_chunked(wgi, n_wg);
  int32_t mine = wgr + lane * n_wg;
  int4 rec = (!dense_list && lane < spec_lanes && mine < list_cap) ? view_list[mine] : make_int4((int32_t)SLOT_NONE, 0, 0, 0);
  int32_t n = m.counters[C_VIEW_COUNT + (f0.frame_id & 3)];
  if (n > list_cap) n = list_cap;
  if (wgi == 0 && tid == 192) __hip_atomic_store(&m.host_mirror[2], n, __ATOMIC_RELAXED, __HIP_MEMORY_SCOPE_SYSTEM);
  int32_t dpre[NSH + 1];
  auto dense_at = [&](int32_t k) -> int32_t {
    int sh = 0; int32_t base = 0;
#pragma unroll
    for (int q = 1; q < NSH; q++) if (k >= dpre[q]) { sh = q; base = dpre[q]; }
    return dense_list[(size_t)sh * list_cap + (k - base)];
  };
  if (dense_list) {
    int32_t c[NSH];
#pragma unroll
    for (int q = 0; q < NSH; q++) c[q] = *shc_at(m, S_LIDAR_SPARSE, q, 1);
    dpre[0] = 0;
#pragma unroll
    for (int q = 0; q < NSH; q++) dpre[q + 1] = dpre[q] + min(c[q], list_cap);
    n = dpre[NSH];
    if (mine < n) rec = view_list[dense_at(mine)];
  } else {
    if (lane >= spec_lanes && mine < n) rec = view_list[mine];
    if (view_class && mine < n && view_class[mine]) rec.x = (int32_t)SLOT_NONE;
  }
  if (view_export && wgi == 0 && tid == 0) { view_export[0] = min(n, view_export_cap); view_export[1] = 0; view_export[2] = 0; }
  if (wgi == 0 && tid == 64) __hip_atomic_store(&m.host_mirror[0], m.counters[C_FREE_TOP], __ATOMIC_RELAXED, __HIP_MEMORY_SCOPE_SYSTEM);
  if (wgi == 0 && tid == 128) __hip_atomic_store(&m.host_mirror[1], m.counters[C_HIGH_WATER], __ATOMIC_RELAXED, __HIP_MEMORY_SCOPE_SYSTEM);
  const int vx = tid >> 6, vy = (tid >> 3) & 7, vz = tid & 7;
  float off0[3] = {0.0f, 0.0f, 0.0f};
  if (NB == 1) sensor_voxel_offset(f0, vx, vy, vz, off0);
  Frame fl = f0; Img img0 = fs.img[0];
  if (Sensor::kLongRays && NB == 1) { fl.cols = in_vgpr(f0.cols); fl.rows = in_vgpr(f0.rows); img0.p = in_vgpr(fs.img[0].p); }
  for (int32_t i0 = wgr; i0 < n; i0 += 64 * n_wg) {
    if (i0 != wgr) {
      mine = i0 + lane * n_wg;
      if (dense_list) rec = mine < n ? view_list[dense_at(mine)] : make_int4((int32_t)SLOT_NONE, 0, 0, 0);
      else {
        rec = mine < n ? view_list[mine] : make_int4((int32_t)SLOT_NONE, 0, 0, 0);
        if (view_class && mine < n && view_class[mine]) rec.x = (int32_t)SLOT_NONE;
      }
    }
    if (view_export && tid < 64 && mine < n && mine < view_export_cap) { int32_t* e = view_export + 3 * (1 + (int64_t)mine); e[0] = rec.y; e[1] = rec.z; e[2] = rec.w; }
    float org[3] = {0.0f, 0.0f, 0.0f};
    if (NB == 1) sensor_block_origin(f0, rec.y, rec.z, rec.w, org);
#pragma unroll 1
    for (int32_t j = 0; j < 64 && i0 + j * n_wg < n; j++) {
      const uint32_t slot = (uint32_t)__builtin_amdgcn_readlane(rec.x, j);
      if (!slot_ok(slot)) continue;
      float2* vp = &m.tsdf[(size_t)slot * 512 + tid];
      const float2 cur_c = *vp;
      uint32_t cams = 1u;
      if (NB > 1) cams = __builtin_amdgcn_readfirstlane(m.table[m.slot_entry[slot]].stamp & 0xFFu);
      uint32_t old = 0;
      if (tid == 0) old = atomicOr(&m.slot_flags[slot], F_TSDF | F_DIRTY_ESDF | F_DIRTY_MESH | ((Sensor::kLongRays && (Plain || !f0.occupancy)) ? F_BAND_STALE : 0u));
      if (!Sensor::kLongRays && tid == 64) m.slot_cam[slot] = (f0.frame_id << 8) | cams;
      const int32_t bx = __builtin_amdgcn_readlane(rec.y, j), by = __builtin_amdgcn_readlane(rec.z, j), bz = __builtin_amdgcn_readlane(rec.w, j);
      float2 fin = cur_c;
      bool touched = false;
#pragma unroll 1
      for (int c = 0; c < (NB > 1 ? fs.n : 1); c++) {
        if (NB > 1 && !((cams >> c) & 1u)) continue;
        const Frame& f = (Sensor::kLongRays && NB == 1) ? fl : fs.f[c];
        const Img& img = (Sensor::kLongRays && NB == 1) ? img0 : fs.img[c];
        float pc[3];
        if (NB == 1) {
          pc[0] = __int_as_float(__builtin_amdgcn_readlane(__float_as_int(org[0]), j)) + off0[0];
          pc[1] = __int_as_float(__builtin_amdgcn_readlane(__float_as_int(org[1]), j)) + off0[1];
          pc[2] = __int_as_float(__builtin_amdgcn_readlane(__float_as_int(org[2]), j)) + off0[2];
        } else {
          float o[3], d[3];
          sensor_block_origin(f, bx, by, bz, o); sensor_voxel_offset(f, vx, vy, vz, d);
          pc[0] = o[0] + d[0]; pc[1] = o[1] + d[1]; pc[2] = o[2] + d[2];
        }
        float ds = 0.0f, vd = 0.0f;
        const int got = sensor.sample(f, img, pc, &ds, &vd);
        if (Plain) {
          if (got > 0 && tsdf_fuse_plain(f, &fin, ds, vd)) touched = true;
        } else if (f.occupancy) {
          if (got > 0) { fin = make_float2(occupancy_update(f, fin.x, ds, vd), 0.0f); touched = true; }
        } else {
          if (got < 0 && f.invalid_decay >= 0.0f) { fin = make_float2(fin.x, fin.y * f.invalid_decay); touched = true; }
          if (got > 0 && tsdf_fuse(f, &fin, ds, vd)) touched = true;
        }
      }
      if (touched) *vp = fin;
      if (Plain || !f0.occupancy) {
        if (!Sensor::kLongRays) {
          const int any_band = __syncthreads_or(in_band(fin.x, fin.y, f0.trunc) ? 1 : 0);
          if (tid == 0) { if (any_band) atomicOr(&m.slot_flags[slot], F_BAND); else atomicAnd(&m.slot_flags[slot], ~F_BAND); if (old & F_BAND_STALE) atomicAnd(&m.slot_flags[slot], ~F_BAND_STALE); }
        }
      }
      if (tid == 0) {
        if (!(old & F_DIRTY_ESDF)) list_append(m, S_LIST_ESDF_DIRTY, (int32_t)slot);
        if (!(old & F_DIRTY_MESH)) list_append(m, mesh_list, (int32_t)slot);
      }
    }
  }
}
template <typename Img, typename Sensor, int NB, bool Plain>
__global__ __launch_bounds__(512) __attribute__((amdgpu_waves_per_eu(8, 8))) void k_integrate_tsdf(DMap m, FrameSet<Img, NB> fs, Sensor sensor, const int4* view_list, int32_t list_cap,
                                                        int32_t mesh_list, int32_t* view_export, int32_t view_export_cap, int32_t spec_lanes, const uint8_t* view_class,
                                                        const int32_t* dense_list) {
  NVBX_INV_WRITER_BEGIN(m);
  integrate_tsdf_worker<Img, Sensor, NB, Plain>(m, fs, sensor, view_list, list_cap, mesh_list, view_export, view_export_cap, spec_lanes, view_class, (int32_t)blockIdx.x, (int32_t)gridDim.x, dense_list);
  NVBX_INV_WRITER_END(m);
}

template <typename Img, typename Pix, int NB, bool Plain>
__device__ __forceinline__ void integrate_tsdf_color_body(const DMap& m, const FrameSet<Img, NB>& fs, const CameraSensor& sensor, const int4* view_list, int32_t list_cap,
                                                          int32_t mesh_list, int32_t* view_export, int32_t view_export_cap, int32_t spec_lanes, int32_t n_tsdf_wg,
                                                          const FrameSetC<Pix, NB>& fsc, const float* synth, int32_t srows, int32_t scols, const int4* cand, int32_t cand_cnt_idx,
                                                          int32_t n_edt_wg, const EsdfArgs& ea, const ImportArgs& imp, const int32_t b, const int32_t n_wg_total, unsigned char* smem) {
  NVBX_T(1, 0);
  if (b < n_edt_wg) { esdf_edt_worker<512>(m, ea, (int)b, n_edt_wg, reinterpret_cast<EdtShared*>(smem)); NVBX_T(1, 1); NVBX_T(1, 7); return; }
  if (b < n_edt_wg + n_tsdf_wg) {
    NVBX_INV_WRITER_BEGIN(m);
    integrate_tsdf_worker<Img, CameraSensor, NB, Plain>(m, fs, sensor, view_list, list_cap, mesh_list, view_export, view_export_cap, spec_lanes, nullptr, b - n_edt_wg, n_tsdf_wg);
    NVBX_INV_WRITER_END(m);
    NVBX_T(1, 2); NVBX_T(1, 7);
    return;
  }
  const int32_t n_color_wg = n_wg_total - n_edt_wg - n_tsdf_wg - imp.n_wg;
  if (b >= n_edt_wg + n_tsdf_wg + n_color_wg) { esdf_import_dirty_worker(m, imp, (int64_t)(b - n_edt_wg - n_tsdf_wg - n_color_wg) * 512 + threadIdx.x, (int64_t)imp.n_wg * 512); return; }
  color_integrate_list_worker<Pix, NB>(m, fsc, synth, srows, scols, mesh_list, cand, cand_cnt_idx, b - n_edt_wg - n_tsdf_wg, n_color_wg);
  NVBX_T(1, 3); NVBX_T(1, 7);
}
template <typename Img, typename Pix, int NB, bool Plain>
__global__ __launch_bounds__(512) NVBX_FUSED_ATTR void k_integrate_tsdf_color(DMap m, FrameSet<Img, NB> fs, CameraSensor sensor, const int4* view_list, int32_t list_cap,
                                                              int32_t mesh_list, int32_t* view_export, int32_t view_export_cap, int32_t spec_lanes, int32_t n_tsdf_wg,
                                                              FrameSetC<Pix, NB> fsc, const float* synth, int32_t srows, int32_t scols, const int4* cand, int32_t cand_cnt_idx,
                                                              int32_t n_edt_wg, EsdfArgs ea, ImportArgs imp) {
  __shared__ __align__(16) unsigned char smem[sizeof(EdtShared)];
  integrate_tsdf_color_body<Img, Pix, NB, Plain>(m, fs, sensor, view_list, list_cap, mesh_list, view_export, view_export_cap, spec_lanes, n_tsdf_wg, fsc, synth, srows, scols, cand, cand_cnt_idx,
                                                 n_edt_wg, ea, imp, (int32_t)blockIdx.x, (int32_t)gridDim.x, smem);
}
template <typename Img, typename Pix> struct FusedArgs {
  DMap m; FrameSet<Img, 1> fs; const int4* view_list; int32_t list_cap, mesh_list; int32_t* view_export; int32_t view_export_cap, spec_lanes, n_tsdf_wg;
  FrameSetC<Pix, 1> fsc; const float* synth; int32_t srows, scols; const int4* cand; int32_t cand_cnt_idx, n_edt_wg; EsdfArgs ea; ImportArgs imp; int32_t n_wg; };
template <typename Img, typename Pix>
__global__ __launch_bounds__(512) void k_integrate_tsdf_color_pair(FusedArgs<Img, Pix> a, FusedArgs<Img, Pix> b) {
  __shared__ __align__(16) unsigned char smem[sizeof(EdtShared)];
  const int32_t g = (int32_t)blockIdx.x;
  const bool is_a = g < a.n_wg; const int32_t wg = is_a ? g : g - a.n_wg;
  if (is_a)
    integrate_tsdf_color_body<Img, Pix, 1, false>(a.m, a.fs, CameraSensor{}, a.view_list, a.list_cap, a.mesh_list, a.view_export, a.view_export_cap, a.spec_lanes, a.n_tsdf_wg, a.fsc, a.synth, a.srows,
                                                  a.scols, a.cand, a.cand_cnt_idx, a.n_edt_wg, a.ea, a.imp, wg, a.n_wg, smem);
  else
    integrate_tsdf_color_body<Img, Pix, 1, false>(b.m, b.fs, CameraSensor{}, b.view_list, b.list_cap, b.mesh_list, b.view_export, b.view_export_cap, b.spec_lanes, b.n_tsdf_wg, b.fsc, b.synth, b.srows,
                                                  b.scols, b.cand, b.cand_cnt_idx, b.n_edt_wg, b.ea, b.imp, wg, b.n_wg, smem);
}
static_assert(2 * sizeof(FusedArgs<DepthF32, PixRgb8>) <= 4096, "k_integrate_tsdf_color_pair: kernel arguments");
static_assert(sizeof(DMap) + sizeof(FrameSet<DepthF32, MAX_BATCH>) + sizeof(FrameSetC<PixRgb8, MAX_BATCH>) + sizeof(EsdfArgs) + sizeof(ImportArgs) + 160 <= 4096, "k_integrate_tsdf_color<.., MAX_BATCH>: kernel arguments");

static bool fused_colour_applies(const nvbx_mapper* m) {
  static const int fuse_on = nvbx_knob_switch(getenv("NVBX_FUSE_COLC"));
  return fuse_on && m->p.projective_layer_type != 1 && m->p.esdf_mode == 0 && m->p.esdf_propagation == 0 && !m->lidar_integrated && m->capacity <= (1ll << 24);
}
template <int NB> struct DepthSteps {
  int tiles = 0, edt_wg = 0; EsdfArgs ea{}; TraceRiderT<NB> tr{};
  bool plain = true, has_color = false, pipelined = false, fused = false;
  HeldColorFrames<NB> col{};
  int grid = 8; int32_t spec_lanes = 1;
  int32_t n_edt = 0; EsdfArgs ea_edt{}; const int4* cand = nullptr; int32_t cand_idx = 0; int cgrid = 0; ImportArgs imp{};
  nvbx_mapper::ModeScope pipelined_order;
};
template <typename Img, typename Sensor, int NB>
static int depth_step_before_mark_view(nvbx_mapper* m, FrameSet<Img, NB>& fs, DepthSteps<NB>& st) {
  size_ray_grid(fs);
  const Frame& f = fs.f[0];
  st.tiles = mark_view_tile_wgs<Sensor>(f) * fs.n;
  st.edt_wg = 0; st.ea = m->held.edt_args;
  if (m->held.edt_pending) {
    if (Sensor::kRiders) { st.edt_wg = 256; m->held.edt_pending = false; }
    else if (m->flush_edt()) return NVBX_E_DEVICE;
  }
  st.tr = TraceRiderT<NB>{};
  st.plain = true;
  for (int c = 0; c < fs.n; c++) st.plain = st.plain && frame_is_plain(fs.f[c]);
  st.has_color = m->held.color_pending.on;
  st.pipelined = Sensor::kRiders && (st.has_color ? m->held.color_pending.carried_by(NB) : m->held.esdf_update_pending);
  st.fused = false;
  if (st.pipelined) {
    st.fused = st.has_color ? fused_colour_applies(m)
                            : true;
    if (st.fused && st.edt_wg) { m->held.edt_pending = true; st.edt_wg = 0; if (m->flush_edt()) return NVBX_E_DEVICE; }
    st.pipelined_order.enter(m->pipelined_order);
    if (st.has_color) { const int rc = m->pending_color_trace_rider<NB>(&st.tr); if (rc) return rc; }
    static const int tiles_first_env = nvbx_knob_mark_tiles_first(getenv("NVBX_MARK_TILES_FIRST"));
    const bool tiles_first = tiles_first_env >= 0 ? tiles_first_env != 0 : NB == 1;
    if (tiles_first) st.tr.n_tile_wg = st.tiles;
    if (st.fused && !st.has_color) m->pending_marking_args(&st.tr.n_mark_wg, &st.ea, NB == 1);
    if (st.fused && st.has_color) {
      if (m->color_cand.ensure(m->stream, (size_t)m->capacity * 2 * sizeof(int4))) return NVBX_E_DEVICE;
      const int64_t hw_seen = std::max<int64_t>(1, __atomic_load_n(&m->h_mirror[1], __ATOMIC_RELAXED));
      st.tr.n_scan_wg = (int32_t)std::min<int64_t>(256, 8 * ((hw_seen + hw_seen / 4 + 64 + 2047) / 2048));
      st.tr.cand = m->color_cand.as<int4>() + (size_t)m->cand_parity * (size_t)m->capacity;
      st.tr.cand_cnt_idx = C_CAND_COUNT + m->cand_parity; st.tr.cand_reset_idx = C_CAND_COUNT + (1 - m->cand_parity);
      m->cand_parity ^= 1;
      m->pending_marking_args(&st.tr.n_mark_wg, &st.ea, NB == 1);
    }
  }
  st.tr.fence_report = m->next_fence_report();
  return NVBX_OK;
}
static int64_t with_grid_margin(int64_t n) {
  struct Margin { int pct, blocks; Margin() { nvbx_knob_grid_margin(getenv("NVBX_GRID_MARGIN"), &pct, &blocks); } };
  static const Margin mg;
  return n + n * mg.pct / 100 + mg.blocks;
}
template <typename Sensor, int NB>
static int depth_step_between(nvbx_mapper* m, DepthSteps<NB>& st) {
  if (st.pipelined) {
    if (!st.fused) m->premark_consumed = false;
    int rc = NVBX_OK;
    if (st.fused) { if (st.has_color) rc = m->pending_color_fused_args<NB>(&st.col); }
    else rc = m->launch_pending_color_after_trace();
    if (rc == NVBX_OK && m->held.esdf_update_pending) { m->held.esdf_update_pending = false; rc = nvbx_update_esdf(m); }
    st.pipelined_order.leave();
    if (rc) return rc;
  }
  m->premark_consumed = false; m->dirty_since_mark = true;
  static const int grid_cap_env = nvbx_knob_integ_grid(getenv("NVBX_INTEG_GRID"));
  const int grid_cap = grid_cap_env > 0 ? grid_cap_env : (NB > 1 ? 512 : 1024);
  const int64_t n_hint = std::max<int64_t>(0, __atomic_load_n(&m->h_mirror[2], __ATOMIC_RELAXED));
  const int64_t n_want = with_grid_margin(n_hint);
  const int64_t want = n_hint == 0 ? (int64_t)grid_cap : ((n_want + 7) / 8) * 8;
  st.grid = (int)std::max<int64_t>(8, std::min<int64_t>(std::min<int64_t>(m->capacity, grid_cap), want));
  st.spec_lanes = (int32_t)std::min<int64_t>(64, (n_want + st.grid - 1) / st.grid);
  return NVBX_OK;
}
template <int NB>
static void depth_step_fused_riders(nvbx_mapper* m, DepthSteps<NB>& st) {
  st.n_edt = 0; st.ea_edt = m->held.edt_args;
  static const int edt_riders = nvbx_knob_edt_riders(getenv("NVBX_EDT_RIDERS"));
  if (m->held.edt_pending) { st.n_edt = edt_riders; m->held.edt_pending = false; }
  st.cand = st.tr.cand;
  st.cand_idx = st.tr.cand_cnt_idx;
  const int64_t c_hint = std::max<int64_t>(0, __atomic_load_n(&m->h_mirror[3], __ATOMIC_RELAXED));
  static const int color_cap = nvbx_knob_color_grid(getenv("NVBX_COLOR_GRID"));
  st.cgrid = !st.has_color ? 0 : (int)std::max<int64_t>(8, std::min<int64_t>(std::min<int64_t>(m->capacity, color_cap), c_hint == 0 ? (int64_t)st.grid : ((with_grid_margin(c_hint) + 7) / 8) * 8));
  st.imp = ImportArgs{};
  if (m->held.import_pending) {
    st.imp.g = m->held.import_ptr; st.imp.world = m->held.import_world; st.imp.self_rank = m->held.import_rank; st.imp.max_count = m->held.import_max; st.imp.n_wg = 8;
    m->held.import_pending = false;
  }
}
// ... 214 lines not shown
```

Before: 47660 frames/s.

## Store block coordinates alongside slots in ESDF dirty list to hoist hash probes

```diff
diff --git a/isaac_ros_nvblox_amd/csrc/esdf.hip b/isaac_ros_nvblox_amd/csrc/esdf.hip
--- a/isaac_ros_nvblox_amd/csrc/esdf.hip
+++ b/isaac_ros_nvblox_amd/csrc/esdf.hip
@@ -379,7 +379,7 @@
   int32_t n = list_open(m, S_LIST_ESDF_DIRTY, &lv); if (n > cap) n = cap;
   if (blockIdx.x == 0 && threadIdx.x == 0) *out_count = n;
   for (int32_t i = blockIdx.x * blockDim.x + threadIdx.x; i < n; i += gridDim.x * blockDim.x) {
-    const int32_t s = list_at(m, S_LIST_ESDF_DIRTY, lv, i);
+    const int32_t s = esdf_dirty_at(m, lv, i).x;
     out_idx[3 * i] = m.slot_index[3 * s]; out_idx[3 * i + 1] = m.slot_index[3 * s + 1]; out_idx[3 * i + 2] = m.slot_index[3 * s + 2];
   }
 }
@@ -401,7 +401,7 @@
     const uint32_t s = find_slot(m, idx[3 * i], idx[3 * i + 1], idx[3 * i + 2], F_TSDF);
     if (!slot_ok(s)) continue;
     const uint32_t old = atomicOr(&m.slot_flags[s], F_DIRTY_ESDF);
-    if (!(old & F_DIRTY_ESDF)) list_append(m, S_LIST_ESDF_DIRTY, (int32_t)s);
+    if (!(old & F_DIRTY_ESDF)) esdf_dirty_append(m, (int32_t)s, idx[3 * i], idx[3 * i + 1], idx[3 * i + 2]);
   }
 }
 extern "C" int nvbx_mark_esdf_dirty(nvbx_mapper* m, const int32_t* indices_dev, const int32_t* count_dev, int64_t max_count) {
@@ -423,7 +423,7 @@
     const uint32_t s = find_slot(m, idx[3 * i], idx[3 * i + 1], idx[3 * i + 2], F_TSDF);
     if (!slot_ok(s)) continue;
     const uint32_t old = atomicOr(&m.slot_flags[s], F_DIRTY_ESDF);
-    if (!(old & F_DIRTY_ESDF)) list_append(m, S_LIST_ESDF_DIRTY, (int32_t)s);
+    if (!(old & F_DIRTY_ESDF)) esdf_dirty_append(m, (int32_t)s, idx[3 * i], idx[3 * i + 1], idx[3 * i + 2]);
   }
 }
 __global__ __launch_bounds__(64) void k_import_mark_gathered(DMap m, EsdfArgs a, const int32_t* g, int32_t self_rank, int64_t max_count) {
@@ -436,7 +436,7 @@
   for (int64_t i = blockIdx.x; i < n; i += gridDim.x) {
     const uint32_t s = find_slot(m, idx[3 * i], idx[3 * i + 1], idx[3 * i + 2], F_TSDF);
     if (!slot_ok(s)) continue;
-    esdf_mark_entry(m, a, s, srec, sh);
+    esdf_mark_entry(m, a, s, idx[3 * i], idx[3 * i + 1], idx[3 * i + 2], srec, sh);
   }
 }
 extern "C" int nvbx_mark_esdf_dirty_gathered(nvbx_mapper* m, const int32_t* gathered_dev, int32_t world, int32_t self_rank, int64_t max_count) {
@@ -469,7 +469,7 @@
       m.slot_consumed[s] = STAMP_NEVER;
       if (flags & (F_TSDF | F_COLOR | F_ESDF | F_MESH | F_ESDF_PENDING)) {
         const uint32_t old = atomicOr(&m.slot_flags[s], F_DIRTY_ESDF);
-        if (!(old & F_DIRTY_ESDF)) list_append(m, S_LIST_ESDF_DIRTY, s);
+        if (!(old & F_DIRTY_ESDF)) esdf_dirty_append_slot(m, s);
       }
     }
     if (stamp_unres) {
diff --git a/isaac_ros_nvblox_amd/csrc/esdf3d.hip b/isaac_ros_nvblox_amd/csrc/esdf3d.hip
--- a/isaac_ros_nvblox_amd/csrc/esdf3d.hip
+++ b/isaac_ros_nvblox_amd/csrc/esdf3d.hip
@@ -13,7 +13,7 @@
   ListView lv;
   const int32_t n = list_open(m, S_LIST_ESDF_DIRTY, &lv);
   for (int32_t i = blockIdx.x; i < n; i += gridDim.x) {
-    const uint32_t s = (uint32_t)list_at(m, S_LIST_ESDF_DIRTY, lv, i);
+    const uint32_t s = (uint32_t)esdf_dirty_at(m, lv, i).x;
     const uint32_t flags = m.slot_flags[s];
     if (!(flags & (F_TSDF | F_ESDF))) continue;
     const float2 tv = m.tsdf[(size_t)s * 512 + tid];
diff --git a/isaac_ros_nvblox_amd/csrc/layers.hip b/isaac_ros_nvblox_amd/csrc/layers.hip
--- a/isaac_ros_nvblox_amd/csrc/layers.hip
+++ b/isaac_ros_nvblox_amd/csrc/layers.hip
@@ -82,7 +82,7 @@
       if (layer == F_TSDF) add |= F_DIRTY_ESDF | F_DIRTY_MESH;
       const uint32_t old = atomicOr(&m.slot_flags[s], add);
       if (layer == F_TSDF) {
-        if (!(old & F_DIRTY_ESDF)) list_append(m, S_LIST_ESDF_DIRTY, (int32_t)s);
+        if (!(old & F_DIRTY_ESDF)) esdf_dirty_append(m, (int32_t)s, x, y, z);
         if (!(old & F_DIRTY_MESH)) list_append(m, mesh_list, (int32_t)s);
       }
       if (layer == F_ESDF && z == bz_out) {
diff --git a/isaac_ros_nvblox_amd/csrc/lidar.hip b/isaac_ros_nvblox_amd/csrc/lidar.hip
--- a/isaac_ros_nvblox_amd/csrc/lidar.hip
+++ b/isaac_ros_nvblox_amd/csrc/lidar.hip
@@ -440,8 +440,9 @@
       float2 fin = *vp;
       if (tsdf_fuse_plain(f, &fin, d, r)) *vp = fin;
     }
+    const int32_t bx = __builtin_amdgcn_readlane(rec_g.y, 8 * j), by = __builtin_amdgcn_readlane(rec_g.z, 8 * j), bz = __builtin_amdgcn_readlane(rec_g.w, 8 * j);
     if (lane == 0) {
-      if (!(old & F_DIRTY_ESDF)) list_append(m, S_LIST_ESDF_DIRTY, (int32_t)slot);
+      if (!(old & F_DIRTY_ESDF)) esdf_dirty_append(m, (int32_t)slot, bx, by, bz);
       if (!(old & F_DIRTY_MESH)) list_append(m, mesh_list, (int32_t)slot);
     }
     n_mine++;
diff --git a/isaac_ros_nvblox_amd/csrc/maintenance.hip b/isaac_ros_nvblox_amd/csrc/maintenance.hip
--- a/isaac_ros_nvblox_amd/csrc/maintenance.hip
+++ b/isaac_ros_nvblox_amd/csrc/maintenance.hip
@@ -13,18 +13,23 @@
   m.slot_consumed[slot] = STAMP_NEVER; m.slot_stamp[slot] = STAMP_NEVER; m.slot_cam[slot] = STAMP_NEVER;
 }
 
-__device__ inline void wave_list_append(const DMap& m, int32_t list, bool push, int32_t v, int lane) {
+__device__ inline int32_t wave_list_reserve(const DMap& m, int32_t list, bool push, int lane) {
   const u64 mask = __ballot(push);
-  if (!mask) return;
-  const int sh = my_shard();
+  if (!mask) return -1;
   int32_t base = 0;
   const int leader = __ffsll((long long)mask) - 1;
-  if (lane == leader) base = atomicAdd(shc_at(m, list, sh, 0), (int32_t)__popcll(mask));
+  if (lane == leader) base = atomicAdd(shc_at(m, list, my_shard(), 0), (int32_t)__popcll(mask));
   base = __shfl(base, leader);
-  if (push) {
-    const int32_t p = base + (int32_t)__popcll(mask & ((1ull << lane) - 1ull));
-    if (p < (int32_t)m.capacity) m.lists[((size_t)list * NSH + sh) * m.capacity + p] = v;
-  }
+  const int32_t p = base + (int32_t)__popcll(mask & ((1ull << lane) - 1ull));
+  return push && p < (int32_t)m.capacity ? p : -1;
+}
+__device__ inline void wave_list_append(const DMap& m, int32_t list, bool push, int32_t v, int lane) {
+  const int32_t p = wave_list_reserve(m, list, push, lane);
+  if (p >= 0) m.lists[list_seg(list, my_shard()) * m.capacity + p] = v;
+}
+__device__ inline void wave_esdf_dirty_append(const DMap& m, bool push, int4 rec, int lane) {
+  const int32_t p = wave_list_reserve(m, S_LIST_ESDF_DIRTY, push, lane);
+  if (p >= 0) esdf_dirty_shard(m, my_shard())[p] = rec;
 }
 template <bool OCC>
 __global__ __launch_bounds__(512) __attribute__((amdgpu_waves_per_eu(8, 8))) void k_decay(DMap m, float factor, float thresh, uint32_t exclude_stamp, uint32_t exclude_mask, int32_t mesh_list,
@@ -100,7 +105,10 @@
       if (lane == j) { my_alive = alive; my_band = band; }
     }
     const int32_t slot = mine;
-    bool push_esdf = false, push_esdf2 = false, push_mesh = false, push_cleared = false; int32_t esdf2 = 0;
+    bool push_esdf = false, push_esdf2 = false, push_mesh = false, push_cleared = false;
+    int32_t ix = 0, iy = 0, iz = 0;
+    if (mine < hw && (act || (next_table && (fl & LAYER_MASK)))) { ix = m.slot_index[3 * slot]; iy = m.slot_index[3 * slot + 1]; iz = m.slot_index[3 * slot + 2]; }
+    const int4 rec = make_int4(slot, ix, iy, iz); int4 rec2 = make_int4(0, 0, 0, 0);
     if (act) {
       uint32_t old = F_DIRTY_MESH;
       if (my_alive) {
@@ -112,20 +120,20 @@
         if (!OCC) old = atomicOr(&m.slot_flags[slot], F_DIRTY_MESH);
         push_cleared = true;
         atomicAnd(&m.slot_flags[slot], ~(F_TSDF | F_COLOR | F_FEATURE | F_MESH | F_FREESPACE | F_BAND | F_BAND_STALE));
-        const int32_t bx = m.slot_index[3 * slot], by = m.slot_index[3 * slot + 1], bz = m.slot_index[3 * slot + 2];
+        const int32_t bx = ix, by = iy, bz = iz;
         if (bz >= bz_lo && bz <= bz_hi) {
           const uint32_t es = bz_out == INT32_MIN ? (uint32_t)slot : any_slot(m, bx, by, bz_out);
           if (slot_ok(es) && (m.slot_flags[es] & F_ESDF)) {
             const uint32_t eold = atomicOr(&m.slot_flags[es], F_ESDF_REMARK | F_DIRTY_ESDF);
-            if (!(eold & F_DIRTY_ESDF)) { push_esdf2 = true; esdf2 = (int32_t)es; }
+            if (!(eold & F_DIRTY_ESDF)) { push_esdf2 = true; rec2 = make_int4((int32_t)es, bx, by, bz_out == INT32_MIN ? bz : bz_out); }
           }
         }
         if (!(fl & (F_ESDF | F_ESDF_PENDING))) { atomicAnd(&m.slot_flags[slot], OCC ? ~(F_DIRTY_ESDF | F_DIRTY_MESH) : ~F_DIRTY_ESDF); free_slot(m, (uint32_t)slot); }
       }
       push_mesh = !(old & F_DIRTY_MESH);
     }
-    wave_list_append(m, S_LIST_ESDF_DIRTY, push_esdf, slot, lane);
-    wave_list_append(m, S_LIST_ESDF_DIRTY, push_esdf2, esdf2, lane);
+    wave_esdf_dirty_append(m, push_esdf, rec, lane);
+    wave_esdf_dirty_append(m, push_esdf2, rec2, lane);
     wave_list_append(m, mesh_list, push_mesh, slot, lane);
     {
       const u64 cm = __ballot(push_cleared);
@@ -136,14 +144,14 @@
         base = __shfl(base, leader);
         if (push_cleared) {
           const int32_t p = base + (int32_t)__popcll(cm & ((1ull << lane) - 1ull));
-          if (p < (int32_t)m.capacity) { cleared_idx[3 * p] = m.slot_index[3 * slot]; cleared_idx[3 * p + 1] = m.slot_index[3 * slot + 1]; cleared_idx[3 * p + 2] = m.slot_index[3 * slot + 2]; }
+          if (p < (int32_t)m.capacity) { cleared_idx[3 * p] = ix; cleared_idx[3 * p + 1] = iy; cleared_idx[3 * p + 2] = iz; }
         }
       }
     }
     if (next_table && mine < hw) {
       const uint32_t layers_after = (act && !my_alive) ? (fl & (F_ESDF | F_ESDF_PENDING)) : (fl & LAYER_MASK);
       if (layers_after) {
-        const int32_t x = m.slot_index[3 * slot], y = m.slot_index[3 * slot + 1], z = m.slot_index[3 * slot + 2];
+        const int32_t x = ix, y = iy, z = iz;
         const uint32_t stamp = m.table[m.slot_entry[slot]].stamp;
         const u64 key = pack_key(x, y, z);
         uint32_t h = table_pos(m, x, y, z);
@@ -235,7 +243,7 @@
     if (s_touched && !occupancy) publish_band(m.slot_flags, (uint32_t)slot, tid, in_band(fin.x, fin.y, trunc));
     if (tid == 0 && s_touched) {
       const uint32_t old = atomicOr(&m.slot_flags[slot], F_DIRTY_ESDF | F_DIRTY_MESH);
-      if (!(old & F_DIRTY_ESDF)) list_append(m, S_LIST_ESDF_DIRTY, slot);
+      if (!(old & F_DIRTY_ESDF)) esdf_dirty_append_slot(m, slot);
       if (!(old & F_DIRTY_MESH)) list_append(m, mesh_list, slot);
     }
   }
@@ -442,7 +450,7 @@
   uint32_t* saved = (uint32_t*)take((size_t)old_cap * sizeof(uint32_t)); ok = ok && saved;
   std::vector<void*> np(arrs.size(), nullptr);
   for (size_t i = 0; ok && i < arrs.size(); i++) { np[i] = take(arrs[i].bytes_per_block * (size_t)new_cap); ok = ok && np[i]; }
-  int32_t* nl = ok ? (int32_t*)take((size_t)N_LISTS * NSH * (size_t)new_cap * 4) : nullptr; ok = ok && nl;
+  int32_t* nl = ok ? (int32_t*)take((size_t)LIST_SEGS * (size_t)new_cap * 4) : nullptr; ok = ok && nl;
   float* nv = nullptr; float* nn = nullptr; uint8_t* nc = nullptr; int32_t* nt = nullptr;
   if (ok && grow_mesh) {
     nv = (float*)take(new_vcap * 12); nn = (float*)take(new_vcap * 12); nc = (uint8_t*)take(new_vcap * 4); nt = (int32_t*)take(new_tcap * 12);
@@ -461,8 +469,9 @@
     NVBX_HIP(hipMemcpyAsync(np[i], *a.p, a.bytes_per_block * (size_t)old_cap, hipMemcpyDeviceToDevice, stream));
     if (a.fill >= 0) NVBX_HIP(hipMemsetAsync((char*)np[i] + a.bytes_per_block * (size_t)old_cap, a.fill, a.bytes_per_block * (size_t)(new_cap - old_cap), stream));
   }
-  for (int q = 0; q < N_LISTS * NSH; q++)
-    NVBX_HIP(hipMemcpyAsync(nl + (size_t)q * new_cap, d.lists + (size_t)q * old_cap, (size_t)old_cap * 4, hipMemcpyDeviceToDevice, stream));
+  for (int l = 0; l < N_LISTS; l++)
+    for (int sh = 0; sh < NSH; sh++)
+      NVBX_HIP(hipMemcpyAsync(nl + list_seg(l, sh) * (size_t)new_cap, d.lists + list_seg(l, sh) * (size_t)old_cap, (size_t)old_cap * (l == S_LIST_ESDF_DIRTY ? 16 : 4), hipMemcpyDeviceToDevice, stream));
   if (grow_mesh) {
     const int64_t ovr = mesh_vert_cap / NSH, otr = mesh_tri_cap / NSH, nvr = new_vcap / NSH, ntr = new_tcap / NSH;
     if (mesh_epoch) {
diff --git a/isaac_ros_nvblox_amd/csrc/mapper.hip b/isaac_ros_nvblox_amd/csrc/mapper.hip
--- a/isaac_ros_nvblox_amd/csrc/mapper.hip
+++ b/isaac_ros_nvblox_amd/csrc/mapper.hip
@@ -56,7 +56,7 @@
       per_block(&mesh_rec, sizeof(MeshRecord), -1),
       PoolArr{reinterpret_cast<void**>(&d.freespace), 512 * 16, 0, 0},
       PoolArr{&feat_val, 1024 * (size_t)feat_channels, -1, 0}, PoolArr{reinterpret_cast<void**>(&feat_w), feat_channels ? (size_t)2048 : 0, -1, 0},
-      other(&d.table, hash_slots(cap) * sizeof(Entry)), other(&d.lists, (size_t)N_LISTS * NSH * n * 4),
+      other(&d.table, hash_slots(cap) * sizeof(Entry)), other(&d.lists, (size_t)LIST_SEGS * n * 4),
       other(&mesh_vert, mv * 12), other(&mesh_nrm, mv * 12), other(&mesh_col, mv * 4), other(&mesh_tri, mv * 2 * 12),
       other(&d.counters, C_NUM * 4), other(&d.shc, S_NUM * NSH * SH_STRIDE * 4), other(&export_count, 64),
       other(&table_spare, 0), other(&table_dirty, 0)};
diff --git a/isaac_ros_nvblox_amd/csrc/measure.hip b/isaac_ros_nvblox_amd/csrc/measure.hip
--- a/isaac_ros_nvblox_amd/csrc/measure.hip
+++ b/isaac_ros_nvblox_amd/csrc/measure.hip
@@ -56,7 +56,8 @@
   const int tid = threadIdx.x;
   if (blockIdx.x == 0 && tid == 64) __hip_atomic_store(&m.host_mirror[0], m.counters[C_FREE_TOP], __ATOMIC_RELAXED, __HIP_MEMORY_SCOPE_SYSTEM);
   for (int32_t i = blockIdx.x; i < n; i += gridDim.x) {
-    const uint32_t slot = (uint32_t)view_list[i].x;
+    const int4 rec = view_list[i];
+    const uint32_t slot = (uint32_t)rec.x;
     if (!slot_ok(slot)) continue;
     float2* vp = &m.tsdf[(size_t)slot * 512 + tid];
     float2 fin = *vp;
@@ -83,7 +84,7 @@
       if (tid == 0) { if (any_band) atomicOr(&m.slot_flags[slot], F_BAND); else atomicAnd(&m.slot_flags[slot], ~F_BAND); if (old & F_BAND_STALE) atomicAnd(&m.slot_flags[slot], ~F_BAND_STALE); }
     }
     if (tid == 0) {
-      if (!(old & F_DIRTY_ESDF)) list_append(m, S_LIST_ESDF_DIRTY, (int32_t)slot);
+      if (!(old & F_DIRTY_ESDF)) esdf_dirty_append(m, (int32_t)slot, rec.y, rec.z, rec.w);
       if (!(old & F_DIRTY_MESH)) list_append(m, mesh_list, (int32_t)slot);
     }
   }
diff --git a/isaac_ros_nvblox_amd/csrc/nvbx_esdf_mark.h b/isaac_ros_nvblox_amd/csrc/nvbx_esdf_mark.h
--- a/isaac_ros_nvblox_amd/csrc/nvbx_esdf_mark.h
+++ b/isaac_ros_nvblox_amd/csrc/nvbx_esdf_mark.h
@@ -3,11 +3,12 @@
 
 namespace nvbx {
 
-__device__ inline void esdf_mark_entry(const DMap& m, const EsdfArgs& a, uint32_t tslot, int srec, int sh, bool from_dirty_list = false) {
+__device__ inline void esdf_mark_entry(const DMap& m, const EsdfArgs& a, uint32_t tslot, int32_t bx, int32_t by, int32_t bz, int srec, int sh, bool from_dirty_list = false) {
   const int lane = threadIdx.x & 63;
   const int vx = lane & 7, vy = lane >> 3;
   const uint32_t tflags = m.slot_flags[tslot];
-  const int32_t bx = m.slot_index[3 * tslot], by = m.slot_index[3 * tslot + 1], bz = m.slot_index[3 * tslot + 2];
+  int32_t sx = bx, sy = by, sz = bz;
+  if (from_dirty_list) { sx = m.slot_index[3 * tslot]; sy = m.slot_index[3 * tslot + 1]; sz = m.slot_index[3 * tslot + 2]; }
   int32_t kz_lo = a.kz_min, kz_hi = a.kz_max, bz_lo = a.bz_lo, bz_hi = a.bz_hi;
   if (a.plane_on) {
     const float bs = a.voxel_size * 8.0f;
@@ -20,18 +21,26 @@
     if (bz_hi - bz_lo > 61) bz_hi = bz_lo + 61;
   }
   const int nz = bz_hi - bz_lo + 1;
-  if (from_dirty_list && !(tflags & F_DIRTY_ESDF)) return;
+  const bool z_in_band = bz >= bz_lo && bz <= bz_hi;
+  const int32_t qz = lane == 0 ? a.bz_out : bz_lo + lane - 1;
+  const bool own = qz == bz;
+  const bool probing = lane <= nz && !own;
+  const u64 qkey = pack_key(bx, by, qz);
+  const uint32_t qh = probing ? table_pos(m, bx, by, qz) : 0u;
+  uint4 qe = make_uint4(0u, 0u, 0u, 0u);
+  if (z_in_band) qe = ld_entry(m, qh);
+  __builtin_amdgcn_sched_barrier(0);
+  if (from_dirty_list && (!(tflags & F_DIRTY_ESDF) || sx != bx || sy != by || sz != bz)) return;
   NVBX_INV_TSDF_READER(m);
   NVBX_INV_COUNT(m, C_INV_I4, lane == 0 && from_dirty_list && !(tflags & (F_TSDF | F_ESDF)));
   NVBX_TV(0, 3, wall_clock64());
   if (lane == 0) { atomicAnd(&m.slot_flags[tslot], ~F_DIRTY_ESDF); m.slot_consumed[tslot] = a.mark_pass; }
-  if (!(tflags & F_ESDF_REMARK) && (bz < bz_lo || bz > bz_hi)) return;
-  const int32_t qz = lane == 0 ? a.bz_out : bz_lo + lane - 1;
-  const bool probing = lane <= nz;
-  const u64 qkey = pack_key(bx, by, qz);
-  const uint32_t qh = probing ? table_pos(m, bx, by, qz) : 0u;
-  const uint4 qe = ld_entry(m, qh);
+  if (!z_in_band) {
+    if (!(tflags & F_ESDF_REMARK)) return;
+    qe = ld_entry(m, qh);
+  }
   uint32_t qslot = probing ? resolve_any(m, qkey, qh, qe) : SLOT_NONE;
+  if (own && lane <= nz) qslot = tslot;
   uint32_t eslot = __shfl(qslot, 0);
   NVBX_TV(0, 4, wall_clock64());
   const bool early = (tflags & F_TSDF) && slot_ok(eslot);
@@ -96,13 +105,13 @@
   const int per = nwg >> 3;
   const int sh_l = wg & (NSH - 1), j0 = wg >> 3;
   if (per < 1 || j0 >= per) return;
-  const int32_t* base = &m.lists[((size_t)S_LIST_ESDF_DIRTY * NSH + sh_l) * m.capacity];
-  const int32_t first = base[j0];
+  const int4* base = esdf_dirty_shard(m, sh_l);
+  const int4 first = base[j0];
   int32_t cnt = *shc_at(m, S_LIST_ESDF_DIRTY, sh_l, 0);
   if (cnt > (int32_t)m.capacity) cnt = (int32_t)m.capacity;
   const int srec = S_ESDF_REC + (int)(a.epoch & 1), sh = my_shard();
   int n_done = 0;
-  for (int32_t j = j0; j < cnt; j += per) { esdf_mark_entry(m, a, (uint32_t)(j == j0 ? first : base[j]), srec, sh, true); n_done++;  if (n_done == 1) NVBX_TV(0, 1, wall_clock64()); }
+  for (int32_t j = j0; j < cnt; j += per) { const int4 r = j == j0 ? first : base[j]; esdf_mark_entry(m, a, (uint32_t)r.x, r.y, r.z, r.w, srec, sh, true); n_done++;  if (n_done == 1) NVBX_TV(0, 1, wall_clock64()); }
   NVBX_TV(0, 6, n_done); NVBX_TV(0, 2, wall_clock64());
 }
 
@@ -139,7 +148,7 @@
   for (int64_t i = wi; i < n; i += per_rank) {
     const uint32_t s = find_slot(m, idx[3 * i], idx[3 * i + 1], idx[3 * i + 2], F_TSDF);
     if (!slot_ok(s)) continue;
-    esdf_mark_entry(m, a, s, srec, sh);
+    esdf_mark_entry(m, a, s, idx[3 * i], idx[3 * i + 1], idx[3 * i + 2], srec, sh);
   }
 }
 
@@ -153,7 +162,7 @@
       const uint32_t s = find_slot(m, idx[3 * i], idx[3 * i + 1], idx[3 * i + 2], F_TSDF);
       if (!slot_ok(s)) continue;
       const uint32_t old = atomicOr(&m.slot_flags[s], F_DIRTY_ESDF);
-      if (!(old & F_DIRTY_ESDF)) list_append(m, S_LIST_ESDF_DIRTY, (int32_t)s);
+      if (!(old & F_DIRTY_ESDF)) esdf_dirty_append(m, (int32_t)s, idx[3 * i], idx[3 * i + 1], idx[3 * i + 2]);
     }
   }
 }
diff --git a/isaac_ros_nvblox_amd/csrc/nvbx_internal.h b/isaac_ros_nvblox_amd/csrc/nvbx_internal.h
--- a/isaac_ros_nvblox_amd/csrc/nvbx_internal.h
+++ b/isaac_ros_nvblox_amd/csrc/nvbx_internal.h
@@ -74,6 +74,8 @@
   S_NUM = 10
 };
 constexpr int N_LISTS = 4;
+constexpr int LIST_SEGS = (N_LISTS + 3) * NSH;
+__host__ __device__ inline size_t list_seg(int list, int shard) { return list == S_LIST_ESDF_DIRTY ? (size_t)4 * shard : (size_t)(list + 3) * NSH + shard; }
 
 struct DMap {
   Entry* table; uint32_t mask; uint32_t shift;
@@ -160,7 +162,16 @@
 __device__ inline void list_append(const DMap& m, int list, int32_t v) {
   const int sh = my_shard();
   const int32_t p = atomicAdd(shc_at(m, list, sh, 0), 1);
-  if (p < (int32_t)m.capacity) m.lists[((size_t)list * NSH + sh) * m.capacity + p] = v;
+  if (p < (int32_t)m.capacity) m.lists[list_seg(list, sh) * m.capacity + p] = v;
+}
+__device__ inline int4* esdf_dirty_shard(const DMap& m, int sh) { return reinterpret_cast<int4*>(m.lists) + (size_t)sh * m.capacity; }
+__device__ inline void esdf_dirty_append(const DMap& m, int32_t slot, int32_t x, int32_t y, int32_t z) {
+  const int sh = my_shard();
+  const int32_t p = atomicAdd(shc_at(m, S_LIST_ESDF_DIRTY, sh, 0), 1);
+  if (p < (int32_t)m.capacity) esdf_dirty_shard(m, sh)[p] = make_int4(slot, x, y, z);
+}
+__device__ inline void esdf_dirty_append_slot(const DMap& m, int32_t slot) {
+  esdf_dirty_append(m, slot, m.slot_index[3 * slot], m.slot_index[3 * slot + 1], m.slot_index[3 * slot + 2]);
 }
 struct ListView { int32_t pre[NSH + 1]; };
 __device__ inline int32_t list_open(const DMap& m, int list, ListView* v) {
@@ -172,11 +183,19 @@
   for (int s = 0; s < NSH; s++) v->pre[s + 1] = v->pre[s] + min(c[s], (int32_t)m.capacity);
   return v->pre[NSH];
 }
+__device__ inline int list_shard_of(const ListView& v, int32_t i, int32_t* base) {
+  int s = 0; *base = 0;
+#pragma unroll
+  for (int q = 1; q < NSH; q++) if (i >= v.pre[q]) { s = q; *base = v.pre[q]; }
+  return s;
+}
 __device__ inline int32_t list_at(const DMap& m, int list, const ListView& v, int32_t i) {
-  int s = 0; int32_t base = 0;
-#pragma unroll
-  for (int q = 1; q < NSH; q++) if (i >= v.pre[q]) { s = q; base = v.pre[q]; }
-  return m.lists[((size_t)list * NSH + s) * m.capacity + (i - base)];
+  int32_t base; const int s = list_shard_of(v, i, &base);
+  return m.lists[list_seg(list, s) * m.capacity + (i - base)];
+}
+__device__ inline int4 esdf_dirty_at(const DMap& m, const ListView& v, int32_t i) {
+  int32_t base; const int s = list_shard_of(v, i, &base);
+  return esdf_dirty_shard(m, s)[i - base];
 }
 __device__ inline void list_reset(const DMap& m, int list) {
 #pragma unroll
diff --git a/isaac_ros_nvblox_amd/csrc/tsdf.hip b/isaac_ros_nvblox_amd/csrc/tsdf.hip
--- a/isaac_ros_nvblox_amd/csrc/tsdf.hip
+++ b/isaac_ros_nvblox_amd/csrc/tsdf.hip
@@ -137,8 +137,9 @@
           if (tid == 0) { if (any_band) atomicOr(&m.slot_flags[slot], F_BAND); else atomicAnd(&m.slot_flags[slot], ~F_BAND); if (old & F_BAND_STALE) atomicAnd(&m.slot_flags[slot], ~F_BAND_STALE); }
         }
       }
+      const int32_t rx = __builtin_amdgcn_readlane(rec.y, j), ry = __builtin_amdgcn_readlane(rec.z, j), rz = __builtin_amdgcn_readlane(rec.w, j);
       if (tid == 0) {
-        if (!(old & F_DIRTY_ESDF)) list_append(m, S_LIST_ESDF_DIRTY, (int32_t)slot);
+        if (!(old & F_DIRTY_ESDF)) esdf_dirty_append(m, (int32_t)slot, rx, ry, rz);
         if (!(old & F_DIRTY_MESH)) list_append(m, mesh_list, (int32_t)slot);
       }
     }
```

Result: no change. 47550 frames/s (-0.2%).
